# DavidXu-JJ/StreetUnveiler

Measured on AMD Instinct MI355X. Metric: Msplats/s fwd+bwd @1920x1080, 3M Gaussians, higher is better.
Workload: dtype f32; 1 GPU; C3: 3M Gaussians, 1920x1080, fwd+bwd with depth/normal aux outputs (all 7 aux-map gradients live); gaussians=3000000, width=1920, height=1080, sh_degree=3, frames_per_rank=1, parallelism=single GPU, camera_rig=benchmark

## Files before the change

streetunveiler_amd/csrc/api.hip:

```cpp
#include <cfloat>
#include <cstdarg>
#include <cstdio>
#include <cstring>
#include <cmath>
#include <atomic>
#include <mutex>

#include "launch.h"

using namespace sr;

namespace {

thread_local char g_err[512] = "";
std::atomic<int> g_timing{0};
std::mutex g_ring_mu;

int fail(int code, const char* fmt, ...) {
    va_list ap;
    va_start(ap, fmt);
    vsnprintf(g_err, sizeof(g_err), fmt, ap);
    va_end(ap);
    return code;
}

#define SR_HIP(expr)                                                                                         \
    do {                                                                                                     \
        hipError_t _e = (expr);                                                                              \
        if (_e != hipSuccess) return fail(SR_ERR_HIP, "%s failed: %s (%s:%d)", #expr, hipGetErrorString(_e), \
                                          __FILE__, __LINE__);                                               \
    } while (0)

constexpr int kEvRing = 512;
struct EvRing {
    hipEvent_t ev[kEvRing][2];
    bool closed[kEvRing];
    int created = 0, used = 0;
};
EvRing g_ring[SR_STAGE_COUNT];

struct StageTimer {
    int stage; hipStream_t s; int slot = -1;
    StageTimer(int st, hipStream_t stream) : stage(st), s(stream) {
        const int mode = g_timing.load();
        if (!mode || (mode != 1 && !((mode >> 1) & (1 << stage)))) return;
        std::lock_guard<std::mutex> lk(g_ring_mu);
        EvRing& r = g_ring[stage];
        if (r.used >= kEvRing) return;
        if (r.used >= r.created) {
            if (hipEventCreate(&r.ev[r.created][0]) != hipSuccess || hipEventCreate(&r.ev[r.created][1]) != hipSuccess) return;
            ++r.created;
        }
        slot = r.used++;
        r.closed[slot] = false;
        (void)hipEventRecord(r.ev[slot][0], s);
    }
    ~StageTimer() {
        if (slot < 0) return;
        std::lock_guard<std::mutex> lk(g_ring_mu);
        if (hipEventRecord(g_ring[stage].ev[slot][1], s) == hipSuccess) g_ring[stage].closed[slot] = true;
    }
};

int debug_sync(const SrFrame* frame, hipStream_t s, const char* what) {
    if (!frame->debug) return SR_OK;
    hipError_t e = hipStreamSynchronize(s);
    if (e == hipSuccess) e = hipGetLastError();
    if (e != hipSuccess) return fail(SR_ERR_HIP, "[debug] after %s: %s", what, hipGetErrorString(e));
    return SR_OK;
}

uint32_t* pinned_words() {
    static thread_local uint32_t* pinned = nullptr;
    if (!pinned && hipHostMalloc(reinterpret_cast<void**>(&pinned), 64, hipHostMallocPortable | hipHostMallocMapped) != hipSuccess) { pinned = nullptr; (void)hipGetLastError(); }
    return pinned;
}

int stream_device(hipStream_t s, int* dev) {
    hipDevice_t d = 0;
    if (s && hipStreamGetDevice(s, &d) == hipSuccess) { *dev = (int)d; return SR_OK; }
    (void)hipGetLastError();
    SR_HIP(hipGetDevice(dev));
    return SR_OK;
}

constexpr int kMaxDevices = 64;
std::atomic<int> g_rank_mode[kMaxDevices];
int rank_mode(hipStream_t s, bool force_ballot, RankMode* mode) {
    int dev = 0;
    { const int rc = stream_device(s, &dev); if (rc != SR_OK) return rc; }
    if (dev < 0 || dev >= kMaxDevices) return fail(SR_ERR_UNSUPPORTED, "device index %d beyond %d", dev, kMaxDevices);
    int m = g_rank_mode[dev].load(std::memory_order_acquire);
    if (m == kRankUnknown) {
        hipStreamCaptureStatus cap = hipStreamCaptureStatusNone;
        if (hipStreamIsCapturing(s, &cap) == hipSuccess && cap != hipStreamCaptureStatusNone)
            return fail(SR_ERR_UNSUPPORTED, "the stream is capturing and device %d has not run the rank self-check yet: call sr_rank_mode(stream) once before the capture", dev);
        (void)hipGetLastError();
        struct Scratch { uint32_t* p = nullptr; ~Scratch() { if (p) (void)hipFree(p); } } scratch;
        uint32_t* host = pinned_words();
        uint32_t* result = nullptr;
        const bool temp = !(host && hipHostGetDevicePointer(reinterpret_cast<void**>(&result), host + 8, 0) == hipSuccess && result);
        if (!temp) host[8] = 0;
        else { (void)hipGetLastError(); SR_HIP(hipMalloc(reinterpret_cast<void**>(&scratch.p), 4)); result = scratch.p; SR_HIP(hipMemsetAsync(result, 0, 4, s)); }
        SR_HIP(launch_rank_selfcheck(result, s));
        uint32_t r = 0;
        if (temp) { SR_HIP(hipMemcpyAsync(&r, result, 4, hipMemcpyDeviceToHost, s)); SR_HIP(hipStreamSynchronize(s)); }
        else { SR_HIP(hipStreamSynchronize(s)); r = *reinterpret_cast<volatile uint32_t*>(host + 8); }
        if (!(r & 0x100u)) return fail(SR_ERR_HIP, "the rank self-check kernel did not report back");
        m = (r & 1u) ? kRankAtomic : ((r & 2u) ? kRankBallot : kRankNone);
        g_rank_mode[dev].store(m, std::memory_order_release);
    }
    if (m == kRankNone) return fail(SR_ERR_UNSUPPORTED, "neither LDS-atomic nor ballot ranking passes the self-check on device %d", dev);
    *mode = force_ballot ? kRankBallot : static_cast<RankMode>(m);
    return SR_OK;
}

constexpr int kMaxTilesPerAxis = SR_MAX_TILES_PER_AXIS;
template <class T> T* at(void* base, size_t off) { return reinterpret_cast<T*>(static_cast<char*>(base) + off); }
struct Carver {
    size_t off = 0;
    size_t take(size_t bytes) { const size_t o = off; off = align_up(off + bytes, 256); return o; }
};

struct GeomLayout {
    size_t recs, depth_keys, tiles_touched, rect, clamped, sorted_keys, sorted_gid, rect_sorted, first, sh_jac, block_base, base_bytes,
        counts, temp, temp_bytes, total;
};
GeomLayout geom_layout(int P) {
    GeomLayout L{};
    const size_t n = (size_t)(P > 0 ? P : 1);
    Carver c;
    L.recs = c.take(n * kRecFloats * 4);
    L.depth_keys = c.take(n * 4);
    L.tiles_touched = c.take(n * 4);
    L.rect = c.take(n * 8);
    L.clamped = c.take(n);
    L.sorted_keys = c.take(n * 4);
    L.sorted_gid = c.take(n * 4);
    L.rect_sorted = c.take(n * 8);
    L.first = c.take(n * 4);
    L.sh_jac = c.take(n * 36);
    L.base_bytes = tile_scan_temp_bytes(P);
    L.block_base = c.take(L.base_bytes);
    const size_t n_scan_blocks = (n + 2047) / 2048;
    L.counts = L.block_base + n_scan_blocks * 4;
    static thread_local int memo_P = -1;
    static thread_local size_t memo_bytes = 0;
    if (memo_P != P) {
        memo_bytes = depth_sort_temp_bytes(P);
        const size_t hx = align_up(expand_x_hist_bytes(P, kMaxTilesPerAxis), 256);
        if (hx > memo_bytes) memo_bytes = hx;
        memo_P = P;
    }
    L.temp_bytes = memo_bytes;
    L.temp = c.take(L.temp_bytes);
    L.total = c.off;
    return L;
}
enum FrameCount { kCountDuplicates = 0, kCountVisible = 1, kCountOverflow = 2 };
struct GeomView {
    float4* recs; uint32_t* depth_keys; uint32_t* tiles_touched; uint2* rect; uint8_t* clamped;
    uint32_t* sorted_keys; uint32_t* sorted_gid; uint2* rect_sorted; uint32_t* first;
    float* sh_jac;
    uint32_t* block_base; void* temp;
    uint32_t* counts;
};
GeomView geom_view(void* geom, const GeomLayout& L) {
    return GeomView{at<float4>(geom, L.recs), at<uint32_t>(geom, L.depth_keys), at<uint32_t>(geom, L.tiles_touched), at<uint2>(geom, L.rect),
                    at<uint8_t>(geom, L.clamped), at<uint32_t>(geom, L.sorted_keys), at<uint32_t>(geom, L.sorted_gid), at<uint2>(geom, L.rect_sorted),
                    at<uint32_t>(geom, L.first), at<float>(geom, L.sh_jac), at<uint32_t>(geom, L.block_base), at<void>(geom, L.temp),
                    at<uint32_t>(geom, L.counts)};
}

struct BinLayout {
    size_t columns, point_list, hit_mask, ranges, order, tile_counts, row_total, n_columns, hist, hist_bytes, total;
};
BinLayout bin_layout(uint32_t D, int W, int H) {
    BinLayout L{};
    const size_t n = (size_t)(D > 0 ? D : 1);
    const int tiles = ((W + 7) / 8) * ((H + 7) / 8);
    Carver c;
    L.columns = c.take(n * 8);
    L.point_list = c.take(n * 4);
    L.hit_mask = c.take(n * 2);
    L.ranges = c.take((size_t)(tiles > 0 ? tiles : 1) * 8);
    L.order = c.take((size_t)(tiles > 0 ? tiles : 1) * 4);
    L.tile_counts = c.take((size_t)(tiles > 0 ? tiles : 1) * 4);
    L.row_total = c.take((size_t)kMaxTilesPerAxis * 4);
    L.n_columns = c.take(4);
    L.hist_bytes = expand_y_hist_bytes(D, (H + 7) / 8);
    L.hist = c.take(L.hist_bytes);
    L.total = c.off;
    return L;
}
struct BinView {
    uint2* columns;
    uint32_t* point_list; uint16_t* hit_mask; uint2* ranges; uint32_t* order; uint32_t* tile_counts; uint32_t* row_total; uint32_t* n_columns; uint32_t* hist;
    uint32_t* class_list() const { return reinterpret_cast<uint32_t*>(columns); }
};
BinView bin_view(void* binning, const BinLayout& L) {
    return BinView{at<uint2>(binning, L.columns), at<uint32_t>(binning, L.point_list), at<uint16_t>(binning, L.hit_mask), at<uint2>(binning, L.ranges),
                   at<uint32_t>(binning, L.order), at<uint32_t>(binning, L.tile_counts), at<uint32_t>(binning, L.row_total), at<uint32_t>(binning, L.n_columns),
                   at<uint32_t>(binning, L.hist)};
}

struct ImgLayout { size_t final_T, n_contrib, total; };
ImgLayout img_layout(int W, int H) {
    ImgLayout L{};
    const size_t hw = (size_t)(W > 0 ? W : 1) * (size_t)(H > 0 ? H : 1);
    L.final_T = 0;
    L.n_contrib = align_up(hw * 3 * 4, 256);
    L.total = align_up(L.n_contrib + hw * 2 * 4, 256);
    return L;
}
struct ImgView { float* final_T; uint32_t* n_contrib; };
ImgView img_view(void* image, const ImgLayout& L) { return ImgView{at<float>(image, L.final_T), at<uint32_t>(image, L.n_contrib)}; }

size_t record_bytes(int color_channels) { return (size_t)(color_channels == 9 ? kGradFloats + 4 : kGradFloats) * 4; }
struct WorkspaceLayout { size_t written, total; };
WorkspaceLayout workspace_layout(uint32_t D, int color_channels) {
    const size_t n = (size_t)(D > 0 ? D : 1);
    WorkspaceLayout L{};
    L.written = align_up(n * record_bytes(color_channels), 256);
    L.total = L.written + align_up(n, 256);
    return L;
}
struct WorkspaceView { float4* records; uint8_t* written; };
WorkspaceView workspace_view(void* workspace, uint32_t D, int color_channels) {
    return WorkspaceView{static_cast<float4*>(workspace), at<uint8_t>(workspace, workspace_layout(D, color_channels).written)};
}

struct TileShape { int w, h; };
TileShape tile_shape(const SrFrame* frame) {
    return TileShape{frame->tile_width > 0 ? frame->tile_width : kTile, frame->tile_height > 0 ? frame->tile_height : kTile};
}

int check_common(const SrFrame* frame, const SrGaussians* g) {
    if (!frame || !g) return fail(SR_ERR_INVALID_ARGUMENT, "frame / gaussians is NULL");
    if (frame->image_width <= 0 || frame->image_height <= 0) return fail(SR_ERR_INVALID_ARGUMENT, "bad image size %dx%d", frame->image_width, frame->image_height);
    if (g->P < 0) return fail(SR_ERR_INVALID_ARGUMENT, "P < 0");
    {
        const TileShape t = tile_shape(frame);
        const bool known = (t.w == 16 && t.h == 16) || (t.w == 8 && t.h == 8) || (t.w == 16 && t.h == 8) || (t.w == 32 && t.h == 8) || (t.w == 32 && t.h == 16);
        if (!known) return fail(SR_ERR_UNSUPPORTED, "tile shape %dx%d not in {8x8, 16x8, 16x16, 32x8, 32x16}", t.w, t.h);
    }
    if (!frame->bg || !frame->viewmatrix || !frame->projmatrix || !frame->campos) return fail(SR_ERR_INVALID_ARGUMENT, "bg / viewmatrix / projmatrix / campos must be non-NULL device pointers");
    if (g->P > 0) {
        if (!g->means3D || !g->opacities) return fail(SR_ERR_INVALID_ARGUMENT, "means3D / opacities is NULL");
        if (g->color_channels == 9) {
            if (!g->shs || !g->colors_precomp) return fail(SR_ERR_INVALID_ARGUMENT, "9 colour channels need SHs AND a [P,6] precomputed colour array");
        } else if ((g->shs != nullptr) == (g->colors_precomp != nullptr)) return fail(SR_ERR_INVALID_ARGUMENT, "Please provide exactly one of either SHs or precomputed colors!");
        if (g->color_channels != 0 && g->color_channels != 3 && g->color_channels != 6 && g->color_channels != 9) return fail(SR_ERR_UNSUPPORTED, "color_channels %d not in {3, 6, 9}", g->color_channels);
        if (g->activations & ~(SR_ACT_EXP_SCALES | SR_ACT_SIGMOID_OPACITY | SR_ACT_NORMALIZE_ROTATIONS)) return fail(SR_ERR_UNSUPPORTED, "unknown activation bits 0x%x", g->activations);
        if (g->color_channels == 6 && g->shs) return fail(SR_ERR_INVALID_ARGUMENT, "6 colour channels need precomputed colors, not SHs");
        const bool sr_pair = g->scales != nullptr && g->rotations != nullptr;
        if ((g->scales != nullptr) != (g->rotations != nullptr) || sr_pair == (g->transMat_precomp != nullptr))
            return fail(SR_ERR_INVALID_ARGUMENT, "Please provide exactly one of either scale/rotation pair or precomputed transMat!");
        if (g->shs) {
            if (frame->sh_degree < 0 || frame->sh_degree > 3) return fail(SR_ERR_UNSUPPORTED, "sh_degree %d not in 0..3", frame->sh_degree);
            if (g->sh_coeffs < (frame->sh_degree + 1) * (frame->sh_degree + 1)) return fail(SR_ERR_INVALID_ARGUMENT, "shs has %d coefficients, degree %d needs %d", g->sh_coeffs, frame->sh_degree, (frame->sh_degree + 1) * (frame->sh_degree + 1));
        }
    }
    return SR_OK;
}

int check_backward_frame(const SrFrame* frame) {
#if SR_BACKWARD_WH_FROM_FOCAL
    if (!(frame->tanfovx > 0.f) || !(frame->tanfovy > 0.f) || !std::isfinite(frame->tanfovx) || !std::isfinite(frame->tanfovy))
        return fail(SR_ERR_INVALID_ARGUMENT, "tanfovx / tanfovy must be finite and > 0 for a backward call (got %g, %g)", (double)frame->tanfovx, (double)frame->tanfovy);
#else
    (void)frame;
#endif
    return SR_OK;
}

FrameDev make_frame(const SrFrame* frame, const SrGaussians* g) {
    FrameDev f{};
    f.W = frame->image_width; f.H = frame->image_height;
    f.bw_W = f.W; f.bw_H = f.H;
#if SR_BACKWARD_WH_FROM_FOCAL
    if (frame->tanfovx > 0.f && frame->tanfovy > 0.f && std::isfinite(frame->tanfovx) && std::isfinite(frame->tanfovy)) {
        const float focal_x = (float)f.W / (2.0f * frame->tanfovx), focal_y = (float)f.H / (2.0f * frame->tanfovy);
        f.bw_W = (int)(focal_x * frame->tanfovx * 2); f.bw_H = (int)(focal_y * frame->tanfovy * 2);
    }
#endif
    const TileShape t = tile_shape(frame);
    f.tile_w = t.w; f.tile_h = t.h;
    f.inv_tile_w = 1.f / (float)f.tile_w; f.inv_tile_h = 1.f / (float)f.tile_h;
    f.tiles_x = (f.W + f.tile_w - 1) / f.tile_w; f.tiles_y = (f.H + f.tile_h - 1) / f.tile_h;
    f.sh_degree = frame->sh_degree; f.sh_coeffs = g->sh_coeffs;
    f.colors = g->color_channels == 6 ? 6 : (g->color_channels == 9 ? 9 : 3);
    f.activations = g->activations;
    f.scale_modifier = frame->scale_modifier;
    f.bg = frame->bg; f.view = frame->viewmatrix; f.proj = frame->projmatrix; f.campos = frame->campos;
    f.overflow = nullptr;
    return f;
}
void set_backward_state(FrameDev* f, const SrFrame* frame, const GeomView& G) {
    f->first = G.first; f->first_base = G.block_base; f->sh_jac = G.sh_jac;
    if (frame->flags & SR_FLAG_BINNING_CAPACITY) f->overflow = G.counts + kCountOverflow;
}

int choose_blend(const SrFrame* frame, const FrameDev& f, bool forward_call, BlendChoice* out) {
    const uint32_t flags = frame->flags;
    const uint32_t pair = flags & (SR_FLAG_ONE_WAVE_BACKWARD | SR_FLAG_COOP_BACKWARD | SR_FLAG_ROW_BACKWARD);
    if (pair & (pair - 1))
        return fail(SR_ERR_INVALID_ARGUMENT, "SR_FLAG_ONE_WAVE_BACKWARD, SR_FLAG_COOP_BACKWARD and SR_FLAG_ROW_BACKWARD exclude each other (flags 0x%x)", pair);
    const bool reference = f.tile_w == 16 && f.tile_h == 16 && f.colors == 3;
    const bool cull = !(flags & SR_FLAG_NO_QUADRANT_CULL), counters = forward_call && frame->blend_counters != nullptr;
    const bool rows = forward_call && (flags & SR_FLAG_ROW_MAPPED_FORWARD), quads = forward_call && (flags & SR_FLAG_QUADRANT_MAPPED_FORWARD);
    const bool fwd_only = forward_call && (flags & SR_FLAG_FORWARD_ONLY);
    if (fwd_only && counters) return fail(SR_ERR_UNSUPPORTED, "SR_FLAG_FORWARD_ONLY and blend_counters exclude each other");
    if (counters && !(f.tile_w == 16 && f.tile_h == 16 && (f.colors == 3 || f.colors == 6)))
        return fail(SR_ERR_UNSUPPORTED, "blend_counters: the counting variant of the forward blend exists for the 16x16 tile with 3 or 6 colour channels only");
    if (rows && quads) return fail(SR_ERR_INVALID_ARGUMENT, "SR_FLAG_ROW_MAPPED_FORWARD and SR_FLAG_QUADRANT_MAPPED_FORWARD exclude each other");
    if (rows && (!reference || counters || !cull))
        return fail(SR_ERR_UNSUPPORTED, "SR_FLAG_ROW_MAPPED_FORWARD: 16x16 tile, three colour channels, no counters, culling on");
    if ((pair & SR_FLAG_ROW_BACKWARD) && (!reference || counters || !cull || quads || fwd_only))
        return fail(SR_ERR_UNSUPPORTED, "SR_FLAG_ROW_BACKWARD: 16x16 tile, three colour channels, no counters, culling on, the row-mapped forward, a backward to follow");
    out->cull = cull;
    out->mask = HitMaskFormat::kQuadrant;
    out->backward = BackwardBlend::kOneWave;
    out->forward = counters ? ForwardBlend::kCounting : ForwardBlend::kQuadrantBands;
    if (!reference) return SR_OK;
    out->backward = (pair & SR_FLAG_ROW_BACKWARD) ? BackwardBlend::kRows
                    : (pair & SR_FLAG_ONE_WAVE_BACKWARD) ? BackwardBlend::kOneWave
                    : (pair & SR_FLAG_COOP_BACKWARD) ? BackwardBlend::kCoop : BackwardBlend::kByTileCount;
    if (counters) return SR_OK;
    if (cull && !rows && !quads && (pair & SR_FLAG_COOP_BACKWARD)) out->forward = ForwardBlend::kCoop;
    else if (pair & SR_FLAG_ROW_BACKWARD) { out->forward = ForwardBlend::kRowsCellMasks; out->mask = HitMaskFormat::kCell; }
    else if (rows) out->forward = ForwardBlend::kRows;
    else if (cull && !quads) out->forward = ForwardBlend::kDevicePicked;
    return SR_OK;
}

}

extern "C" {

int sr_abi_version(void) { return SR_ABI_VERSION; }
uint32_t sr_build_switches(void) { return SR_SWITCH_BITS; }
const char* sr_last_error(void) { return g_err; }

size_t sr_geom_bytes(int32_t P) { return geom_layout(P).total; }
size_t sr_binning_bytes(int32_t P, uint32_t num_rendered, int32_t W, int32_t H) { (void)P; return bin_layout(num_rendered, W, H).total; }
size_t sr_image_bytes(int32_t W, int32_t H) { return img_layout(W, H).total; }
size_t sr_backward_workspace_bytes(int32_t P, uint32_t num_rendered, int32_t color_channels) { (void)P; return workspace_layout(num_rendered, color_channels).total; }

int sr_geom_view(void* geom, size_t geom_bytes, int32_t P, SrGeomView* out) {
    if (!geom || !out) return fail(SR_ERR_INVALID_ARGUMENT, "NULL argument");
    const GeomLayout L = geom_layout(P);
    if (geom_bytes < L.total) return fail(SR_ERR_BUFFER_TOO_SMALL, "geom buffer %zu < %zu", geom_bytes, L.total);
    const GeomView G = geom_view(geom, L);
    out->splats = reinterpret_cast<float*>(G.recs); out->depth_keys = G.depth_keys;
    out->tiles_touched = G.tiles_touched; out->clamped = G.clamped;
    out->sorted_gid = G.sorted_gid;
    out->frame_counts = G.counts;
    return SR_OK;
}

int sr_binning_view(void* binning, size_t binning_bytes, int32_t P, uint32_t D, int32_t W, int32_t H, SrBinningView* out) {
    (void)P;
    if (!binning || !out) return fail(SR_ERR_INVALID_ARGUMENT, "NULL argument");
    const BinLayout L = bin_layout(D, W, H);
    if (binning_bytes < L.total) return fail(SR_ERR_BUFFER_TOO_SMALL, "binning buffer %zu < %zu", binning_bytes, L.total);
    const BinView B = bin_view(binning, L);
    out->point_list = B.point_list;
    out->ranges = reinterpret_cast<uint32_t*>(B.ranges); out->tile_order = B.order;
    return SR_OK;
}

int sr_image_view(void* image, size_t image_bytes, int32_t W, int32_t H, SrImageView* out) {
    if (!image || !out) return fail(SR_ERR_INVALID_ARGUMENT, "NULL argument");
    const ImgLayout L = img_layout(W, H);
    if (image_bytes < L.total) return fail(SR_ERR_BUFFER_TOO_SMALL, "image buffer %zu < %zu", image_bytes, L.total);
    const ImgView I = img_view(image, L);
    out->final_T = I.final_T; out->n_contrib = I.n_contrib;
    return SR_OK;
}

int sr_forward_plan(const SrFrame* frame, const SrGaussians* g, void* geom, size_t geom_bytes, int32_t* radii,
                    uint32_t* num_rendered_host, void* stream) {
    if (int rc = check_common(frame, g)) return rc;
    if (!num_rendered_host) return fail(SR_ERR_INVALID_ARGUMENT, "num_rendered_host is NULL");
    *num_rendered_host = 0;
    const int P = g->P;
    if (P == 0) return SR_OK;
    if (!geom || !radii) return fail(SR_ERR_INVALID_ARGUMENT, "geom / radii is NULL");
    const GeomLayout L = geom_layout(P);
    if (geom_bytes < L.total) return fail(SR_ERR_BUFFER_TOO_SMALL, "geom buffer %zu < %zu", geom_bytes, L.total);
    const GeomView G = geom_view(geom, L);
    hipStream_t s = static_cast<hipStream_t>(stream);
    FrameDev f = make_frame(frame, g);
    f.sh_jac = (frame->flags & SR_FLAG_FORWARD_ONLY) ? nullptr : G.sh_jac;
    {
        StageTimer t(SR_STAGE_PREPROCESS, s);
        SR_HIP(launch_preprocess_forward(P, f, *g, G.recs, G.depth_keys, G.tiles_touched, G.rect, G.clamped, radii, s));
    }
    if (int rc = debug_sync(frame, s, "preprocess_forward")) return rc;
    RankMode sort_mode = kRankUnknown;
    if (int rc = rank_mode(s, (frame->flags & SR_FLAG_BALLOT_RANKING) != 0, &sort_mode)) return rc;
    const bool read_back = !(frame->flags & SR_FLAG_BINNING_CAPACITY);
    uint32_t* pinned = read_back ? pinned_words() : nullptr;
    uint32_t* pinned_dev = nullptr;
    if (pinned && (hipHostGetDevicePointer(reinterpret_cast<void**>(&pinned_dev), pinned, 0) != hipSuccess)) pinned_dev = nullptr;
    {
        StageTimer t(SR_STAGE_SCAN, s);
        SR_HIP(run_tile_count_scan(P, G.tiles_touched, G.first, G.block_base, L.base_bytes, pinned_dev, s));
    }
    if (int rc = debug_sync(frame, s, "emission_scan")) return rc;
    hipEvent_t copied = nullptr;
    if (read_back) {
        static thread_local hipEvent_t copied_ev[kMaxDevices] = {};
        int dev = 0;
        SR_HIP(hipGetDevice(&dev));
        if (dev >= 0 && dev < kMaxDevices) {
            if (!copied_ev[dev] && hipEventCreateWithFlags(&copied_ev[dev], hipEventDisableTiming) != hipSuccess) copied_ev[dev] = nullptr;
            copied = copied_ev[dev];
        }
        if (!pinned_dev) SR_HIP(hipMemcpyAsync(pinned ? pinned : num_rendered_host, G.counts + kCountDuplicates, 4, hipMemcpyDeviceToHost, s));
        if (copied && pinned && hipEventRecord(copied, s) != hipSuccess) copied = nullptr;
    }
    {
        StageTimer t(SR_STAGE_DEPTH_SORT, s);
        SR_HIP(run_depth_sort(P, G.depth_keys, G.rect, G.sorted_keys, G.sorted_gid, G.rect_sorted, G.temp, L.temp_bytes, sort_mode,
                              (frame->flags & SR_FLAG_ONE_SWEEP_SORT) != 0, f.tiles_x, f.tiles_y, G.counts + kCountVisible, s));
    }
    if (!read_back) {
        *num_rendered_host = 0xFFFFFFFFu;
        return debug_sync(frame, s, "depth_sort");
    }
    if (int rc = debug_sync(frame, s, "depth_sort")) return rc;
    if (copied && pinned) SR_HIP(hipEventSynchronize(copied));
    else SR_HIP(hipStreamSynchronize(s));
    if (pinned) *num_rendered_host = *reinterpret_cast<volatile uint32_t*>(pinned);
    return SR_OK;
}

namespace {
int bin_duplicates(const SrFrame* frame, const SrGaussians* g, const FrameDev& f, void* geom, size_t geom_bytes, const BinView& B,
                   uint32_t D, hipStream_t s, float4** recs_out) {
    const int P = g->P;
    const int n_tiles = f.tiles_x * f.tiles_y;
    *recs_out = nullptr;
    if (P > 0 && D > 0) {
        if (!geom) return fail(SR_ERR_INVALID_ARGUMENT, "geom is NULL");
        const GeomLayout L = geom_layout(P);
        if (geom_bytes < L.total) return fail(SR_ERR_BUFFER_TOO_SMALL, "geom buffer %zu < %zu", geom_bytes, L.total);
        const GeomView G = geom_view(geom, L);
        *recs_out = G.recs;
        if (f.tiles_x > kMaxTilesPerAxis || f.tiles_y > kMaxTilesPerAxis)
            return fail(SR_ERR_INVALID_ARGUMENT, "%d x %d tiles: at most %d per axis (use a larger tile)", f.tiles_x, f.tiles_y, kMaxTilesPerAxis);
        if (L.temp_bytes < expand_x_hist_bytes(P, f.tiles_x)) return fail(SR_ERR_BUFFER_TOO_SMALL, "geom scratch too small for the column histogram");
        RankMode sort_mode = kRankUnknown;
        if (int rc = rank_mode(s, (frame->flags & SR_FLAG_BALLOT_RANKING) != 0, &sort_mode)) return rc;
        if (frame->flags & SR_FLAG_BINNING_CAPACITY)
            SR_HIP(run_capacity_guard(G.counts, D, s));
        {
            StageTimer t(SR_STAGE_EXPAND_X, s);
            SR_HIP(run_expand_columns(P, f.tiles_x, n_tiles, G.rect_sorted, G.sorted_gid, B.columns, B.n_columns, static_cast<uint32_t*>(G.temp), B.row_total,
                                      B.tile_counts, sort_mode, G.counts + kCountVisible, s));
        }
        if (int rc = debug_sync(frame, s, "expand_columns")) return rc;
        {
            StageTimer t(SR_STAGE_EXPAND_Y, s);
            SR_HIP(run_expand_rows(D, f.tiles_x, f.tiles_y, B.columns, B.n_columns, B.hist, B.row_total, B.point_list, B.tile_counts, sort_mode, s));
        }
        if (int rc = debug_sync(frame, s, "expand_rows")) return rc;
    } else {
        SR_HIP(launch_zero_bytes(B.tile_counts, sizeof(uint32_t) * (size_t)n_tiles, s));
    }
    {
        StageTimer t(SR_STAGE_RANGES, s);
        SR_HIP(run_tile_ranges_order(n_tiles, B.tile_counts, B.ranges, B.order, s));
    }
    return debug_sync(frame, s, "tile_ranges");
}

struct ClassLayout { size_t state, last, tile_total, ranges, total; };
ClassLayout class_layout(int W, int H, int n_classes) {
    ClassLayout L{};
    const size_t hw = (size_t)(W > 0 ? W : 1) * (size_t)(H > 0 ? H : 1), n = (size_t)(n_classes > 0 ? n_classes : 1);
    const size_t tiles = (size_t)((W + 7) / 8) * (size_t)((H + 7) / 8);
    L.state = 0;
    L.last = align_up(n * 3 * hw * 4, 256);
    L.tile_total = L.last + align_up(n * hw * 4, 256);
    L.ranges = L.tile_total + align_up((tiles > 0 ? tiles : 1) * n * 4, 256);
    L.total = L.ranges + align_up((tiles > 0 ? tiles : 1) * n * 8, 256);
    return L;
}
struct ClassView { float* state; uint32_t* last; uint32_t* tile_total; uint2* ranges; };
ClassView class_view(void* class_image, const ClassLayout& L) {
    return ClassView{at<float>(class_image, L.state), at<uint32_t>(class_image, L.last), at<uint32_t>(class_image, L.tile_total), at<uint2>(class_image, L.ranges)};
}

enum class ClassIds { kInColors, kOwnArray };
int check_class_pass(const SrFrame* frame, const SrGaussians* g, int n_classes, ClassIds ids, bool refuse_transmat) {
    if (int rc = check_common(frame, g)) return rc;
    if (frame->flags & SR_FLAG_BINNING_CAPACITY) return fail(SR_ERR_UNSUPPORTED, "SR_FLAG_BINNING_CAPACITY serves the operator (sr_forward_* / sr_backward*), not the per-class pass");
    if (n_classes < 1 || n_classes > 6) return fail(SR_ERR_UNSUPPORTED, "n_classes %d not in 1..6", n_classes);
    if (ids == ClassIds::kInColors && g->P > 0 && (g->shs || !g->colors_precomp || (g->color_channels != 0 && g->color_channels != 3)))
        return fail(SR_ERR_INVALID_ARGUMENT, "the per-class distortion pass takes the class ids in colors_precomp[P,3] (column 0), no SHs");
    if (refuse_transmat && g->transMat_precomp) return fail(SR_ERR_UNSUPPORTED, "the per-class pass takes scales and rotations, not a precomputed transMat");
    return SR_OK;
}
}

int sr_forward_render(const SrFrame* frame, const SrGaussians* g, void* geom, size_t geom_bytes, void* binning,
                      size_t binning_bytes, void* image, size_t image_bytes, uint32_t D, float* out_color,
                      float* out_allmap, void* stream) {
    if (int rc = check_common(frame, g)) return rc;
    const FrameDev f = make_frame(frame, g);
    BlendChoice blend;
    if (int rc = choose_blend(frame, f, true, &blend)) return rc;
    const bool fwd_only = (frame->flags & SR_FLAG_FORWARD_ONLY) != 0;
    if (!binning || (!image && !fwd_only) || !out_color || !out_allmap) return fail(SR_ERR_INVALID_ARGUMENT, "binning / image / out_color / out_allmap is NULL");
    const int W = frame->image_width, H = frame->image_height;
    const BinLayout BL = bin_layout(D, W, H);
    const ImgLayout IL = img_layout(W, H);
    if (binning_bytes < BL.total) return fail(SR_ERR_BUFFER_TOO_SMALL, "binning buffer %zu < %zu", binning_bytes, BL.total);
    if (!fwd_only && image_bytes < IL.total) return fail(SR_ERR_BUFFER_TOO_SMALL, "image buffer %zu < %zu", image_bytes, IL.total);
    const BinView B = bin_view(binning, BL);
    const ImgView I = fwd_only ? ImgView{nullptr, nullptr} : img_view(image, IL);
    hipStream_t s = static_cast<hipStream_t>(stream);
    float4* recs = nullptr;
    if (int rc = bin_duplicates(frame, g, f, geom, geom_bytes, B, D, s, &recs)) return rc;
    {
        StageTimer t(SR_STAGE_BLEND_FWD, s);
        const GeomView G = geom_view(geom, geom_layout(g->P));
        SR_HIP(launch_render_forward(f, B.ranges, B.order, B.point_list, recs, g->colors_precomp, out_color, out_allmap, I.final_T, I.n_contrib,
                                     fwd_only ? nullptr : B.hit_mask, blend, reinterpret_cast<unsigned long long*>(frame->blend_counters), G.counts, s));
    }
    return debug_sync(frame, s, "render_forward");
}

size_t sr_class_image_bytes(int32_t W, int32_t H, int32_t n_classes) { return class_layout(W, H, n_classes).total; }

int sr_class_forward_render(const SrFrame* frame, const SrGaussians* g, int32_t n_classes, void* geom, size_t geom_bytes, void* binning,
                            size_t binning_bytes, void* class_image, size_t class_image_bytes, uint32_t D, float* out_dist, void* stream) {
    if (int rc = check_class_pass(frame, g, n_classes, ClassIds::kInColors, false)) return rc;
    if (!binning || !class_image || !out_dist) return fail(SR_ERR_INVALID_ARGUMENT, "binning / class_image / out_dist is NULL");
    if (g->P > 0 && !geom) return fail(SR_ERR_INVALID_ARGUMENT, "geom is NULL (the class ids of the P Gaussians are staged in it, even when no duplicate was emitted)");
    const int W = frame->image_width, H = frame->image_height;
    const BinLayout BL = bin_layout(D, W, H);
    const ClassLayout CL = class_layout(W, H, n_classes);
    if (binning_bytes < BL.total) return fail(SR_ERR_BUFFER_TOO_SMALL, "binning buffer %zu < %zu", binning_bytes, BL.total);
    if (class_image_bytes < CL.total) return fail(SR_ERR_BUFFER_TOO_SMALL, "class image buffer %zu < %zu", class_image_bytes, CL.total);
    const BinView B = bin_view(binning, BL);
    const ClassView C = class_view(class_image, CL);
    hipStream_t s = static_cast<hipStream_t>(stream);
    const FrameDev f = make_frame(frame, g);
    float4* recs = nullptr;
    if (int rc = bin_duplicates(frame, g, f, geom, geom_bytes, B, D, s, &recs)) return rc;
    {
        StageTimer t(SR_STAGE_CLASS_PARTITION, s);
        uint8_t* ids = g->P > 0 && geom ? reinterpret_cast<uint8_t*>(geom_view(geom, geom_layout(g->P)).sh_jac) : nullptr;
        SR_HIP(launch_class_partition(g->P, f.tiles_x * f.tiles_y, n_classes, g->colors_precomp, nullptr, B.ranges, B.point_list, ids, B.class_list(), C.ranges, s));
    }
    if (int rc = debug_sync(frame, s, "class_partition")) return rc;
    {
        StageTimer t(SR_STAGE_CLASS_FWD, s);
        SR_HIP(launch_class_forward(f, n_classes, C.ranges, B.order, B.class_list(), recs, out_dist, C.state, C.last, C.tile_total, B.hit_mask,
                                    (frame->flags & SR_FLAG_NO_QUADRANT_CULL) ? 0 : 1, s));
    }
    return debug_sync(frame, s, "class_forward");
}

int sr_class_backward(const SrFrame* frame, const SrGaussians* g, int32_t n_classes, const int32_t* radii, void* geom, size_t geom_bytes,
                      void* binning, size_t binning_bytes, void* class_image, size_t class_image_bytes, uint32_t D, const float* dL_ddist,
                      void* workspace, size_t workspace_bytes, const SrGradients* grads, void* stream) {
    if (int rc = check_class_pass(frame, g, n_classes, ClassIds::kInColors, false)) return rc;
    if (int rc = check_backward_frame(frame)) return rc;
    if (!grads) return fail(SR_ERR_INVALID_ARGUMENT, "grads is NULL");
    const int P = g->P;
    if (P == 0) return SR_OK;
    if (!radii || !geom || !binning || !class_image || !dL_ddist || !workspace) return fail(SR_ERR_INVALID_ARGUMENT, "NULL buffer argument");
    const int W = frame->image_width, H = frame->image_height;
    const GeomLayout L = geom_layout(P);
    const BinLayout BL = bin_layout(D, W, H);
    const ClassLayout CL = class_layout(W, H, n_classes);
    if (geom_bytes < L.total || binning_bytes < BL.total || class_image_bytes < CL.total) return fail(SR_ERR_BUFFER_TOO_SMALL, "state buffer too small");
    if (workspace_bytes < workspace_layout(D, 3).total) return fail(SR_ERR_BUFFER_TOO_SMALL, "workspace %zu < %zu", workspace_bytes, workspace_layout(D, 3).total);
    const GeomView G = geom_view(geom, L);
    const BinView B = bin_view(binning, BL);
    const ClassView C = class_view(class_image, CL);
    const WorkspaceView ws = workspace_view(workspace, D, 3);
    hipStream_t s = static_cast<hipStream_t>(stream);
    FrameDev f = make_frame(frame, g);
    f.first = G.first; f.first_base = G.block_base; f.sh_jac = G.sh_jac;
    {
        StageTimer t(SR_STAGE_CLASS_BWD, s);
        if (D > 0) SR_HIP(launch_zero_bytes(ws.written, D, s));
        if (D > 0)
            SR_HIP(launch_class_backward(f, n_classes, C.ranges, B.order, B.class_list(), G.recs, C.state, C.last, C.tile_total, dL_ddist, B.hit_mask,
                                         ws.records, ws.written, 0, s));
    }
    if (int rc = debug_sync(frame, s, "class_backward")) return rc;
    {
        StageTimer t(SR_STAGE_PREPROCESS_BWD, s);
        SR_HIP(launch_preprocess_backward(P, f, *g, radii, G.clamped, G.recs, ws.records, ws.written, G.tiles_touched, *grads, s));
    }
    return debug_sync(frame, s, "preprocess_backward");
}

namespace {
struct ClassSharedLayout { ClassLayout C; size_t ids, hit, total; };
ClassSharedLayout class_shared_layout(int P, int W, int H, int n_classes, uint32_t D) {
    ClassSharedLayout L{};
    L.C = class_layout(W, H, n_classes);
    L.ids = L.C.total;
    L.hit = L.ids + align_up((size_t)(P > 0 ? P : 1), 256);
    L.total = L.hit + align_up((size_t)(D > 0 ? D : 1) * 2, 256);
    return L;
}
}

size_t sr_class_shared_bytes(int32_t P, int32_t W, int32_t H, int32_t n_classes, uint32_t D) { return class_shared_layout(P, W, H, n_classes, D).total; }

int sr_class_forward_shared(const SrFrame* frame, const SrGaussians* g, int32_t n_classes, const int32_t* classes, void* geom, size_t geom_bytes,
                            void* binning, size_t binning_bytes, void* class_state, size_t class_state_bytes, uint32_t D, float* out_dist, void* stream) {
    if (int rc = check_class_pass(frame, g, n_classes, ClassIds::kOwnArray, true)) return rc;
    if (!binning || !class_state || !out_dist || (g->P > 0 && !classes)) return fail(SR_ERR_INVALID_ARGUMENT, "binning / class_state / out_dist / classes is NULL");
    const int W = frame->image_width, H = frame->image_height, P = g->P;
    const BinLayout BL = bin_layout(D, W, H);
    const ClassSharedLayout SL = class_shared_layout(P, W, H, n_classes, D);
    if (binning_bytes < BL.total) return fail(SR_ERR_BUFFER_TOO_SMALL, "binning buffer %zu < %zu", binning_bytes, BL.total);
    if (class_state_bytes < SL.total) return fail(SR_ERR_BUFFER_TOO_SMALL, "class state buffer %zu < %zu", class_state_bytes, SL.total);
    float4* recs = nullptr;
    if (P > 0 && D > 0) {
        if (!geom) return fail(SR_ERR_INVALID_ARGUMENT, "geom is NULL");
        const GeomLayout L = geom_layout(P);
        if (geom_bytes < L.total) return fail(SR_ERR_BUFFER_TOO_SMALL, "geom buffer %zu < %zu", geom_bytes, L.total);
        recs = geom_view(geom, L).recs;
    }
    const BinView B = bin_view(binning, BL);
    const ClassView C = class_view(class_state, SL.C);
    hipStream_t s = static_cast<hipStream_t>(stream);
    const FrameDev f = make_frame(frame, g);
    {
        StageTimer t(SR_STAGE_CLASS_PARTITION, s);
        SR_HIP(launch_class_partition(P, f.tiles_x * f.tiles_y, n_classes, nullptr, classes, B.ranges, B.point_list, at<uint8_t>(class_state, SL.ids), B.class_list(),
                                      C.ranges, s));
    }
    if (int rc = debug_sync(frame, s, "class_partition")) return rc;
    {
        StageTimer t(SR_STAGE_CLASS_FWD, s);
        SR_HIP(launch_class_forward(f, n_classes, C.ranges, B.order, B.class_list(), recs, out_dist, C.state, C.last, C.tile_total, at<uint16_t>(class_state, SL.hit),
                                    (frame->flags & SR_FLAG_NO_QUADRANT_CULL) ? 0 : 1, s));
    }
    return debug_sync(frame, s, "class_forward");
}

int sr_class_backward_shared(const SrFrame* frame, const SrGaussians* g, int32_t n_classes, void* geom, size_t geom_bytes, void* binning,
                             size_t binning_bytes, void* class_state, size_t class_state_bytes, uint32_t D, const float* dL_ddist, void* workspace,
                             size_t workspace_bytes, void* stream) {
    if (int rc = check_class_pass(frame, g, n_classes, ClassIds::kOwnArray, false)) return rc;
    if (int rc = check_backward_frame(frame)) return rc;
    const int P = g->P;
    if (P == 0 || D == 0) return SR_OK;
    if (!geom || !binning || !class_state || !dL_ddist || !workspace) return fail(SR_ERR_INVALID_ARGUMENT, "NULL buffer argument");
    const int W = frame->image_width, H = frame->image_height;
    const GeomLayout L = geom_layout(P);
    const BinLayout BL = bin_layout(D, W, H);
    const ClassSharedLayout SL = class_shared_layout(P, W, H, n_classes, D);
    if (geom_bytes < L.total || binning_bytes < BL.total || class_state_bytes < SL.total) return fail(SR_ERR_BUFFER_TOO_SMALL, "state buffer too small");
    const size_t ws_bytes = workspace_layout(D, g->color_channels).total;
    if (workspace_bytes < ws_bytes) return fail(SR_ERR_BUFFER_TOO_SMALL, "workspace %zu < %zu", workspace_bytes, ws_bytes);
    const GeomView G = geom_view(geom, L);
    const BinView B = bin_view(binning, BL);
    const ClassView C = class_view(class_state, SL.C);
    const WorkspaceView ws = workspace_view(workspace, D, g->color_channels);
    hipStream_t s = static_cast<hipStream_t>(stream);
    FrameDev f = make_frame(frame, g);
    f.first = G.first; f.first_base = G.block_base;
    {
        StageTimer t(SR_STAGE_CLASS_BWD, s);
        SR_HIP(launch_class_backward(f, n_classes, C.ranges, B.order, B.class_list(), G.recs, C.state, C.last, C.tile_total, dL_ddist, at<uint16_t>(class_state, SL.hit),
                                     ws.records, ws.written, (int)(record_bytes(g->color_channels) / 16), s));
    }
    return debug_sync(frame, s, "class_backward_shared");
}

namespace {
struct BackwardCtx {
    int P; GeomView G; BinView B; ImgView I; WorkspaceView ws; FrameDev f; BlendChoice blend; hipStream_t s;
};
int backward_ctx(const SrFrame* frame, const SrGaussians* g, void* geom, size_t geom_bytes, void* binning, size_t binning_bytes,
                 void* image, size_t image_bytes, uint32_t D, void* workspace, size_t workspace_bytes, void* stream, BackwardCtx* c) {
    if (int rc = check_common(frame, g)) return rc;
    if (int rc = check_backward_frame(frame)) return rc;
    c->f = make_frame(frame, g);
    if (int rc = choose_blend(frame, c->f, false, &c->blend)) return rc;
    c->P = g->P;
    if (c->P == 0) return SR_OK;
    if (!geom || !binning || !image || !workspace) return fail(SR_ERR_INVALID_ARGUMENT, "NULL buffer argument");
    const int W = frame->image_width, H = frame->image_height;
    const GeomLayout L = geom_layout(c->P);
    const BinLayout BL = bin_layout(D, W, H);
    const ImgLayout IL = img_layout(W, H);
    if (geom_bytes < L.total) return fail(SR_ERR_BUFFER_TOO_SMALL, "geom buffer %zu < %zu", geom_bytes, L.total);
    if (binning_bytes < BL.total) return fail(SR_ERR_BUFFER_TOO_SMALL, "binning buffer %zu < %zu", binning_bytes, BL.total);
    if (image_bytes < IL.total) return fail(SR_ERR_BUFFER_TOO_SMALL, "image buffer %zu < %zu", image_bytes, IL.total);
    const size_t ws_bytes = workspace_layout(D, g->color_channels).total;
    if (workspace_bytes < ws_bytes) return fail(SR_ERR_BUFFER_TOO_SMALL, "workspace %zu < %zu", workspace_bytes, ws_bytes);
    c->G = geom_view(geom, L); c->B = bin_view(binning, BL); c->I = img_view(image, IL);
    c->ws = workspace_view(workspace, D, g->color_channels);
    c->s = static_cast<hipStream_t>(stream);
    set_backward_state(&c->f, frame, c->G);
    return SR_OK;
}
}

int sr_backward_blend(const SrFrame* frame, const SrGaussians* g, void* geom, size_t geom_bytes, void* binning, size_t binning_bytes,
                      void* image, size_t image_bytes, uint32_t D, const float* dL_dcolor, const float* dL_dallmap, void* workspace,
                      size_t workspace_bytes, void* stream) {
    BackwardCtx c;
    if (int rc = backward_ctx(frame, g, geom, geom_bytes, binning, binning_bytes, image, image_bytes, D, workspace, workspace_bytes, stream, &c)) return rc;
    if (c.P == 0) return SR_OK;
    if (!dL_dcolor || !dL_dallmap) return fail(SR_ERR_INVALID_ARGUMENT, "dL_dcolor / dL_dallmap is NULL");
    {
        StageTimer t(SR_STAGE_BLEND_BWD, c.s);
        if (D > 0) SR_HIP(launch_zero_bytes(c.ws.written, D, c.s));
        if (D > 0)
            SR_HIP(launch_render_backward(c.f, c.B.ranges, c.B.order, c.B.point_list, c.G.recs, g->colors_precomp, c.I.final_T, c.I.n_contrib, dL_dcolor, dL_dallmap,
                                          c.B.hit_mask, c.ws.records, c.ws.written, !(frame->flags & SR_FLAG_NO_PRECOMP_COLOR_GRAD), c.blend.backward, c.s));
    }
    return debug_sync(frame, c.s, "render_backward");
}

// ... 376 lines not shown
```

streetunveiler_amd/csrc/binning.hip:

```cpp
#include "launch.h"

namespace sr {

constexpr int kXpThreads = 256, kXpWaves = kXpThreads / 64;
constexpr int kXpInputsX = 1024, kXpInputsY = 2048;
template <int AXIS> constexpr int xp_inputs() { return AXIS == 0 ? kXpInputsX : kXpInputsY; }
constexpr int kXpBatch = 2048;
constexpr int kXpMaxBins = 1024;
__device__ inline uint32_t pack_column(int miny, int h, int tx) { return (uint32_t)miny | ((uint32_t)h << 10) | ((uint32_t)tx << 21); }

__device__ inline uint32_t block_exclusive_scan(uint32_t x, uint32_t* s_w, uint32_t& total) {
    const int lane = threadIdx.x & 63, w = threadIdx.x >> 6;
    uint32_t incl = wave_inclusive_scan(x);
    __syncthreads();
    if (lane == 63) s_w[w] = incl;
    __syncthreads();
    uint32_t off = 0, tot = 0;
#pragma unroll
    for (int k = 0; k < kXpWaves; ++k) { const uint32_t c = s_w[k]; if (k < w) off += c; tot += c; }
    total = tot;
    return off + incl - x;
}

template <int AXIS> __device__ inline void expansion_of(uint2 item, int& start, int& len) {
// ... 27 lines not shown
        const uint32_t idx = base + (uint32_t)(i * kXpThreads + tid);
        if (idx < n) {
            const uint2 it = in[idx];
            int start, len; expansion_of<AXIS>(it, start, len);
            if (len) {
                atomicAdd(&s_diff[start], 1u); atomicSub(&s_diff[start + len], 1u);
                if (AXIS == 1) {
                    const int tx = (int)(it.y >> 21);
                    const uint32_t rel = (uint32_t)(tx - tx0);
                    if (rel < 4u) { atomicAdd(&s_full[rel][start], 1u); atomicSub(&s_full[rel][start + len], 1u); }
                    else for (int k = 0; k < len; ++k) atomicAdd(&tile_counts[(start + k) * tiles_x + tx], 1u);
                }
            }
        }
    }
    __syncthreads();
    {
        uint32_t v[4], sum = 0;
#pragma unroll
        for (int j = 0; j < 4; ++j) { const int b = 4 * tid + j; sum += b < bins ? s_diff[b] : 0u; v[j] = sum; }
        uint32_t total;
        const uint32_t excl = block_exclusive_scan(sum, s_w, total);
#pragma unroll
        for (int j = 0; j < 4; ++j) { const int b = 4 * tid + j; if (b < bins) hist[(size_t)b * stride + blockIdx.x] = excl + v[j]; }
    }
    if (AXIS == 1 && tx0 + w < tiles_x) {
        uint32_t carry = 0;
        for (int c = 0; c < bins; c += 64) {
            const int row = c + lane;
            uint32_t incl = wave_inclusive_scan(row < bins ? s_full[w][row] : 0u);
            const uint32_t cnt = carry + incl;
            if (row < bins && cnt) atomicAdd(&tile_counts[row * tiles_x + tx0 + w], cnt);
            carry += (uint32_t)__shfl((int)incl, 63);
        }
    }
}

__global__ __launch_bounds__(kXpThreads) void expand_scan_rows_kernel(uint32_t* __restrict__ hist, int stride, uint32_t n_host,
                                                                      const uint32_t* __restrict__ n_dev, int inputs_per_block,
                                                                      uint32_t* __restrict__ row_total) {
    __shared__ uint32_t s_w[kXpWaves];
    const uint32_t n = n_dev ? *n_dev : n_host;
    const int nblocks = (int)((n + (uint32_t)inputs_per_block - 1) / (uint32_t)inputs_per_block);
    uint32_t* row = hist + (size_t)blockIdx.x * stride;
    uint32_t carry = 0;
    for (int c = 0; c < nblocks; c += kXpThreads) {
        const int i = c + (int)threadIdx.x;
        const uint32_t x = i < nblocks ? row[i] : 0u;
        uint32_t total;
        const uint32_t excl = block_exclusive_scan(x, s_w, total);
        if (i < nblocks) row[i] = carry + excl;
        carry += total;
    }
    if (threadIdx.x == 0) row_total[blockIdx.x] = carry;
}

template <int AXIS, int kBits, bool kAtomicRank>
__global__ __launch_bounds__(kXpThreads) void expand_scatter_kernel(
    const uint2* __restrict__ in, uint32_t n_host, const uint32_t* __restrict__ n_dev, int bins, const uint32_t* __restrict__ hist, int stride,
    const uint32_t* __restrict__ row_total,
    const uint32_t* __restrict__ sorted_gid, uint2* __restrict__ columns_out, uint32_t* __restrict__ n_columns_out,
    uint32_t* __restrict__ point_list) {
    constexpr int kBins = 1 << kBits;
    constexpr int kPer = kBins / kXpThreads > 0 ? kBins / kXpThreads : 1;
    constexpr int kInputs = xp_inputs<AXIS>(), kXpPerThread = kInputs / kXpThreads;
    __shared__ __attribute__((aligned(16))) uint8_t s_start[kXpBatch];
    __shared__ uint32_t s_prefix[kInputs + 1];
    __shared__ uint32_t s_count[kXpWaves][kBins];
    __shared__ uint32_t s_lstart[kBins];
    __shared__ uint32_t s_goff[kBins];
    __shared__ uint32_t s_w[kXpWaves];
    __shared__ uint32_t s_id[kXpBatch];
    __shared__ uint32_t s_rows[AXIS == 0 ? kXpBatch : 1];
    __shared__ uint16_t s_dig[kXpBatch];
    const int tid = threadIdx.x, lane = tid & 63, w = tid >> 6;
    const uint32_t n = n_dev ? *n_dev : n_host;
    const uint32_t base = blockIdx.x * (uint32_t)kInputs;
    if (base >= n) return;
    const int n_items = (int)min((uint32_t)kInputs, n - base);
    uint32_t E;
    uint32_t it_first[kXpPerThread];
    {
        uint32_t incl[kXpPerThread], sum = 0;
#pragma unroll
        for (int i = 0; i < kXpPerThread; ++i) {
            const int j = tid * kXpPerThread + i;
            int start = 0, len = 0;
            if (j < n_items) {
                const uint2 it = in[base + j];
                expansion_of<AXIS>(it, start, len);
            }
            it_first[i] = len ? sum : 0xFFFFFFFFu;
            sum += (uint32_t)len;
            incl[i] = sum;
        }
        for (int k = tid; k < kXpBatch / 4; k += kXpThreads) reinterpret_cast<uint32_t*>(s_start)[k] = 0;
        const uint32_t excl = block_exclusive_scan(sum, s_w, E);
#pragma unroll
        for (int i = 0; i < kXpPerThread; ++i) {
            s_prefix[tid * kXpPerThread + i + 1] = excl + incl[i];
            if (it_first[i] != 0xFFFFFFFFu) it_first[i] += excl;
        }
        if (tid == 0) s_prefix[0] = 0;
    }
    {
        uint32_t v[kPer], sum = 0;
#pragma unroll
        for (int j = 0; j < kPer; ++j) { const int d = tid * kPer + j; const uint32_t c = (d < bins) ? row_total[d] : 0u; v[j] = sum; sum += c; }
        uint32_t total;
        const uint32_t excl = block_exclusive_scan(sum, s_w, total);
#pragma unroll
        for (int j = 0; j < kPer; ++j) { const int d = tid * kPer + j; if (d < kBins) s_goff[d] = d < bins ? excl + v[j] + hist[(size_t)d * stride + blockIdx.x] : 0u; }
        if (AXIS == 0 && blockIdx.x == 0 && tid == 0) *n_columns_out = total;
    }
    for (uint32_t q0 = 0; q0 < E; q0 += kXpBatch) {
        for (int k = tid; k < kXpWaves * kBins; k += kXpThreads) (&s_count[0][0])[k] = 0;
#pragma unroll
        for (int i = 0; i < kXpPerThread; ++i)
            if (it_first[i] - q0 < (uint32_t)kXpBatch) s_start[it_first[i] - q0] = 1;
        __syncthreads();
        const uint32_t s0 = q0 + (uint32_t)(w * (kXpBatch / kXpWaves));
        uint32_t marks_before = 0;
        if (s0 < E) {
            int lo = 0;
#pragma unroll
            for (int step = kInputs / 2; step > 0; step >>= 1)
                if (lo + step < n_items && s_prefix[lo + step] <= s0) lo += step;
            marks_before = (uint32_t)lo + (s_prefix[lo] == s0 ? 0u : 1u);
        }
        uint32_t dig[kXpBatch / kXpThreads], id[kXpBatch / kXpThreads], rows[AXIS == 0 ? kXpBatch / kXpThreads : 1];
#pragma unroll
        for (int i = 0; i < kXpBatch / kXpThreads; ++i) {
            const uint32_t slot = s0 + (uint32_t)(i * 64 + lane);
            dig[i] = 0; id[i] = 0;
            if (AXIS == 0) rows[i] = 0;
            const bool mark = slot < E && s_start[slot - q0] != 0;
            const unsigned long long marks = ballot64(mark);
            const uint32_t lo = marks_before + __builtin_amdgcn_mbcnt_hi((uint32_t)(marks >> 32), __builtin_amdgcn_mbcnt_lo((uint32_t)marks, 0u)) +
                                (mark ? 1u : 0u) - 1u;
            marks_before += (uint32_t)__popcll(marks);
            if (slot < E) {
                const uint2 it = in[base + lo];
                int start, len; expansion_of<AXIS>(it, start, len);
                dig[i] = (uint32_t)start + (slot - s_prefix[lo]);
                if (AXIS == 0) { id[i] = sorted_gid[base + lo]; rows[i] = (it.x >> 16) | ((it.y >> 16) << 10); }
                else id[i] = it.x;
                atomicAdd(&s_count[w][dig[i]], 1u);
            }
        }
        __syncthreads();
        for (int k = tid; k < kXpBatch / 4; k += kXpThreads) reinterpret_cast<uint32_t*>(s_start)[k] = 0;
        uint32_t tot[kPer];
        {
            uint32_t sum = 0;
#pragma unroll
            for (int j = 0; j < kPer; ++j) {
                const int d = tid * kPer + j;
                tot[j] = 0;
                if (d < kBins) {
#pragma unroll
                    for (int k = 0; k < kXpWaves; ++k) tot[j] += s_count[k][d];
                }
                sum += tot[j];
            }
            uint32_t total;
            uint32_t run = block_exclusive_scan(sum, s_w, total);
#pragma unroll
            for (int j = 0; j < kPer; ++j) {
                const int d = tid * kPer + j;
                if (d < kBins) {
                    s_lstart[d] = run;
#pragma unroll
                    for (int k = 0; k < kXpWaves; ++k) { const uint32_t c = s_count[k][d]; s_count[k][d] = run; run += c; }
                }
            }
        }
        __syncthreads();
#pragma unroll
        for (int i = 0; i < kXpBatch / kXpThreads; ++i) {
            const uint32_t slot = q0 + (uint32_t)(w * (kXpBatch / kXpWaves) + i * 64 + lane);
            const bool live = slot < E;
            const uint32_t d = dig[i];
            const uint32_t pos = take_run_slot<kAtomicRank>(s_count[w], d, live, kBits);
            if (live) { s_id[pos] = id[i]; s_dig[pos] = (uint16_t)d; if (AXIS == 0) s_rows[pos] = rows[i]; }
        }
        __syncthreads();
        const uint32_t count = min((uint32_t)kXpBatch, E - q0);
#pragma unroll
        for (int i = 0; i < kXpBatch / kXpThreads; ++i) {
            const uint32_t li = (uint32_t)(i * kXpThreads + tid);
            if (li < count) {
                const uint32_t d = s_dig[li];
                const uint32_t g = s_goff[d] + (li - s_lstart[d]);
                if (AXIS == 0) columns_out[g] = make_uint2(s_id[li], s_rows[li] | (d << 21));
                else point_list[g] = s_id[li];
            }
        }
        __syncthreads();
#pragma unroll
        for (int j = 0; j < kPer; ++j) { const int d = tid * kPer + j; if (d < kBins) s_goff[d] += tot[j]; }
    }
}

constexpr int kOrderThreads = 1024, kOrderClasses = 16;
__device__ __forceinline__ uint32_t row_inclusive_scan16(uint32_t x) {
    int v = (int)x;
    v += __builtin_amdgcn_update_dpp(0, v, 0x111, 0xf, 0xf, true);
    v += __builtin_amdgcn_update_dpp(0, v, 0x112, 0xf, 0xf, true);
    v += __builtin_amdgcn_update_dpp(0, v, 0x114, 0xf, 0xf, true);
    v += __builtin_amdgcn_update_dpp(0, v, 0x118, 0xf, 0xf, true);
    return (uint32_t)v;
}
__global__ __launch_bounds__(kOrderThreads) void tile_ranges_order_kernel(int n_tiles, const uint32_t* __restrict__ counts, uint2* __restrict__ ranges,
                                                                          uint32_t* __restrict__ order) {
    constexpr int kPer = 8, kWaves = kOrderThreads / 64, kChunk = kOrderThreads * kPer;
    static_assert(kWaves == 16 && kOrderClasses == 16, "the cross-wave prefix below runs on 16 x 16 values, one 16-lane row per class");
    __shared__ uint32_t s_cls[kOrderClasses][kWaves];
    __shared__ uint32_t s_off[kOrderClasses][kWaves];
    __shared__ uint32_t s_tot[kOrderClasses];
    __shared__ uint32_t s_wsum[kWaves], s_woff[kWaves];
    __shared__ uint32_t s_carry, s_cls_base[kOrderClasses];
    const int tid = threadIdx.x, lane = tid & 63, w = tid >> 6;
    auto cls_of = [](uint32_t len) { return len ? min(kOrderClasses - 1, max(0, (int)__clz(len) - 11)) : kOrderClasses - 1; };
    const bool single_chunk = n_tiles <= kChunk;
    if (tid < kOrderClasses) s_cls_base[tid] = 0;
    if (tid == 0) s_carry = 0;
    if (!single_chunk) {
        uint32_t my_cls[kOrderClasses];
#pragma unroll
        for (int k = 0; k < kOrderClasses; ++k) my_cls[k] = 0;
        for (int t = tid; t < n_tiles; t += kOrderThreads) { const int c = cls_of(counts[t]);
#pragma unroll
            for (int k = 0; k < kOrderClasses; ++k) my_cls[k] += (c == k); }
        __syncthreads();
#pragma unroll
        for (int k = 0; k < kOrderClasses; ++k) {
            const uint32_t v = wave_inclusive_scan(my_cls[k]);
            if (lane == 63 && v) atomicAdd(&s_cls_base[k], v);
        }
        __syncthreads();
        if (tid == 0) { uint32_t run = 0; for (int k = 0; k < kOrderClasses; ++k) { const uint32_t c = s_cls_base[k]; s_cls_base[k] = run; run += c; } }
    }
    __syncthreads();
    for (int base = 0; base < n_tiles; base += kChunk) {
        const int t0 = base + tid * kPer;
        uint32_t c[kPer], sum = 0;
#pragma unroll
        for (int i = 0; i < kPer; ++i) { c[i] = t0 + i < n_tiles ? counts[t0 + i] : 0u; sum += c[i]; }
        const uint32_t incl = wave_inclusive_scan(sum);
        if (lane == 63) s_wsum[w] = incl;
        uint32_t mine[kOrderClasses];
#pragma unroll
        for (int k = 0; k < kOrderClasses; ++k) mine[k] = 0;
#pragma unroll
        for (int i = 0; i < kPer; ++i) { if (t0 + i < n_tiles) { const int cl = cls_of(c[i]);
#pragma unroll
            for (int k = 0; k < kOrderClasses; ++k) mine[k] += (cl == k); } }
        uint32_t before[kOrderClasses];
#pragma unroll
        for (int k = 0; k < kOrderClasses; ++k) {
            const uint32_t v = wave_inclusive_scan(mine[k]);
            before[k] = v - mine[k];
            if (lane == 63) s_cls[k][w] = v;
        }
        __syncthreads();
        if (tid < kOrderClasses * kWaves) {
            const uint32_t v = s_cls[tid >> 4][tid & 15], in = row_inclusive_scan16(v);
            s_off[tid >> 4][tid & 15] = in - v;
            if ((tid & 15) == 15) s_tot[tid >> 4] = in;
        } else if (tid < kOrderClasses * kWaves + 64) {
            const int j = tid - kOrderClasses * kWaves;
            const uint32_t v = j < kWaves ? s_wsum[j] : 0u, in = row_inclusive_scan16(v);
            if (j < kWaves) s_woff[j] = in - v;
        }
        __syncthreads();
        if (single_chunk) {
            if (tid == 0) { uint32_t run = 0; for (int k = 0; k < kOrderClasses; ++k) { s_cls_base[k] = run; run += s_tot[k]; } }
            __syncthreads();
        }
        uint32_t run = s_carry + s_woff[w] + incl - sum;
#pragma unroll
        for (int k = 0; k < kOrderClasses; ++k) before[k] += s_cls_base[k] + s_off[k][w];
#pragma unroll
        for (int i = 0; i < kPer; ++i) {
            if (t0 + i < n_tiles) {
                ranges[t0 + i] = c[i] ? make_uint2(run, run + c[i]) : make_uint2(0u, 0u);
                run += c[i];
                const int cl = cls_of(c[i]);
                uint32_t pos = 0;
#pragma unroll
                for (int k = 0; k < kOrderClasses; ++k) { if (cl == k) { pos = before[k]; before[k] += 1; } }
                order[pos] = (uint32_t)(t0 + i);
            }
        }
        __syncthreads();
        if (tid == kOrderThreads - 1) s_carry = run;
        if (tid < kOrderClasses) s_cls_base[tid] += s_tot[tid];
        __syncthreads();
    }
}

size_t depth_sort_temp_bytes(int P) {
    const uint32_t n = (uint32_t)(P > 0 ? P : 1);
    return align_up(radix_sort_temp_bytes(n), 256);
}
size_t tile_scan_temp_bytes(int P) { return tile_count_scan_temp_bytes((uint32_t)(P > 0 ? P : 1)); }

size_t expand_x_hist_bytes(int P, int tiles_x) { return (size_t)tiles_x * (((size_t)(P > 0 ? P : 1) + kXpInputsX - 1) / kXpInputsX) * 4; }
size_t expand_y_hist_bytes(uint32_t D, int tiles_y) { return (size_t)tiles_y * (((size_t)(D > 0 ? D : 1) + kXpInputsY - 1) / kXpInputsY) * 4; }

hipError_t run_depth_sort(int P, const uint32_t* depth_keys, const uint2* rect, uint32_t* sorted_keys,
                          uint32_t* sorted_gid, uint2* rect_sorted, void* temp, size_t temp_bytes, RankMode rank_mode, bool one_sweep, int tiles_x,
                          int tiles_y, const uint32_t* n_visible, hipStream_t s) {
    if (P == 0) return hipSuccess;
    const int bx = 32 - __builtin_clz((unsigned)(tiles_x > 0 ? tiles_x : 1)), by = 32 - __builtin_clz((unsigned)(tiles_y > 0 ? tiles_y : 1));
    return radix_sort_pairs(depth_keys, nullptr, sorted_keys, sorted_gid, (uint32_t)P, 32, temp, temp_bytes, s, rect, rect_sorted, rank_mode, one_sweep, bx, by, n_visible);
}

hipError_t run_tile_count_scan(int P, const uint32_t* tiles_touched, uint32_t* first, void* block_base, size_t base_bytes, uint32_t* total_host,
                               hipStream_t s) {
    if (P == 0) return hipSuccess;
    return tile_count_scan(tiles_touched, first, (uint32_t)P, block_base, base_bytes, total_host, s);
}

template <int AXIS, bool kAtomicRank, typename... Args>
static void launch_expand_scatter_r(int bins, int blocks, hipStream_t s, Args... a) {
    if (bins <= 128) hipLaunchKernelGGL((expand_scatter_kernel<AXIS, 7, kAtomicRank>), dim3(blocks), dim3(kXpThreads), 0, s, a...);
    else if (bins <= 256) hipLaunchKernelGGL((expand_scatter_kernel<AXIS, 8, kAtomicRank>), dim3(blocks), dim3(kXpThreads), 0, s, a...);
    else if (bins <= 512) hipLaunchKernelGGL((expand_scatter_kernel<AXIS, 9, kAtomicRank>), dim3(blocks), dim3(kXpThreads), 0, s, a...);
    else hipLaunchKernelGGL((expand_scatter_kernel<AXIS, 10, kAtomicRank>), dim3(blocks), dim3(kXpThreads), 0, s, a...);
}
template <int AXIS, typename... Args>
static void launch_expand_scatter(RankMode rank_mode, int bins, int blocks, hipStream_t s, Args... a) {
    if (rank_mode == kRankAtomic) launch_expand_scatter_r<AXIS, true>(bins, blocks, s, a...);
    else launch_expand_scatter_r<AXIS, false>(bins, blocks, s, a...);
}

hipError_t run_expand_columns(int P, int tiles_x, int n_tiles, const uint2* rect_sorted, const uint32_t* sorted_gid, uint2* columns,
                              uint32_t* n_columns, uint32_t* hist, uint32_t* row_total, uint32_t* tile_counts, RankMode rank_mode, const uint32_t* n_visible,
                              hipStream_t s) {
    if (P == 0) return hipSuccess;
    if (tiles_x > kXpMaxBins || (rank_mode != kRankAtomic && rank_mode != kRankBallot)) return hipErrorInvalidValue;
    const int nb = (P + kXpInputsX - 1) / kXpInputsX;
    hipLaunchKernelGGL(expand_hist_kernel<0>, dim3(nb), dim3(kXpThreads), 0, s, rect_sorted, (uint32_t)P, n_visible, tiles_x, hist, nb,
                       tiles_x, tile_counts, n_tiles);
    hipLaunchKernelGGL(expand_scan_rows_kernel, dim3(tiles_x), dim3(kXpThreads), 0, s, hist, nb, (uint32_t)P, n_visible, kXpInputsX, row_total);
    launch_expand_scatter<0>(rank_mode, tiles_x, nb, s, rect_sorted, (uint32_t)P, n_visible, tiles_x, (const uint32_t*)hist, nb,
                             (const uint32_t*)row_total, sorted_gid, columns, n_columns, (uint32_t*)nullptr);
    return hipGetLastError();
}

hipError_t run_expand_rows(uint32_t D, int tiles_x, int tiles_y, const uint2* columns, const uint32_t* n_columns, uint32_t* hist, uint32_t* row_total,
                           uint32_t* point_list, uint32_t* tile_counts, RankMode rank_mode, hipStream_t s) {
    if (D == 0) return hipSuccess;
    if (tiles_y > kXpMaxBins || (rank_mode != kRankAtomic && rank_mode != kRankBallot)) return hipErrorInvalidValue;
    const int nb = (int)((D + kXpInputsY - 1) / kXpInputsY);
    hipLaunchKernelGGL(expand_hist_kernel<1>, dim3(nb), dim3(kXpThreads), 0, s, columns, D, n_columns, tiles_y, hist, nb, tiles_x, tile_counts,
                       tiles_x * tiles_y);
    hipLaunchKernelGGL(expand_scan_rows_kernel, dim3(tiles_y), dim3(kXpThreads), 0, s, hist, nb, D, n_columns, kXpInputsY, row_total);
    launch_expand_scatter<1>(rank_mode, tiles_y, nb, s, columns, D, n_columns, tiles_y, (const uint32_t*)hist, nb, (const uint32_t*)row_total,
                             (const uint32_t*)nullptr, (uint2*)nullptr, (uint32_t*)nullptr, point_list);
    return hipGetLastError();
}

__global__ void capacity_guard_kernel(uint32_t* __restrict__ counts, uint32_t capacity) {
    const uint32_t over = counts[0] > capacity ? 1u : 0u;
    counts[2] = over;
    if (over) counts[1] = 0u;
}
__global__ __launch_bounds__(256) void zero_bytes_kernel(uint8_t* __restrict__ p, size_t n) {
    const size_t head = (size_t)((16 - (reinterpret_cast<uintptr_t>(p) & 15)) & 15);
    const size_t h = head < n ? head : n;
    const size_t body = (n - h) / 16;
    const size_t i = (size_t)blockIdx.x * 256 + threadIdx.x, stride = (size_t)gridDim.x * 256;
    uint4* q = reinterpret_cast<uint4*>(p + h);
    for (size_t k = i; k < body; k += stride) q[k] = make_uint4(0u, 0u, 0u, 0u);
    if (i < h) p[i] = 0;
    const size_t tail0 = h + body * 16;
    if (i < n - tail0) p[tail0 + i] = 0;
}
hipError_t launch_zero_bytes(void* p, size_t n, hipStream_t s) {
    if (n == 0) return hipSuccess;
    const size_t blocks = (n / 16 + 255) / 256;
    hipLaunchKernelGGL(zero_bytes_kernel, dim3((unsigned)(blocks < 1 ? 1 : (blocks > 4096 ? 4096 : blocks))), dim3(256), 0, s, static_cast<uint8_t*>(p), n);
    return hipGetLastError();
}

hipError_t run_capacity_guard(uint32_t* counts, uint32_t capacity, hipStream_t s) {
    hipLaunchKernelGGL(capacity_guard_kernel, dim3(1), dim3(1), 0, s, counts, capacity);
    return hipGetLastError();
}

hipError_t run_tile_ranges_order(int n_tiles, const uint32_t* tile_counts, uint2* ranges, uint32_t* order, hipStream_t s) {
    if (n_tiles == 0) return hipSuccess;
    hipLaunchKernelGGL(tile_ranges_order_kernel, dim3(1), dim3(kOrderThreads), 0, s, n_tiles, tile_counts, ranges, order);
    return hipGetLastError();
}

}
```

streetunveiler_amd/csrc/common.h:

```cpp
#pragma once
#include <hip/hip_runtime.h>
#include <stdint.h>

#include "../../include/surfel_raster.h"
#include "../../include/surfel_switches.h"

#if defined(__HIP_DEVICE_COMPILE__) && !defined(__gfx950__)
#error "these kernels are written for gfx950 (MI355X): wave64, v_permlane16/32_swap, DPP row controls, and the LDS-atomic lane order the sort kernels rank by (checked at run time, api.hip rank_mode)"
#endif

namespace sr {

constexpr int kTile = SR_TILE;
constexpr int kBlock = kTile * kTile;
constexpr float kNear = 0.2f;
constexpr float kFar = 100.0f;
constexpr float kFilterSize = 0.707106f;
constexpr float kFilterInvSquare = 2.0f;
constexpr float kCutoff = 3.0f;
constexpr float kAlphaCap = 0.99f;
constexpr float kAlphaFloor = 1.0f / 255.0f;
constexpr float kTStop = 0.0001f;
constexpr uint32_t kCulledKey = 0xFFFFFFFFu;

constexpr int kRecQuads = 5;
constexpr int kRecFloats = SR_SPLAT_FLOATS;

constexpr int kGradQuads = 6;
constexpr int kGradFloats = SR_GRAD_FLOATS;

struct FrameDev {
    int W, H, tiles_x, tiles_y;
    int bw_W, bw_H;
    int tile_w, tile_h;
    float inv_tile_w, inv_tile_h;
    int sh_degree, sh_coeffs;
    int colors;
    int activations;
    float scale_modifier;
    const float* bg;
    const float* view;
    const float* proj;
    const float* campos;
    const uint32_t* first;
    const uint32_t* first_base;
    float* sh_jac;
    const uint32_t* overflow;
};
constexpr int kScanTile = 2048;
__device__ __forceinline__ uint32_t first_index(const FrameDev& f, uint32_t gid) { return f.first[gid] + f.first_base[gid / kScanTile]; }

__host__ __device__ inline size_t align_up(size_t x, size_t a) { return (x + a - 1) / a * a; }

__device__ __forceinline__ unsigned long long ballot64(bool p) { return __builtin_amdgcn_ballot_w64(p); }

__device__ __forceinline__ uint32_t wave_inclusive_scan(uint32_t x) {
    int v = (int)x;
    v += __builtin_amdgcn_update_dpp(0, v, 0x111, 0xf, 0xf, true);
    v += __builtin_amdgcn_update_dpp(0, v, 0x112, 0xf, 0xf, true);
    v += __builtin_amdgcn_update_dpp(0, v, 0x114, 0xf, 0xf, true);
    v += __builtin_amdgcn_update_dpp(0, v, 0x118, 0xf, 0xf, true);
    v += __builtin_amdgcn_update_dpp(0, v, 0x142, 0xa, 0xf, true);
    v += __builtin_amdgcn_update_dpp(0, v, 0x143, 0xc, 0xf, true);
    return (uint32_t)v;
}

template <bool kAtomic>
__device__ __forceinline__ uint32_t take_run_slot(uint32_t* run, uint32_t d, bool live, int bits) {
    uint32_t pos = 0;
    if (kAtomic) {
        if (live) pos = atomicAdd(&run[d], 1u);
        return pos;
    }
    unsigned long long same = ballot64(live);
    for (int b = 0; b < bits; ++b) {
        const unsigned long long vote = ballot64(((d >> b) & 1u) != 0u);
        same &= ((d >> b) & 1u) ? vote : ~vote;
    }
    const uint32_t lane = threadIdx.x & 63u;
    const uint32_t rank = (uint32_t)__popcll(same & ((1ull << lane) - 1ull));
    if (live) pos = run[d] + rank;
    __builtin_amdgcn_wave_barrier();
    if (live && rank == 0) run[d] += (uint32_t)__popcll(same);
    __builtin_amdgcn_wave_barrier();
    return pos;
}
enum RankMode { kRankUnknown = 0, kRankAtomic = 1, kRankBallot = 2, kRankNone = 3 };

}
```

streetunveiler_amd/csrc/launch.h:

```cpp
#pragma once
#include "common.h"

namespace sr {

enum class ForwardBlend {
    kDevicePicked,
    kQuadrantBands,
    kRows,
    kRowsCellMasks,
    kCoop,
    kCounting,
};
enum class BackwardBlend {
    kByTileCount,
    kOneWave,
    kCoop,
    kRows,
};
enum class HitMaskFormat { kQuadrant, kCell };
struct BlendChoice {
    ForwardBlend forward;
    BackwardBlend backward;
    HitMaskFormat mask;
    bool cull;
};

hipError_t launch_preprocess_forward(int P, const FrameDev& f, const SrGaussians& g, float4* recs, uint32_t* depth_keys,
                                     uint32_t* tiles_touched, uint2* rect, uint8_t* clamped, int32_t* radii, hipStream_t s);
hipError_t launch_preprocess_backward(int P, const FrameDev& f, const SrGaussians& g, const int32_t* radii,
                                      const uint8_t* clamped, const float4* recs, const float4* inst_grads, const uint8_t* written,
                                      const uint32_t* tiles_touched, const SrGradients& out, hipStream_t s);
hipError_t launch_mark_visible(int P, const float* means3D, const float* view, uint8_t* present, hipStream_t s);
hipError_t launch_sh_gradient_expand(int P, int M, int deg, int V, const float* means3D, const float* campos, const float* gc,
                                     float* dL_dsh, hipStream_t s);
hipError_t launch_color_gradients(int P, const FrameDev& f, const int32_t* radii, const uint8_t* clamped, const float4* recs, const float4* inst_grads,
                                  const uint8_t* written, const uint32_t* tiles_touched, bool mask_clamped, float* dL_dcolors, hipStream_t s);

size_t radix_sort_temp_bytes(uint32_t n);
hipError_t radix_sort_pairs(const uint32_t* keys_in, const uint32_t* vals_in, uint32_t* keys_out, uint32_t* vals_out, uint32_t n,
                            int total_bits, void* temp, size_t temp_bytes, hipStream_t s, const uint2* aux_src, uint2* aux_out, RankMode rank_mode,
                            bool one_sweep, int rect_bx = 0, int rect_by = 0, const uint32_t* n_live = nullptr);
size_t tile_count_scan_temp_bytes(uint32_t n);
hipError_t tile_count_scan(const uint32_t* counts, uint32_t* out, uint32_t n, void* temp, size_t temp_bytes, uint32_t* total_host, hipStream_t s);
hipError_t launch_rank_selfcheck(uint32_t* result, hipStream_t s);
hipError_t lds_atomic_ranks(const uint32_t* digits, uint32_t* ranks, uint32_t n, int bins, hipStream_t s);

size_t depth_sort_temp_bytes(int P);
size_t tile_scan_temp_bytes(int P);
size_t expand_x_hist_bytes(int P, int tiles_x);
size_t expand_y_hist_bytes(uint32_t D, int tiles_y);
hipError_t run_depth_sort(int P, const uint32_t* depth_keys, const uint2* rect, uint32_t* sorted_keys,
                          uint32_t* sorted_gid, uint2* rect_sorted, void* temp, size_t temp_bytes, RankMode rank_mode, bool one_sweep, int tiles_x,
                          int tiles_y, const uint32_t* n_visible, hipStream_t s);
hipError_t run_tile_count_scan(int P, const uint32_t* tiles_touched, uint32_t* first, void* block_base, size_t base_bytes, uint32_t* total_host,
                               hipStream_t s);
hipError_t run_expand_columns(int P, int tiles_x, int n_tiles, const uint2* rect_sorted, const uint32_t* sorted_gid, uint2* columns,
                              uint32_t* n_columns, uint32_t* hist, uint32_t* row_total, uint32_t* tile_counts, RankMode rank_mode, const uint32_t* n_visible,
                              hipStream_t s);
hipError_t run_expand_rows(uint32_t D, int tiles_x, int tiles_y, const uint2* columns, const uint32_t* n_columns, uint32_t* hist, uint32_t* row_total,
                           uint32_t* point_list, uint32_t* tile_counts, RankMode rank_mode, hipStream_t s);
hipError_t run_tile_ranges_order(int n_tiles, const uint32_t* tile_counts, uint2* ranges, uint32_t* order, hipStream_t s);
hipError_t run_capacity_guard(uint32_t* counts, uint32_t capacity, hipStream_t s);
hipError_t launch_zero_bytes(void* p, size_t n, hipStream_t s);

hipError_t launch_render_forward(const FrameDev& f, const uint2* ranges, const uint32_t* tile_order, const uint32_t* point_list, const float4* recs,
                                 const float* extra, float* out_color, float* out_allmap, float* final_T, uint32_t* n_contrib, uint16_t* hit_mask,
                                 const BlendChoice& blend, unsigned long long* counters, const uint32_t* frame_counts, hipStream_t s);
hipError_t launch_render_backward(const FrameDev& f, const uint2* ranges, const uint32_t* tile_order, const uint32_t* point_list, const float4* recs,
                                  const float* extra, const float* final_T, const uint32_t* n_contrib, const float* dL_dcolor,
                                  const float* dL_dallmap, const uint16_t* hit_mask, float4* inst_grads, uint8_t* written, bool precomp_color_grads,
                                  BackwardBlend blend, hipStream_t s);
hipError_t launch_pair_decisions(const FrameDev& f, const uint2* ranges, const uint32_t* point_list, const float4* recs,
                                 unsigned long long* valid_bits, unsigned long long* use3d_bits, hipStream_t s);

hipError_t launch_class_partition(int P, int n_tiles, int n_classes, const float* class_cols, const int32_t* class_i32, const uint2* ranges,
                                  const uint32_t* point_list, uint8_t* ids, uint32_t* cls_list, uint2* cls_ranges, hipStream_t s);
hipError_t launch_class_forward(const FrameDev& f, int n_classes, const uint2* cls_ranges, const uint32_t* tile_order, const uint32_t* cls_list,
                                const float4* recs, float* out_dist, float* cls_state, uint32_t* cls_last, uint32_t* tile_total, uint16_t* hit_mask,
                                int cull, hipStream_t s);
hipError_t launch_class_backward(const FrameDev& f, int n_classes, const uint2* cls_ranges, const uint32_t* tile_order, const uint32_t* cls_list,
                                 const float4* recs, const float* cls_state, const uint32_t* cls_last, const uint32_t* tile_total,
                                 const float* dL_ddist, const uint16_t* hit_mask, float4* inst_grads, uint8_t* written, int shared_rec_quads, hipStream_t s);

size_t knn_workspace_bytes(int nq, int nr);
hipError_t knn_mean_dist2(int nq, const float* query, int nr, const float* reference, int K, int take_sqrt, float* out, void* ws,
                          size_t ws_bytes, RankMode rank_mode, hipStream_t s);
constexpr int kKnnBox = 512;
struct CloudOrder {
    uint32_t* codes;
    uint32_t* codes_sorted;
    uint32_t* order;
    float4* sorted;
};
size_t cloud_bounds_partial_bytes(int n);
hipError_t cloud_bounds_masked(const float* pts, const uint8_t* active, int n, float* partial, float* bounds, hipStream_t s);
hipError_t cloud_order(const float* pts, const uint8_t* active, bool masked, int n, const float* bounds, const CloudOrder& o, void* sort_temp,
                       size_t temp_bytes, RankMode rank_mode, hipStream_t s);
hipError_t cloud_boxes(const float4* sorted, int n, float4* boxes, hipStream_t s);

size_t cluster_workspace_bytes(int n);
hipError_t cluster_radius(int n, const float* xyz, const uint8_t* active, float radius, int64_t* labels, void* ws, size_t ws_bytes,
                          RankMode rank_mode, hipStream_t s);

struct PostCam {
    int W, H;
    float fx, fy, depth_ratio;
    const float* view;
};
hipError_t launch_postprocess_forward(const PostCam& cam, const float* allmap, float* rend_normal, float* surf_depth,
                                      float* surf_normal, float* surf_point, hipStream_t s);
hipError_t launch_postprocess_backward(const PostCam& cam, const float* allmap, const float* g_rend_normal, const float* g_surf_depth,
                                       const float* g_surf_normal, const float* g_surf_point, float* scratch6, float* g_allmap,
                                       hipStream_t s);

struct LossImages {
    int W, H, C;
    float lambda;
    const float* image;
    const float* gt;
    const float* sky;
    const float* alpha;
};
bool image_loss_supported(int W, int H, int C);
size_t image_loss_partial_bytes();
hipError_t launch_image_loss_forward(const LossImages& a, void* workspace, float* out3, hipStream_t s);
hipError_t launch_image_loss_backward(const LossImages& a, const void* workspace, const float* g_loss, float* g_image, float* g_sky,
                                      float* g_alpha, hipStream_t s);

bool adam_supported(const SrAdamSegment* segments, int n_segments);
hipError_t launch_adam_step(const SrAdamSegment* segments, int n_segments, double beta1, double beta2, double eps, hipStream_t s);
hipError_t launch_densification_stats(int P, const float* viewspace_grad, const int* radii, float* xyz_gradient_accum, float* denom,
                                      float* max_radii2D, hipStream_t s);

struct DensifyRule {
    float max_grad, min_opacity, percent_dense_extent, ws_limit;
    int select;
};
size_t densify_workspace_bytes(int P);
hipError_t densify_plan(int P, const float* accum, const float* denom, const float* opacity, const float* scaling, const DensifyRule& rule,
                        const uint8_t* prune_mask, void* workspace, uint32_t* counts_pinned_dev, hipStream_t s);
const uint32_t* densify_counts_device(int P, const void* workspace);
hipError_t densify_apply(int P, const uint32_t* counts, const float* noise, const float* rotation, const float* scaling,
                         const SrDensifySegment* segments, int n_segments, const void* workspace, hipStream_t s);

struct TsdfViewsDev {
    const float* maps;
    const float* full_proj;
    int V, H, W, channels;
};
struct TsdfSpace {
    float trunc;
    int contract;
    float center[3], radius;
};
struct TsdfGrid {
    float lo[3], step[3];
    int ny, nz, ix0;
};
hipError_t launch_tsdf_fuse(const TsdfViewsDev& views, const TsdfSpace& space, const TsdfGrid* grid, int n, const float* samples, float* tsdf,
                            float* rgb, float* weight, hipStream_t s);

}
```

streetunveiler_amd/csrc/preprocess.hip:

```cpp
#include "launch.h"

namespace sr {

__device__ __constant__ float kSH_C0 = 0.28209479177387814f;
__device__ __constant__ float kSH_C1 = 0.4886025119029199f;
__device__ __constant__ float kSH_C2[5] = {1.0925484305920792f, -1.0925484305920792f, 0.31539156525252005f,
                                            -1.0925484305920792f, 0.5462742152960396f};
__device__ __constant__ float kSH_C3[7] = {-0.5900435899266435f, 2.890611442640554f, -0.4570457994644658f,
                                            0.3731763325901154f, -0.4570457994644658f, 1.445305721320277f,
                                            -0.5900435899266435f};

__device__ __forceinline__ void quat_to_R(const float4 q, float R[9]) {
    const float r = q.x, x = q.y, y = q.z, z = q.w;
    R[0] = 1.f - 2.f * (y * y + z * z); R[1] = 2.f * (x * y - r * z);       R[2] = 2.f * (x * z + r * y);
    R[3] = 2.f * (x * y + r * z);       R[4] = 1.f - 2.f * (x * x + z * z); R[5] = 2.f * (y * z - r * x);
    R[6] = 2.f * (x * z - r * y);       R[7] = 2.f * (y * z + r * x);       R[8] = 1.f - 2.f * (x * x + y * y);
}

__device__ __forceinline__ float2 activate_scales(float2 s, int act) {
    if (act & SR_ACT_EXP_SCALES) { s.x = expf(s.x); s.y = expf(s.y); }
    return s;
}
__device__ __forceinline__ float2 load_scales(const float* __restrict__ scales, int i, int act) {
    return activate_scales(reinterpret_cast<const float2*>(scales)[i], act);
}
__device__ __forceinline__ float4 activate_rotation(float4 q, int act, float& norm) {
    norm = 1.f;
    if (act & SR_ACT_NORMALIZE_ROTATIONS) {
        norm = fmaxf(sqrtf(((q.x * q.x + q.y * q.y) + q.z * q.z) + q.w * q.w), 1e-12f);
        q.x /= norm; q.y /= norm; q.z /= norm; q.w /= norm;
    }
    return q;
}
__device__ __forceinline__ float4 load_rotation(const float* __restrict__ rotations, int i, int act, float& norm) {
    return activate_rotation(reinterpret_cast<const float4*>(rotations)[i], act, norm);
}
__device__ __forceinline__ float sigmoidf(float x) { return 1.f / (1.f + expf(-x)); }

__device__ __forceinline__ void build_B(const float* __restrict__ proj, int W, int H, float B[12]) {
    const float hw = 0.5f * (float)W, hh = 0.5f * (float)H;
    const float cw = 0.5f * (float)(W - 1), ch = 0.5f * (float)(H - 1);
#pragma unroll
    for (int k = 0; k < 4; ++k) {
        const float a0 = proj[4 * k + 0], a1 = proj[4 * k + 1], a3 = proj[4 * k + 3];
        B[0 + k] = hw * a0 + cw * a3;
        B[4 + k] = hh * a1 + ch * a3;
        B[8 + k] = a3;
    }
}

__device__ __forceinline__ float dot3(const float* a, float x, float y, float z) { return (a[0] * x + a[1] * y) + a[2] * z; }

constexpr int kShRowFloats = 48;
constexpr int kShLdsStride = 52;
#ifndef SR_PRE_BLOCK
#define SR_PRE_BLOCK 128
#endif
constexpr int kPreBlock = SR_PRE_BLOCK;

__device__ __forceinline__ void sh_rows_to_lds(const float* __restrict__ shs, int base, int P, float* s_sh, int tid) {
    const int nrows = min(kPreBlock, P - base);
    const int nvec = nrows * (kShRowFloats / 4);
    const float4* src = reinterpret_cast<const float4*>(shs + (size_t)base * kShRowFloats);
    float4* dst = reinterpret_cast<float4*>(s_sh);
    for (int f = tid; f < nvec; f += kPreBlock) {
        const int row = f / 12, c4 = f - row * 12;
        dst[row * (kShLdsStride / 4) + c4] = src[f];
    }
}

__device__ __forceinline__ void sh_rows_from_lds(float* __restrict__ out, int base, int P, const float* s_sh, int tid) {
    const int nrows = min(kPreBlock, P - base);
    const int nvec = nrows * (kShRowFloats / 4);
    float4* dst = reinterpret_cast<float4*>(out + (size_t)base * kShRowFloats);
    const float4* src = reinterpret_cast<const float4*>(s_sh);
    for (int f = tid; f < nvec; f += kPreBlock) {
        const int row = f / 12, c4 = f - row * 12;
        dst[f] = src[row * (kShLdsStride / 4) + c4];
    }
}

template <class Row>
__device__ __forceinline__ void sh_to_rgb(int deg, const Row sh, float dx, float dy, float dz, float rgb[3], uint8_t& clamped) {
#pragma unroll
    for (int c = 0; c < 3; ++c) {
        float res = kSH_C0 * sh[c];
        if (deg > 0) {
            const float x = dx, y = dy, z = dz;
            res = res - kSH_C1 * y * sh[3 + c] + kSH_C1 * z * sh[6 + c] - kSH_C1 * x * sh[9 + c];
            if (deg > 1) {
                const float xx = x * x, yy = y * y, zz = z * z, xy = x * y, yz = y * z, xz = x * z;
                res = res + kSH_C2[0] * xy * sh[12 + c] + kSH_C2[1] * yz * sh[15 + c] +
                      kSH_C2[2] * (2.f * zz - xx - yy) * sh[18 + c] + kSH_C2[3] * xz * sh[21 + c] +
                      kSH_C2[4] * (xx - yy) * sh[24 + c];
                if (deg > 2) {
                    res = res + kSH_C3[0] * y * (3.f * xx - yy) * sh[27 + c] + kSH_C3[1] * xy * z * sh[30 + c] +
                          kSH_C3[2] * y * (4.f * zz - xx - yy) * sh[33 + c] +
                          kSH_C3[3] * z * (2.f * zz - 3.f * xx - 3.f * yy) * sh[36 + c] +
                          kSH_C3[4] * x * (4.f * zz - xx - yy) * sh[39 + c] +
                          kSH_C3[5] * z * (xx - yy) * sh[42 + c] + kSH_C3[6] * x * (xx - 3.f * yy) * sh[45 + c];
                }
            }
        }
        res += 0.5f;
        if (res < 0.f) clamped |= (uint8_t)(1u << c);
        rgb[c] = fmaxf(res, 0.f);
    }
}

constexpr int kShHalfFloats = 24, kShHalfStride = 28;
__device__ __forceinline__ void sh_half_load(const float* __restrict__ shs, int base, int P, int half, int tid, const uint8_t* skip, float4 (&r)[6]) {
    const int nrows = min(kPreBlock, P - base);
    const float4* src = reinterpret_cast<const float4*>(shs + (size_t)base * kShRowFloats);
#pragma unroll
    for (int k = 0; k < 6; ++k) {
        const int f = tid + k * kPreBlock, row = f / 6, c4 = f - row * 6;
        r[k] = (row < nrows && !skip[row]) ? src[row * 12 + half * 6 + c4] : make_float4(0.f, 0.f, 0.f, 0.f);
    }
}
__device__ __forceinline__ void sh_half_store(float* s_sh, int tid, const float4 (&r)[6]) {
    float4* dst = reinterpret_cast<float4*>(s_sh);
#pragma unroll
    for (int k = 0; k < 6; ++k) {
        const int f = tid + k * kPreBlock, row = f / 6, c4 = f - row * 6;
        dst[row * (kShHalfStride / 4) + c4] = r[k];
    }
}
__device__ __forceinline__ void sh_to_rgb_lo(int deg, const float* lo, float x, float y, float z, float res[3]) {
#pragma unroll
    for (int c = 0; c < 3; ++c) {
        float r = kSH_C0 * lo[c];
        if (deg > 0) {
            r = r - kSH_C1 * y * lo[3 + c] + kSH_C1 * z * lo[6 + c] - kSH_C1 * x * lo[9 + c];
            if (deg > 1) {
                const float xx = x * x, yy = y * y, zz = z * z, xy = x * y, yz = y * z, xz = x * z;
                r = r + kSH_C2[0] * xy * lo[12 + c] + kSH_C2[1] * yz * lo[15 + c] + kSH_C2[2] * (2.f * zz - xx - yy) * lo[18 + c] +
                    kSH_C2[3] * xz * lo[21 + c];
            }
        }
        res[c] = r;
    }
}
__device__ __forceinline__ void sh_to_rgb_hi(int deg, const float* hi, float x, float y, float z, const float res[3], float rgb[3], uint8_t& clamped) {
#pragma unroll
    for (int c = 0; c < 3; ++c) {
        float r = res[c];
        if (deg > 1) {
            const float xx = x * x, yy = y * y, zz = z * z, xy = x * y;
            r = r + kSH_C2[4] * (xx - yy) * hi[c];
            if (deg > 2) {
                r = r + kSH_C3[0] * y * (3.f * xx - yy) * hi[3 + c] + kSH_C3[1] * xy * z * hi[6 + c] +
                    kSH_C3[2] * y * (4.f * zz - xx - yy) * hi[9 + c] +
                    kSH_C3[3] * z * (2.f * zz - 3.f * xx - 3.f * yy) * hi[12 + c] +
                    kSH_C3[4] * x * (4.f * zz - xx - yy) * hi[15 + c] +
                    kSH_C3[5] * z * (xx - yy) * hi[18 + c] + kSH_C3[6] * x * (xx - 3.f * yy) * hi[21 + c];
            }
        }
        r += 0.5f;
        if (r < 0.f) clamped |= (uint8_t)(1u << c);
        rgb[c] = fmaxf(r, 0.f);
    }
}
__device__ __forceinline__ void sh_dir_jacobian_lo(int deg, const float* lo, float x, float y, float z, float d[9]) {
#pragma clang fp contract(fast)
#pragma unroll
    for (int c = 0; c < 3; ++c) {
        float dx = 0.f, dy = 0.f, dz = 0.f;
        if (deg > 0) {
            dx = -kSH_C1 * lo[9 + c]; dy = -kSH_C1 * lo[3 + c]; dz = kSH_C1 * lo[6 + c];
            if (deg > 1) {
                dx += (kSH_C2[0] * y) * lo[12 + c] + (-2.f * kSH_C2[2] * x) * lo[18 + c] + (kSH_C2[3] * z) * lo[21 + c];
                dy += (kSH_C2[0] * x) * lo[12 + c] + (kSH_C2[1] * z) * lo[15 + c] + (-2.f * kSH_C2[2] * y) * lo[18 + c];
                dz += (kSH_C2[1] * y) * lo[15 + c] + (4.f * kSH_C2[2] * z) * lo[18 + c] + (kSH_C2[3] * x) * lo[21 + c];
            }
        }
        d[3 * c] = dx; d[3 * c + 1] = dy; d[3 * c + 2] = dz;
    }
}
__device__ __forceinline__ void sh_dir_jacobian_hi(int deg, const float* hi, float x, float y, float z, float len, const float d[9], float J[9]) {
#pragma clang fp contract(fast)
    const float inv_len = 1.f / len;
    const float xx = x * x, yy = y * y, zz = z * z, xy = x * y, yz = y * z, xz = x * z;
#pragma unroll
    for (int c = 0; c < 3; ++c) {
        float dx = d[3 * c], dy = d[3 * c + 1], dz = d[3 * c + 2];
        if (deg > 1) {
            dx += (2.f * kSH_C2[4] * x) * hi[c];
            dy += (-2.f * kSH_C2[4] * y) * hi[c];
            if (deg > 2) {
                dx += (6.f * kSH_C3[0] * xy) * hi[3 + c] + (kSH_C3[1] * yz) * hi[6 + c] + (-2.f * kSH_C3[2] * xy) * hi[9 + c] +
                      (-6.f * kSH_C3[3] * xz) * hi[12 + c] + (kSH_C3[4] * (-3.f * xx + 4.f * zz - yy)) * hi[15 + c] +
                      (2.f * kSH_C3[5] * xz) * hi[18 + c] + (3.f * kSH_C3[6] * (xx - yy)) * hi[21 + c];
                dy += (3.f * kSH_C3[0] * (xx - yy)) * hi[3 + c] + (kSH_C3[1] * xz) * hi[6 + c] + (kSH_C3[2] * (-3.f * yy + 4.f * zz - xx)) * hi[9 + c] +
                      (-6.f * kSH_C3[3] * yz) * hi[12 + c] + (-2.f * kSH_C3[4] * xy) * hi[15 + c] + (-2.f * kSH_C3[5] * yz) * hi[18 + c] +
                      (-6.f * kSH_C3[6] * xy) * hi[21 + c];
                dz += (kSH_C3[1] * xy) * hi[6 + c] + (8.f * kSH_C3[2] * yz) * hi[9 + c] + (3.f * kSH_C3[3] * (2.f * zz - xx - yy)) * hi[12 + c] +
                      (8.f * kSH_C3[4] * xz) * hi[15 + c] + (kSH_C3[5] * (xx - yy)) * hi[18 + c];
            }
        }
        const float nd = (x * dx + y * dy) + z * dz;
        J[3 * c + 0] = (dx - x * nd) * inv_len; J[3 * c + 1] = (dy - y * nd) * inv_len; J[3 * c + 2] = (dz - z * nd) * inv_len;
    }
}

template <class Row>
__device__ __forceinline__ void sh_dir_jacobian(int deg, const Row sh, float x, float y, float z, float len, float J[9]) {
#pragma clang fp contract(fast)
    const float inv_len = 1.f / len;
    const float xx = x * x, yy = y * y, zz = z * z, xy = x * y, yz = y * z, xz = x * z;
#pragma unroll
    for (int c = 0; c < 3; ++c) {
        float dx = 0.f, dy = 0.f, dz = 0.f;
        if (deg > 0) {
            dx = -kSH_C1 * sh[9 + c]; dy = -kSH_C1 * sh[3 + c]; dz = kSH_C1 * sh[6 + c];
            if (deg > 1) {
                dx += (kSH_C2[0] * y) * sh[12 + c] + (-2.f * kSH_C2[2] * x) * sh[18 + c] + (kSH_C2[3] * z) * sh[21 + c] + (2.f * kSH_C2[4] * x) * sh[24 + c];
                dy += (kSH_C2[0] * x) * sh[12 + c] + (kSH_C2[1] * z) * sh[15 + c] + (-2.f * kSH_C2[2] * y) * sh[18 + c] + (-2.f * kSH_C2[4] * y) * sh[24 + c];
                dz += (kSH_C2[1] * y) * sh[15 + c] + (4.f * kSH_C2[2] * z) * sh[18 + c] + (kSH_C2[3] * x) * sh[21 + c];
                if (deg > 2) {
                    dx += (6.f * kSH_C3[0] * xy) * sh[27 + c] + (kSH_C3[1] * yz) * sh[30 + c] + (-2.f * kSH_C3[2] * xy) * sh[33 + c] +
                          (-6.f * kSH_C3[3] * xz) * sh[36 + c] + (kSH_C3[4] * (-3.f * xx + 4.f * zz - yy)) * sh[39 + c] +
                          (2.f * kSH_C3[5] * xz) * sh[42 + c] + (3.f * kSH_C3[6] * (xx - yy)) * sh[45 + c];
                    dy += (3.f * kSH_C3[0] * (xx - yy)) * sh[27 + c] + (kSH_C3[1] * xz) * sh[30 + c] + (kSH_C3[2] * (-3.f * yy + 4.f * zz - xx)) * sh[33 + c] +
                          (-6.f * kSH_C3[3] * yz) * sh[36 + c] + (-2.f * kSH_C3[4] * xy) * sh[39 + c] + (-2.f * kSH_C3[5] * yz) * sh[42 + c] +
                          (-6.f * kSH_C3[6] * xy) * sh[45 + c];
                    dz += (kSH_C3[1] * xy) * sh[30 + c] + (8.f * kSH_C3[2] * yz) * sh[33 + c] + (3.f * kSH_C3[3] * (2.f * zz - xx - yy)) * sh[36 + c] +
                          (8.f * kSH_C3[4] * xz) * sh[39 + c] + (kSH_C3[5] * (xx - yy)) * sh[42 + c];
                }
            }
        }
        const float nd = (x * dx + y * dy) + z * dz;
        J[3 * c + 0] = (dx - x * nd) * inv_len; J[3 * c + 1] = (dy - y * nd) * inv_len; J[3 * c + 2] = (dz - z * nd) * inv_len;
    }
}

template <class RowOut>
__device__ __forceinline__ void sh_basis_adjoint(int deg, int M, RowOut dsh, float x, float y, float z, const float gcol[3]) {
#pragma unroll
    for (int c = 0; c < 3; ++c) {
        const float g = gcol[c];
        dsh[c] = kSH_C0 * g;
        if (deg > 0) {
            dsh[3 + c] = -kSH_C1 * y * g; dsh[6 + c] = kSH_C1 * z * g; dsh[9 + c] = -kSH_C1 * x * g;
            if (deg > 1) {
                const float xx = x * x, yy = y * y, zz = z * z, xy = x * y, yz = y * z, xz = x * z;
                dsh[12 + c] = kSH_C2[0] * xy * g; dsh[15 + c] = kSH_C2[1] * yz * g;
                dsh[18 + c] = kSH_C2[2] * (2.f * zz - xx - yy) * g;
                dsh[21 + c] = kSH_C2[3] * xz * g; dsh[24 + c] = kSH_C2[4] * (xx - yy) * g;
                if (deg > 2) {
                    dsh[27 + c] = kSH_C3[0] * y * (3.f * xx - yy) * g;
                    dsh[30 + c] = kSH_C3[1] * xy * z * g;
                    dsh[33 + c] = kSH_C3[2] * y * (4.f * zz - xx - yy) * g;
                    dsh[36 + c] = kSH_C3[3] * z * (2.f * zz - 3.f * xx - 3.f * yy) * g;
                    dsh[39 + c] = kSH_C3[4] * x * (4.f * zz - xx - yy) * g;
                    dsh[42 + c] = kSH_C3[5] * z * (xx - yy) * g;
                    dsh[45 + c] = kSH_C3[6] * x * (xx - 3.f * yy) * g;
                }
            }
        }
    }
    const int used = (deg + 1) * (deg + 1);
    for (int k = used * 3; k < M * 3; ++k) dsh[k] = 0.f;
}

__device__ __forceinline__ void splat_transform(const float B[12], float px, float py, float pz, const float R[9], float su, float sv, float Tm[9]) {
    const float L0[3] = {R[0] * su, R[3] * su, R[6] * su};
    const float L1[3] = {R[1] * sv, R[4] * sv, R[7] * sv};
#pragma unroll
    for (int r = 0; r < 3; ++r) {
        const float* b = B + 4 * r;
        Tm[3 * r + 0] = dot3(b, L0[0], L0[1], L0[2]);
        Tm[3 * r + 1] = dot3(b, L1[0], L1[1], L1[2]);
        Tm[3 * r + 2] = dot3(b, px, py, pz) + b[3];
    }
}
__device__ __forceinline__ float bbox_cutoff(float act_opacity) {
#if SR_TIGHTBBOX
    return sqrtf(fmaxf(9.f + 2.f * logf(act_opacity), 0.000001f));
#else
    (void)act_opacity;
    return kCutoff;
#endif
}
struct SplatBox { float dist, cx, cy, ex, ey; };
__device__ __forceinline__ SplatBox splat_box(const float Tm[9], float cutoff) {
    const float* Tu = Tm; const float* Tv = Tm + 3; const float* Tw = Tm + 6;
    const float c2 = cutoff * cutoff;
    const float t0 = c2, t1 = c2, t2 = -1.f;
    SplatBox b;
    b.dist = ((Tw[0] * Tw[0]) * t0 + (Tw[1] * Tw[1]) * t1) + (Tw[2] * Tw[2]) * t2;
    const float inv = 1.f / b.dist;
    const float f0 = inv * t0, f1 = inv * t1, f2 = inv * t2;
    b.cx = ((f0 * Tu[0]) * Tw[0] + (f1 * Tu[1]) * Tw[1]) + (f2 * Tu[2]) * Tw[2];
    b.cy = ((f0 * Tv[0]) * Tw[0] + (f1 * Tv[1]) * Tw[1]) + (f2 * Tv[2]) * Tw[2];
    const float tx = ((f0 * Tu[0]) * Tu[0] + (f1 * Tu[1]) * Tu[1]) + (f2 * Tu[2]) * Tu[2];
    const float ty = ((f0 * Tv[0]) * Tv[0] + (f1 * Tv[1]) * Tv[1]) + (f2 * Tv[2]) * Tv[2];
    const float hx = b.cx * b.cx - tx, hy = b.cy * b.cy - ty;
    b.ex = sqrtf(fmaxf(1e-4f, hx)); b.ey = sqrtf(fmaxf(1e-4f, hy));
    return b;
}

template <bool kLdsSH>
__global__ __launch_bounds__(kPreBlock) void preprocess_forward_kernel(
    int P, FrameDev f, const float* __restrict__ means3D, const float* __restrict__ opacities,
    const float* __restrict__ scales, const float* __restrict__ rotations, const float* __restrict__ shs,
    const float* __restrict__ colors_precomp, const float* __restrict__ transMat_precomp,
    const uint8_t* __restrict__ mask, float4* __restrict__ recs, uint32_t* __restrict__ depth_keys,
    uint32_t* __restrict__ tiles_touched, uint2* __restrict__ rect, uint8_t* __restrict__ clamped, int32_t* __restrict__ radii) {
    constexpr int kK1LdsFloats = kPreBlock * (kShHalfStride > kRecFloats + 9 ? kShHalfStride : kRecFloats + 9);
    __shared__ __attribute__((aligned(16))) float s_sh[kLdsSH ? kK1LdsFloats : 4];
    __shared__ uint8_t s_skip[kLdsSH ? kPreBlock : 4];
    const int tid = threadIdx.x, base = blockIdx.x * kPreBlock;
    const int i = base + tid;
    float px = 0.f, py = 0.f, pz = 0.f, raw_opacity = 0.f;
    float4 raw_rot = make_float4(0.f, 0.f, 0.f, 0.f);
    float2 raw_scales = make_float2(0.f, 0.f);
    bool kept = true;
    if (i < P) {
        px = means3D[3 * i]; py = means3D[3 * i + 1]; pz = means3D[3 * i + 2];
        raw_opacity = opacities[i];
        if (!transMat_precomp) { raw_rot = reinterpret_cast<const float4*>(rotations)[i]; raw_scales = reinterpret_cast<const float2*>(scales)[i]; }
        if (mask) kept = mask[i] != 0;
    }
    float4 half_b[6];
    if (kLdsSH) {
        const float* vw = f.view;
        s_skip[tid] = !(i < P && kept && ((vw[2] * px + vw[6] * py) + vw[10] * pz) + vw[14] > kNear);
        __syncthreads();
        float4 half_a[6];
        sh_half_load(shs, base, P, 0, tid, s_skip, half_a);
        sh_half_load(shs, base, P, 1, tid, s_skip, half_b);
        sh_half_store(s_sh, tid, half_a);
        __syncthreads();
    }
    const bool in_range = i < P;
    if (!kLdsSH && !in_range) return;
    int32_t out_radius = 0;
    uint32_t out_tiles = 0, out_key = kCulledKey;
    uint2 out_rect = make_uint2(0u, 0u);
    uint8_t out_clamped = 0;
    float4 q0 = make_float4(0, 0, 0, 0), q1 = q0, q2 = q0, q3 = q0, q4 = q0;

    const float* v = f.view;
    const float vx = ((v[0] * px + v[4] * py) + v[8] * pz) + v[12];
    const float vy = ((v[1] * px + v[5] * py) + v[9] * pz) + v[13];
    const float vz = ((v[2] * px + v[6] * py) + v[10] * pz) + v[14];
    bool alive = in_range && vz > kNear && kept;
    bool need_sh = false;
    float sdx = 0.f, sdy = 0.f, sdz = 0.f, slen = 1.f, sradius = 0.f;
    if (alive) {
        float Tm[9], nrm[3];
        if (transMat_precomp) {
#pragma unroll
            for (int k = 0; k < 9; ++k) Tm[k] = transMat_precomp[9 * (size_t)i + k];
            nrm[0] = 0.f; nrm[1] = 0.f; nrm[2] = 1.f;
        } else {
            float B[12], R[9];
            build_B(f.proj, f.W, f.H, B);
            float qn;
            quat_to_R(activate_rotation(raw_rot, f.activations, qn), R);
            const float2 s = activate_scales(raw_scales, f.activations);
            splat_transform(B, px, py, pz, R, f.scale_modifier * s.x, f.scale_modifier * s.y, Tm);
            const float nx = R[2], ny = R[5], nz = R[8];
            nrm[0] = (v[0] * nx + v[4] * ny) + v[8] * nz;
            nrm[1] = (v[1] * nx + v[5] * ny) + v[9] * nz;
            nrm[2] = (v[2] * nx + v[6] * ny) + v[10] * nz;
        }
        const float cosv = -((vx * nrm[0] + vy * nrm[1]) + vz * nrm[2]);
        alive = cosv != 0.f;
        const float mult = cosv > 0.f ? 1.f : -1.f;
        nrm[0] *= mult; nrm[1] *= mult; nrm[2] *= mult;

        const float* Tu = Tm; const float* Tv = Tm + 3; const float* Tw = Tm + 6;
        const float cutoff = bbox_cutoff((f.activations & SR_ACT_SIGMOID_OPACITY) ? sigmoidf(raw_opacity) : raw_opacity);
        const SplatBox box = splat_box(Tm, cutoff);
        alive = alive && (box.dist != 0.f);
        if (alive) {
            const float cx = box.cx, cy = box.cy, ex = box.ex, ey = box.ey;
#if SR_RADIUS_FILTER_FLOOR
            const float radius = ceilf(fmaxf(fmaxf(ex, ey), cutoff * kFilterSize));
#else
            const float radius = ceilf(fmaxf(ex, ey));
#endif
            int minx = (int)((cx - radius) * f.inv_tile_w), miny = (int)((cy - radius) * f.inv_tile_h);
            int maxx = (int)((cx + radius + (float)(f.tile_w - 1)) * f.inv_tile_w);
            int maxy = (int)((cy + radius + (float)(f.tile_h - 1)) * f.inv_tile_h);
            minx = min(f.tiles_x, max(0, minx)); maxx = min(f.tiles_x, max(0, maxx));
            miny = min(f.tiles_y, max(0, miny)); maxy = min(f.tiles_y, max(0, maxy));
            const int area = (maxx - minx) * (maxy - miny);
            if (area > 0) {
                float rgb[3] = {0.f, 0.f, 0.f};
                if (colors_precomp && f.colors != 9) {
                    const float* c = colors_precomp + (size_t)f.colors * i;
                    rgb[0] = c[0]; rgb[1] = c[1]; rgb[2] = c[2];
                } else {
                    float dx = px - f.campos[0], dy = py - f.campos[1], dz = pz - f.campos[2];
                    const float len = sqrtf((dx * dx + dy * dy) + dz * dz);
                    dx /= len; dy /= len; dz /= len;
                    if (kLdsSH) {
                        need_sh = true; sdx = dx; sdy = dy; sdz = dz; slen = len; sradius = radius;
                    } else {
                        float J[9];
                        sh_to_rgb(f.sh_degree, shs + (size_t)i * f.sh_coeffs * 3, dx, dy, dz, rgb, out_clamped);
                        if (f.sh_jac) {
                            sh_dir_jacobian(f.sh_degree, shs + (size_t)i * f.sh_coeffs * 3, dx, dy, dz, len, J);
#pragma unroll
                            for (int k = 0; k < 9; ++k) f.sh_jac[9 * (size_t)i + k] = J[k];
                        }
                    }
                }
                out_radius = (int32_t)radius;
                out_tiles = (uint32_t)area;
                out_rect = make_uint2((uint32_t)minx | ((uint32_t)miny << 16), (uint32_t)(maxx - minx) | ((uint32_t)(maxy - miny) << 16));
                out_key = __float_as_uint(vz);
                q0 = make_float4(Tu[0], Tu[1], Tu[2], Tv[0]);
                q1 = make_float4(Tv[1], Tv[2], Tw[0], Tw[1]);
                q2 = make_float4(Tw[2], cx, cy, (f.activations & SR_ACT_SIGMOID_OPACITY) ? sigmoidf(raw_opacity) : raw_opacity);
                q3 = make_float4(nrm[0], nrm[1], nrm[2], rgb[0]);
                q4 = make_float4(rgb[1], rgb[2], vz, radius);
            }
        }
    }
    if (kLdsSH) {
        const float* row = s_sh + tid * kShHalfStride;
        float res[3] = {0.f, 0.f, 0.f}, dd[9];
        const bool want_jac = f.sh_jac != nullptr;
        if (need_sh) {
            sh_to_rgb_lo(f.sh_degree, row, sdx, sdy, sdz, res);
            if (want_jac) sh_dir_jacobian_lo(f.sh_degree, row, sdx, sdy, sdz, dd);
        }
        __syncthreads();
        sh_half_store(s_sh, tid, half_b);
        __syncthreads();
        float J[9] = {0.f, 0.f, 0.f, 0.f, 0.f, 0.f, 0.f, 0.f, 0.f};
        if (need_sh) {
            float rgb[3];
            sh_to_rgb_hi(f.sh_degree, row, sdx, sdy, sdz, res, rgb, out_clamped);
            if (want_jac) sh_dir_jacobian_hi(f.sh_degree, row, sdx, sdy, sdz, slen, dd, J);
            q3.w = rgb[0];
            q4 = make_float4(rgb[1], rgb[2], q4.z, sradius);
        }
        __syncthreads();
        float4* s_rec = reinterpret_cast<float4*>(s_sh);
        float* s_jac = s_sh + kPreBlock * kRecFloats;
        s_skip[tid] = out_tiles == 0u;
        s_rec[tid * kRecQuads + 0] = q0; s_rec[tid * kRecQuads + 1] = q1; s_rec[tid * kRecQuads + 2] = q2; s_rec[tid * kRecQuads + 3] = q3;
        s_rec[tid * kRecQuads + 4] = q4;
        if (want_jac) {
#pragma unroll
            for (int k = 0; k < 9; ++k) s_jac[tid * 9 + k] = J[k];
        }
        __syncthreads();
        {
            const int nrows = min(kPreBlock, P - base);
            float4* dst = recs + (size_t)base * kRecQuads;
            for (int fq = tid; fq < nrows * kRecQuads; fq += kPreBlock) {
                const int c0 = fq & ~7, r0 = c0 / kRecQuads, r1 = min((c0 + 7) / kRecQuads, nrows - 1);
                if (!(s_skip[r0] & s_skip[min(r0 + 1, r1)] & s_skip[r1])) dst[fq] = s_rec[fq];
            }
            if (want_jac) {
                float* jd = f.sh_jac + (size_t)base * 9;
                const int nf = nrows * 9, nq = nf / 4;
                for (int fq = tid; fq < nq; fq += kPreBlock) {
                    const int f0 = (fq & ~7) * 4, r0 = f0 / 9, r1 = min((f0 + 31) / 9, nrows - 1);
                    bool dead = true;
                    for (int r = r0; r <= r1; ++r) dead = dead && s_skip[r];
                    if (!dead) reinterpret_cast<float4*>(jd)[fq] = reinterpret_cast<const float4*>(s_jac)[fq];
                }
                for (int fk = nq * 4 + tid; fk < nf; fk += kPreBlock) jd[fk] = s_jac[fk];
            }
        }
        if (!in_range) return;
        radii[i] = out_radius; tiles_touched[i] = out_tiles; rect[i] = out_rect; depth_keys[i] = out_key; clamped[i] = out_clamped;
        return;
    }
    radii[i] = out_radius;
    tiles_touched[i] = out_tiles;
    rect[i] = out_rect;
    depth_keys[i] = out_key;
    clamped[i] = out_clamped;
    float4* rec = recs + (size_t)i * kRecQuads;
    rec[0] = q0; rec[1] = q1; rec[2] = q2; rec[3] = q3; rec[4] = q4;
}

template <bool kLdsSH, int NC>
__global__ __launch_bounds__(kPreBlock) void preprocess_backward_kernel(
    int P, FrameDev f, const float* __restrict__ means3D, const float* __restrict__ scales,
    const float* __restrict__ rotations, const float* __restrict__ shs, const float* __restrict__ transMat_precomp,
    const int32_t* __restrict__ radii, const uint8_t* __restrict__ clamped, const float4* __restrict__ recs,
    const float4* __restrict__ inst_grads, const uint8_t* __restrict__ written, const uint32_t* __restrict__ tiles_touched,
    SrGradients out) {
    __shared__ __attribute__((aligned(16))) float s_sh[kLdsSH ? kPreBlock * kShLdsStride : 4];
    const int tid = threadIdx.x, base = blockIdx.x * kPreBlock;
    const int i = base + tid;
    const int M = f.sh_coeffs;
    if (i < P) {
        float g_means3D[3] = {0, 0, 0}, g_scales[2] = {0, 0}, g_rot[4] = {0, 0, 0, 0}, g_m2d[2] = {0, 0};
        float dT[9] = {0, 0, 0, 0, 0, 0, 0, 0, 0}, dTr[9] = {0, 0, 0, 0, 0, 0, 0, 0, 0}, g_col[9] = {0, 0, 0, 0, 0, 0, 0, 0, 0}, g_opa = 0.f;
        const bool vis = radii[i] > 0 && !(f.overflow && *f.overflow);
        float* dsh_g = (!kLdsSH && out.dL_dsh) ? out.dL_dsh + (size_t)i * M * 3 : nullptr;
        float* row = s_sh + tid * kShLdsStride;
        if (vis) {
            const float px = means3D[3 * i], py = means3D[3 * i + 1], pz = means3D[3 * i + 2];
            float act_opacity = 1.f;
            if (SR_TIGHTBBOX || (f.activations & SR_ACT_SIGMOID_OPACITY)) act_opacity = reinterpret_cast<const float*>(recs)[(size_t)i * kRecFloats + 11];
            float Tm[9];
            float qn = 1.f;
            float4 q = make_float4(1.f, 0.f, 0.f, 0.f);
            float R[9] = {1.f, 0.f, 0.f, 0.f, 1.f, 0.f, 0.f, 0.f, 1.f};
            float2 sc = make_float2(1.f, 1.f);
            if (transMat_precomp) {
#pragma unroll
                for (int k = 0; k < 9; ++k) Tm[k] = transMat_precomp[9 * (size_t)i + k];
            } else {
                float Bf[12];
                build_B(f.proj, f.W, f.H, Bf);
                q = load_rotation(rotations, i, f.activations, qn);
                quat_to_R(q, R);
                sc = load_scales(scales, i, f.activations);
                splat_transform(Bf, px, py, pz, R, f.scale_modifier * sc.x, f.scale_modifier * sc.y, Tm);
            }
            const SplatBox box = splat_box(Tm, bbox_cutoff(act_opacity));
            float4 g0, g1, g2, g3, g4, g5;
            {
                constexpr int kGQ = NC == 9 ? kGradQuads + 1 : kGradQuads;
                float4 g[kGQ];
#pragma unroll
                for (int k = 0; k < kGQ; ++k) g[k] = make_float4(0.f, 0.f, 0.f, 0.f);
                const uint32_t first = first_index(f, (uint32_t)i), cnt = tiles_touched[i];
                constexpr int kTrip = 4;
                const uint32_t end = first + cnt;
                auto load_flags = [&](uint32_t e, uint8_t (&fl)[kTrip]) {
#pragma unroll
                    for (int t = 0; t < kTrip; ++t) fl[t] = e + t < end ? written[e + t] : (uint8_t)0;
                };
                uint8_t fl[kTrip], fn[kTrip] = {0, 0, 0, 0};
                load_flags(first, fl);
                for (uint32_t e = first; e < end; e += kTrip) {
                    if (e + kTrip < end) load_flags(e + kTrip, fn);
                    float4 a[kTrip][kGQ];
#pragma unroll
                    for (int t = 0; t < kTrip; ++t) {
                        const float4* gr = inst_grads + (size_t)(e + t) * kGQ;
#pragma unroll
                        for (int k = 0; k < kGQ; ++k) a[t][k] = fl[t] ? gr[k] : make_float4(0.f, 0.f, 0.f, 0.f);
                    }
#pragma unroll
                    for (int t = 0; t < kTrip; ++t) {
                        if (fl[t]) {
#pragma unroll
                            for (int k = 0; k < kGQ; ++k) { g[k].x += a[t][k].x; g[k].y += a[t][k].y; g[k].z += a[t][k].z; g[k].w += a[t][k].w; }
                        }
                        fl[t] = fn[t];
                    }
                }
                g0 = g[0]; g1 = g[1]; g2 = g[2]; g3 = g[3]; g4 = g[4]; g5 = g[5];
                if (NC == 9) { g_col[6] = g[kGQ - 1].x; g_col[7] = g[kGQ - 1].y; g_col[8] = g[kGQ - 1].z; }
            }
            const float Tu[3] = {Tm[0], Tm[1], Tm[2]}, Tv[3] = {Tm[3], Tm[4], Tm[5]}, Tw[3] = {Tm[6], Tm[7], Tm[8]};
            {
                const float cx = fminf(fmaxf(box.cx, 0.f), (float)(f.W - 1)), cy = fminf(fmaxf(box.cy, 0.f), (float)(f.H - 1));
                const float Tuc[3] = {Tu[0] - cx * Tw[0], Tu[1] - cx * Tw[1], Tu[2] - cx * Tw[2]};
                const float Tvc[3] = {Tv[0] - cy * Tw[0], Tv[1] - cy * Tw[1], Tv[2] - cy * Tw[2]};
                const float S0[3] = {g0.x, g0.y, g0.z}, Sx[3] = {g0.w, g1.x, g1.y}, Sy[3] = {g1.z, g1.w, g2.x}, Z[3] = {g2.y, g2.z, g2.w};
#pragma unroll
                for (int c = 0; c < 3; ++c) {
                    const int c1 = (c + 1) % 3, c2 = (c + 2) % 3;
                    dT[0 + c] = (Tvc[c1] * S0[c2] - Tvc[c2] * S0[c1]) - (Tw[c1] * Sy[c2] - Tw[c2] * Sy[c1]);
                    dT[3 + c] = (S0[c1] * Tuc[c2] - S0[c2] * Tuc[c1]) - (Sx[c1] * Tw[c2] - Sx[c2] * Tw[c1]);
                    dT[6 + c] = (Tuc[c1] * Sy[c2] - Tuc[c2] * Sy[c1]) - (Tvc[c1] * Sx[c2] - Tvc[c2] * Sx[c1]) + Z[c];
                }
#pragma unroll
                for (int c = 0; c < 3; ++c) dT[6 + c] = (dT[6 + c] - cx * dT[0 + c]) - cy * dT[3 + c];
            }
            const float gx2 = g3.x, gy2 = g3.y;
            g_opa = g3.z;
            if (f.activations & SR_ACT_SIGMOID_OPACITY) { const float o = act_opacity; g_opa *= o * (1.f - o); }
            const float gn[3] = {g3.w, g4.x, g4.y};
            g_col[0] = g4.z; g_col[1] = g4.w; g_col[2] = g5.x;
            if (NC >= 6) { g_col[3] = g5.y; g_col[4] = g5.z; g_col[5] = g5.w; }
#if SR_PROXY_DEPTH_VIEW_Z
            const float depth_c = ((f.view[2] * px + f.view[6] * py) + f.view[10] * pz) + f.view[14];
#else
            const float depth_c = Tw[2];
#endif
            g_m2d[0] = dT[2] * depth_c * 0.5f * (float)f.bw_W;
            g_m2d[1] = dT[5] * depth_c * 0.5f * (float)f.bw_H;
#pragma unroll
            for (int k = 0; k < 9; ++k) dTr[k] = dT[k];
            if (gx2 != 0.f || gy2 != 0.f) {
                const float t[3] = {9.f, 9.f, -1.f};
                const float d = (t[0] * Tw[0] * Tw[0] + t[1] * Tw[1] * Tw[1]) + t[2] * Tw[2] * Tw[2];
                float fv[3], dLdd = 0.f;
#pragma unroll
                for (int c = 0; c < 3; ++c) { fv[c] = t[c] / d; dLdd += (gx2 * Tu[c] * Tw[c] + gy2 * Tv[c] * Tw[c]) * fv[c]; }
                dLdd *= (-1.f / d);
#pragma unroll
                for (int c = 0; c < 3; ++c) {
                    dT[0 + c] += gx2 * fv[c] * Tw[c];
                    dT[3 + c] += gy2 * fv[c] * Tw[c];
                    dT[6 + c] += gx2 * fv[c] * Tu[c] + gy2 * fv[c] * Tv[c] + dLdd * (t[c] * Tw[c] * 2.f);
                }
            }
            if (!transMat_precomp) {
                float B[12];
                build_B(f.proj, f.bw_W, f.bw_H, B);
                float dL0[3], dL1[3];
#pragma unroll
                for (int k = 0; k < 3; ++k) {
                    dL0[k] = B[0 + k] * dT[0] + B[4 + k] * dT[3] + B[8 + k] * dT[6];
                    dL1[k] = B[0 + k] * dT[1] + B[4 + k] * dT[4] + B[8 + k] * dT[7];
                    g_means3D[k] = B[0 + k] * dT[2] + B[4 + k] * dT[5] + B[8 + k] * dT[8];
                }
                const float* v = f.view;
                float dtn[3] = {v[0] * gn[0] + v[1] * gn[1] + v[2] * gn[2], v[4] * gn[0] + v[5] * gn[1] + v[6] * gn[2],
                                v[8] * gn[0] + v[9] * gn[1] + v[10] * gn[2]};
                const float vx = ((v[0] * px + v[4] * py) + v[8] * pz) + v[12];
                const float vy = ((v[1] * px + v[5] * py) + v[9] * pz) + v[13];
                const float vz = ((v[2] * px + v[6] * py) + v[10] * pz) + v[14];
                const float nx = R[2], ny = R[5], nz = R[8];
                const float n0 = (v[0] * nx + v[4] * ny) + v[8] * nz;
                const float n1 = (v[1] * nx + v[5] * ny) + v[9] * nz;
                const float n2 = (v[2] * nx + v[6] * ny) + v[10] * nz;
                const float cosv = -((vx * n0 + vy * n1) + vz * n2);
                const float mult = cosv > 0.f ? 1.f : -1.f;
                dtn[0] *= mult; dtn[1] *= mult; dtn[2] *= mult;
                float G[9];
#pragma unroll
                for (int k = 0; k < 3; ++k) { G[3 * k + 0] = dL0[k] * sc.x; G[3 * k + 1] = dL1[k] * sc.y; G[3 * k + 2] = dtn[k]; }
                g_scales[0] = dL0[0] * R[0] + dL0[1] * R[3] + dL0[2] * R[6];
                g_scales[1] = dL1[0] * R[1] + dL1[1] * R[4] + dL1[2] * R[7];
                const float r = q.x, x = q.y, y = q.z, z = q.w;
                g_rot[0] = 2.f * (-z * G[1] + y * G[2] + z * G[3] - x * G[5] - y * G[6] + x * G[7]);
                g_rot[1] = 2.f * (y * G[1] + z * G[2] + y * G[3] - 2.f * x * G[4] - r * G[5] + z * G[6] + r * G[7] - 2.f * x * G[8]);
                g_rot[2] = 2.f * (-2.f * y * G[0] + x * G[1] + r * G[2] + x * G[3] + z * G[5] - r * G[6] + z * G[7] - 2.f * y * G[8]);
                g_rot[3] = 2.f * (-2.f * z * G[0] - r * G[1] + x * G[2] + r * G[3] - 2.f * z * G[4] + y * G[5] + x * G[6] + y * G[7]);
                if (f.activations & SR_ACT_EXP_SCALES) { g_scales[0] *= sc.x; g_scales[1] *= sc.y; }
                if (f.activations & SR_ACT_NORMALIZE_ROTATIONS) {
                    const float qg = ((q.x * g_rot[0] + q.y * g_rot[1]) + q.z * g_rot[2]) + q.w * g_rot[3];
                    g_rot[0] = (g_rot[0] - q.x * qg) / qn; g_rot[1] = (g_rot[1] - q.y * qg) / qn;
                    g_rot[2] = (g_rot[2] - q.z * qg) / qn; g_rot[3] = (g_rot[3] - q.w * qg) / qn;
                }
            }
            if (shs) {
                const float ox = px - f.campos[0], oy = py - f.campos[1], oz = pz - f.campos[2];
                const float len = sqrtf((ox * ox + oy * oy) + oz * oz);
                const float x = ox / len, y = oy / len, z = oz / len;
                const uint8_t cl = clamped[i];
                const float gc[3] = {(cl & 1) ? 0.f : g_col[0], (cl & 2) ? 0.f : g_col[1], (cl & 4) ? 0.f : g_col[2]};
                g_col[0] = gc[0]; g_col[1] = gc[1]; g_col[2] = gc[2];
                if (kLdsSH) { if (out.dL_dsh) sh_basis_adjoint(f.sh_degree, M, row, x, y, z, gc); }
                else if (dsh_g) sh_basis_adjoint(f.sh_degree, M, dsh_g, x, y, z, gc);
                const float* J = f.sh_jac + 9 * (size_t)i;
#pragma unroll
                for (int k = 0; k < 3; ++k) g_means3D[k] += (gc[0] * J[k] + gc[1] * J[3 + k]) + gc[2] * J[6 + k];
            }
        } else if (shs) {
            if (kLdsSH) {
#pragma unroll
                for (int k = 0; k < kShRowFloats / 4; ++k) reinterpret_cast<float4*>(row)[k] = make_float4(0.f, 0.f, 0.f, 0.f);
            } else if (dsh_g) {
                for (int k = 0; k < M * 3; ++k) dsh_g[k] = 0.f;
            }
        }
        if (out.dL_dmeans3D) { out.dL_dmeans3D[3 * (size_t)i] = g_means3D[0]; out.dL_dmeans3D[3 * (size_t)i + 1] = g_means3D[1]; out.dL_dmeans3D[3 * (size_t)i + 2] = g_means3D[2]; }
        if (out.dL_dmeans2D) { out.dL_dmeans2D[3 * (size_t)i] = g_m2d[0]; out.dL_dmeans2D[3 * (size_t)i + 1] = g_m2d[1]; out.dL_dmeans2D[3 * (size_t)i + 2] = 0.f; }
        if (out.dL_dscales) {
            if ((reinterpret_cast<uintptr_t>(out.dL_dscales) & 7u) == 0) reinterpret_cast<float2*>(out.dL_dscales)[i] = make_float2(g_scales[0], g_scales[1]);
            else { out.dL_dscales[2 * (size_t)i] = g_scales[0]; out.dL_dscales[2 * (size_t)i + 1] = g_scales[1]; }
        }
        if (out.dL_drotations) { reinterpret_cast<float4*>(out.dL_drotations)[i] = make_float4(g_rot[0], g_rot[1], g_rot[2], g_rot[3]); }
        if (out.dL_dopacity) out.dL_dopacity[i] = g_opa;
        if (out.dL_dcolors) {
            if (NC == 9) {
#pragma unroll
                for (int c = 0; c < 6; ++c) out.dL_dcolors[6 * (size_t)i + c] = g_col[3 + c];
            } else {
#pragma unroll
                for (int c = 0; c < NC; ++c) out.dL_dcolors[NC * (size_t)i + c] = g_col[c];
            }
        }
        if (out.dL_dtransMat) {
#pragma unroll
            for (int k = 0; k < 9; ++k) out.dL_dtransMat[9 * (size_t)i + k] = transMat_precomp ? dT[k] : dTr[k];
        }
    }
    if (kLdsSH && out.dL_dsh) {
        __syncthreads();
        sh_rows_from_lds(out.dL_dsh, base, P, s_sh, tid);
    }
}

__global__ __launch_bounds__(256) void color_gradient_kernel(int P, const int32_t* __restrict__ radii, const uint8_t* __restrict__ clamped,
                                                             const float4* __restrict__ recs, const float4* __restrict__ inst_grads,
                                                             const uint8_t* __restrict__ written, const uint32_t* __restrict__ tiles_touched,
                                                             FrameDev f, int mask_clamped, float* __restrict__ dL_dcolors) {
    const int i = blockIdx.x * 256 + threadIdx.x;
    if (i >= P) return;
    float c0 = 0.f, c1 = 0.f, c2 = 0.f;
    if (radii[i] > 0 && !(f.overflow && *f.overflow)) {
        const uint32_t first = first_index(f, (uint32_t)i), end = first + tiles_touched[i];
        constexpr int kTrip = 4;
        auto load_flags = [&](uint32_t e, uint8_t (&fl)[kTrip]) {
#pragma unroll
            for (int t = 0; t < kTrip; ++t) fl[t] = e + t < end ? written[e + t] : (uint8_t)0;
        };
        uint8_t fl[kTrip], fn[kTrip] = {0, 0, 0, 0};
        load_flags(first, fl);
        for (uint32_t e = first; e < end; e += kTrip) {
            if (e + kTrip < end) load_flags(e + kTrip, fn);
            float4 a4[kTrip]; float a5[kTrip];
#pragma unroll
            for (int t = 0; t < kTrip; ++t) {
                const float4* gr = inst_grads + (size_t)(e + t) * kGradQuads;
                a4[t] = fl[t] ? gr[4] : make_float4(0.f, 0.f, 0.f, 0.f);
                a5[t] = fl[t] ? gr[5].x : 0.f;
            }
#pragma unroll
            for (int t = 0; t < kTrip; ++t) {
                if (fl[t]) { c0 += a4[t].z; c1 += a4[t].w; c2 += a5[t]; }
                fl[t] = fn[t];
            }
        }
        if (mask_clamped) { const uint8_t cl = clamped[i]; if (cl & 1) c0 = 0.f; if (cl & 2) c1 = 0.f; if (cl & 4) c2 = 0.f; }
    }
    dL_dcolors[3 * (size_t)i] = c0; dL_dcolors[3 * (size_t)i + 1] = c1; dL_dcolors[3 * (size_t)i + 2] = c2;
}

__device__ __forceinline__ void sh_basis(int deg, float x, float y, float z, float b[16]) {
#pragma unroll
    for (int k = 0; k < 16; ++k) b[k] = 0.f;
    b[0] = kSH_C0;
    if (deg > 0) {
        b[1] = -kSH_C1 * y; b[2] = kSH_C1 * z; b[3] = -kSH_C1 * x;
        if (deg > 1) {
            const float xx = x * x, yy = y * y, zz = z * z, xy = x * y, yz = y * z, xz = x * z;
            b[4] = kSH_C2[0] * xy; b[5] = kSH_C2[1] * yz; b[6] = kSH_C2[2] * (2.f * zz - xx - yy);
            b[7] = kSH_C2[3] * xz; b[8] = kSH_C2[4] * (xx - yy);
            if (deg > 2) {
                b[9] = kSH_C3[0] * y * (3.f * xx - yy);
                b[10] = kSH_C3[1] * xy * z;
                b[11] = kSH_C3[2] * y * (4.f * zz - xx - yy);
                b[12] = kSH_C3[3] * z * (2.f * zz - 3.f * xx - 3.f * yy);
                b[13] = kSH_C3[4] * x * (4.f * zz - xx - yy);
                b[14] = kSH_C3[5] * z * (xx - yy);
                b[15] = kSH_C3[6] * x * (xx - 3.f * yy);
            }
        }
    }
}

template <bool kLdsSH>
__global__ __launch_bounds__(kPreBlock) void sh_gradient_expand_kernel(int P, int M, int deg, int V, const float* __restrict__ means3D,
                                                                  const float* __restrict__ campos, const float* __restrict__ gc,
                                                                  float* __restrict__ dL_dsh) {
    __shared__ __attribute__((aligned(16))) float s_sh[kLdsSH ? kPreBlock * kShLdsStride : 4];
    const int tid = threadIdx.x, base = blockIdx.x * kPreBlock;
    const int i = base + tid;
    if (i < P) {
        float acc[48];
#pragma unroll
        for (int k = 0; k < 48; ++k) acc[k] = 0.f;
        const float px = means3D[3 * (size_t)i], py = means3D[3 * (size_t)i + 1], pz = means3D[3 * (size_t)i + 2];
        for (int v = 0; v < V; ++v) {
            const float* g = gc + ((size_t)v * P + i) * 3;
            const float g0 = g[0], g1 = g[1], g2 = g[2];
            if (g0 == 0.f && g1 == 0.f && g2 == 0.f) continue;
            const float ox = px - campos[3 * v], oy = py - campos[3 * v + 1], oz = pz - campos[3 * v + 2];
            const float len = sqrtf((ox * ox + oy * oy) + oz * oz);
            float b[16];
            sh_basis(deg, ox / len, oy / len, oz / len, b);
#pragma unroll
            for (int k = 0; k < 16; ++k) { acc[3 * k] += b[k] * g0; acc[3 * k + 1] += b[k] * g1; acc[3 * k + 2] += b[k] * g2; }
        }
        if (kLdsSH) {
            float4* row = reinterpret_cast<float4*>(s_sh + tid * kShLdsStride);
#pragma unroll
            for (int k = 0; k < kShRowFloats / 4; ++k) row[k] = make_float4(acc[4 * k], acc[4 * k + 1], acc[4 * k + 2], acc[4 * k + 3]);
        } else {
            float* row = dL_dsh + (size_t)i * M * 3;
#pragma unroll
            for (int k = 0; k < 48; ++k) { if (k < M * 3) row[k] = acc[k]; }
            for (int k = 48; k < M * 3; ++k) row[k] = 0.f;
        }
    }
    if (kLdsSH) {
        __syncthreads();
        sh_rows_from_lds(dL_dsh, base, P, s_sh, tid);
    }
}

__global__ void mark_visible_kernel(int P, const float* __restrict__ means3D, const float* __restrict__ view,
                                    uint8_t* __restrict__ present) {
    const int i = blockIdx.x * blockDim.x + threadIdx.x;
    if (i >= P) return;
    const float vz = ((view[2] * means3D[3 * i] + view[6] * means3D[3 * i + 1]) + view[10] * means3D[3 * i + 2]) + view[14];
    present[i] = vz > kNear ? 1 : 0;
}

static bool aligned16(const void* p) { return (reinterpret_cast<uintptr_t>(p) & 15u) == 0; }

hipError_t launch_preprocess_forward(int P, const FrameDev& f, const SrGaussians& g, float4* recs, uint32_t* depth_keys,
                                     uint32_t* tiles_touched, uint2* rect, uint8_t* clamped, int32_t* radii, hipStream_t s) {
    if (P == 0) return hipSuccess;
    const dim3 grid((P + kPreBlock - 1) / kPreBlock), block(kPreBlock);
    if (g.shs && g.sh_coeffs == 16 && aligned16(g.shs))
        hipLaunchKernelGGL(preprocess_forward_kernel<true>, grid, block, 0, s, P, f, g.means3D, g.opacities, g.scales,
                           g.rotations, g.shs, g.colors_precomp, g.transMat_precomp, g.mask, recs, depth_keys, tiles_touched, rect, clamped, radii);
    else
        hipLaunchKernelGGL(preprocess_forward_kernel<false>, grid, block, 0, s, P, f, g.means3D, g.opacities, g.scales,
                           g.rotations, g.shs, g.colors_precomp, g.transMat_precomp, g.mask, recs, depth_keys, tiles_touched, rect, clamped, radii);
    return hipGetLastError();
}

hipError_t launch_preprocess_backward(int P, const FrameDev& f, const SrGaussians& g, const int32_t* radii,
                                      const uint8_t* clamped, const float4* recs, const float4* inst_grads, const uint8_t* written,
                                      const uint32_t* tiles_touched, const SrGradients& out, hipStream_t s) {
    if (P == 0) return hipSuccess;
    const dim3 grid((P + kPreBlock - 1) / kPreBlock), block(kPreBlock);
    if (f.colors == 9 && g.sh_coeffs == 16 && aligned16(g.shs) && (!out.dL_dsh || aligned16(out.dL_dsh)))
        hipLaunchKernelGGL((preprocess_backward_kernel<true, 9>), grid, block, 0, s, P, f, g.means3D, g.scales, g.rotations, g.shs,
                           g.transMat_precomp, radii, clamped, recs, inst_grads, written, tiles_touched, out);
    else if (f.colors == 9)
        hipLaunchKernelGGL((preprocess_backward_kernel<false, 9>), grid, block, 0, s, P, f, g.means3D, g.scales, g.rotations, g.shs,
                           g.transMat_precomp, radii, clamped, recs, inst_grads, written, tiles_touched, out);
    else if (f.colors == 6)
        hipLaunchKernelGGL((preprocess_backward_kernel<false, 6>), grid, block, 0, s, P, f, g.means3D, g.scales, g.rotations, g.shs,
                           g.transMat_precomp, radii, clamped, recs, inst_grads, written, tiles_touched, out);
    else if (g.shs && g.sh_coeffs == 16 && aligned16(g.shs) && (!out.dL_dsh || aligned16(out.dL_dsh)))
        hipLaunchKernelGGL((preprocess_backward_kernel<true, 3>), grid, block, 0, s, P, f, g.means3D, g.scales, g.rotations, g.shs,
                           g.transMat_precomp, radii, clamped, recs, inst_grads, written, tiles_touched, out);
    else
        hipLaunchKernelGGL((preprocess_backward_kernel<false, 3>), grid, block, 0, s, P, f, g.means3D, g.scales, g.rotations, g.shs,
                           g.transMat_precomp, radii, clamped, recs, inst_grads, written, tiles_touched, out);
    return hipGetLastError();
}

hipError_t launch_sh_gradient_expand(int P, int M, int deg, int V, const float* means3D, const float* campos, const float* gc,
                                     float* dL_dsh, hipStream_t s) {
    if (P == 0) return hipSuccess;
    const dim3 grid((P + kPreBlock - 1) / kPreBlock), block(kPreBlock);
    if (M == 16 && aligned16(dL_dsh))
        hipLaunchKernelGGL(sh_gradient_expand_kernel<true>, grid, block, 0, s, P, M, deg, V, means3D, campos, gc, dL_dsh);
    else
        hipLaunchKernelGGL(sh_gradient_expand_kernel<false>, grid, block, 0, s, P, M, deg, V, means3D, campos, gc, dL_dsh);
    return hipGetLastError();
}

hipError_t launch_color_gradients(int P, const FrameDev& f, const int32_t* radii, const uint8_t* clamped, const float4* recs, const float4* inst_grads,
                                  const uint8_t* written, const uint32_t* tiles_touched, bool mask_clamped, float* dL_dcolors, hipStream_t s) {
    if (P == 0) return hipSuccess;
    hipLaunchKernelGGL(color_gradient_kernel, dim3((P + 255) / 256), dim3(256), 0, s, P, radii, clamped, recs, inst_grads, written, tiles_touched,
                       f, mask_clamped ? 1 : 0, dL_dcolors);
    return hipGetLastError();
}

hipError_t launch_mark_visible(int P, const float* means3D, const float* view, uint8_t* present, hipStream_t s) {
    if (P == 0) return hipSuccess;
    hipLaunchKernelGGL(mark_visible_kernel, dim3((P + 255) / 256), dim3(256), 0, s, P, means3D, view, present);
    return hipGetLastError();
}

}
```

streetunveiler_amd/csrc/radix_sort.hip:

```cpp
#include <cstdlib>
#include "launch.h"

namespace sr {

constexpr int kRsThreads = 256;
constexpr int kRsItems = 8;
constexpr int kRsTile = kRsThreads * kRsItems;
static_assert(kRsTile == kScanTile, "first_index() divides by the scan's block size");
constexpr int kSortItemsBig = 16;
constexpr uint32_t kSortBigFrom = 2u << 20;
constexpr int kRsMaxBins = 256;
constexpr uint32_t kSortRideFrom = 1u << 20;

constexpr uint32_t kDropKey = kCulledKey;
template <int kSortItems>
__global__ __launch_bounds__(kRsThreads) void rs_hist_kernel(const uint32_t* __restrict__ keys, uint32_t n_host, const uint32_t* __restrict__ n_dev, int drop,
                                                             int shift, int bits, uint32_t* __restrict__ hist, int nblocks) {
    constexpr int kSortTile = kRsThreads * kSortItems;
    __shared__ uint32_t s_h[kRsThreads / 64][kRsMaxBins];
    const int tid = threadIdx.x, bins = 1 << bits, w = tid >> 6;
    const uint32_t mask = (uint32_t)bins - 1u;
    const uint32_t n = n_dev ? min(*n_dev, n_host) : n_host;
    const uint32_t base = blockIdx.x * (uint32_t)kSortTile;
    if (base >= n) return;
    for (int k = tid; k < (kRsThreads / 64) * kRsMaxBins; k += kRsThreads) (&s_h[0][0])[k] = 0;
    uint32_t key[kSortItems];
#pragma unroll
    for (int i = 0; i < kSortItems; ++i) { const uint32_t idx = base + (uint32_t)(i * kRsThreads + tid); key[i] = idx < n ? keys[idx] : kDropKey; }
    __syncthreads();
#pragma unroll
    for (int i = 0; i < kSortItems; ++i) {
        const uint32_t idx = base + (uint32_t)(i * kRsThreads + tid);
        if (idx < n && !(drop && key[i] == kDropKey)) atomicAdd(&s_h[w][(key[i] >> shift) & mask], 1u);
    }
    __syncthreads();
    if (tid < bins) hist[(size_t)tid * nblocks + blockIdx.x] = (s_h[0][tid] + s_h[1][tid]) + (s_h[2][tid] + s_h[3][tid]);
}

constexpr uint32_t kOneSweepFrom = 1u << 18;
constexpr uint32_t kSwInclusive = 1u << 28, kSwValue = (1u << 28) - 1u;
template <int kSortItems>
__global__ __launch_bounds__(kRsThreads) void rs_hist_all_kernel(const uint32_t* __restrict__ keys, uint32_t n, int drop, uint32_t* __restrict__ ghist) {
    constexpr int kSortTile = kRsThreads * kSortItems;
    __shared__ uint32_t s_h[kRsThreads / 64][4][kRsMaxBins];
    const int tid = threadIdx.x, w = tid >> 6;
    const uint32_t base = blockIdx.x * (uint32_t)kSortTile;
    for (int k = tid; k < (kRsThreads / 64) * 4 * kRsMaxBins; k += kRsThreads) (&s_h[0][0][0])[k] = 0;
    __syncthreads();
#pragma unroll
    for (int i = 0; i < kSortItems; ++i) {
        const uint32_t idx = base + (uint32_t)(i * kRsThreads + tid);
        if (idx < n) {
            const uint32_t key = keys[idx];
            if (!(drop && key == kDropKey)) {
                atomicAdd(&s_h[w][0][key & 255u], 1u); atomicAdd(&s_h[w][1][(key >> 8) & 255u], 1u);
                atomicAdd(&s_h[w][2][(key >> 16) & 255u], 1u); atomicAdd(&s_h[w][3][key >> 24], 1u);
            }
        }
    }
    __syncthreads();
#pragma unroll
    for (int p = 0; p < 4; ++p) {
        const uint32_t c = (s_h[0][p][tid] + s_h[1][p][tid]) + (s_h[2][p][tid] + s_h[3][p][tid]);
        if (c) atomicAdd(&ghist[p * kRsMaxBins + tid], c);
    }
}

__global__ __launch_bounds__(kRsThreads) void rs_scan_rows_kernel(uint32_t* __restrict__ hist, int stride, const uint32_t* __restrict__ n_dev, uint32_t n_host,
                                                                  int items_per_block, uint32_t* __restrict__ row_total) {
    __shared__ uint32_t s_w[kRsThreads / 64];
    __shared__ uint32_t s_carry;
    const uint32_t n = n_dev ? min(*n_dev, n_host) : n_host;
    const int nblocks = (int)((n + (uint32_t)items_per_block - 1) / (uint32_t)items_per_block);
    uint32_t* row = hist + (size_t)blockIdx.x * stride;
    const int tid = threadIdx.x, lane = tid & 63, w = tid >> 6;
    if (tid == 0) s_carry = 0;
    __syncthreads();
    for (int c = 0; c < nblocks; c += kRsThreads) {
        const int i = c + tid;
        const uint32_t x = i < nblocks ? row[i] : 0u;
        uint32_t incl = wave_inclusive_scan(x);
        if (lane == 63) s_w[w] = incl;
        __syncthreads();
        uint32_t wbase = 0;
        for (int k = 0; k < w; ++k) wbase += s_w[k];
        const uint32_t carry = s_carry;
        if (i < nblocks) row[i] = carry + wbase + incl - x;
        __syncthreads();
        if (tid == kRsThreads - 1) s_carry = carry + wbase + incl;
        __syncthreads();
    }
    if (tid == 0) row_total[blockIdx.x] = s_carry;
}

__device__ __forceinline__ uint32_t pack_rect(uint2 r, int bx, int by) {
    return (r.x & 0xFFFFu) | ((r.y & 0xFFFFu) << bx) | ((r.x >> 16) << (2 * bx)) | ((r.y >> 16) << (2 * bx + by));
}
__device__ __forceinline__ uint2 unpack_rect(uint32_t w, int bx, int by) {
    const uint32_t mx = (1u << bx) - 1u, my = (1u << by) - 1u;
    return make_uint2((w & mx) | (((w >> (2 * bx)) & my) << 16), ((w >> bx) & mx) | ((w >> (2 * bx + by)) << 16));
}

template <int kBits, bool kAtomicRank, int kSortItems, bool kWide, bool kOneSweep = false>
__global__ __launch_bounds__(kRsThreads) void rs_scatter_kernel(const uint32_t* __restrict__ keys_in, const uint32_t* __restrict__ vals_in,
                                                                uint32_t* __restrict__ keys_out, uint32_t* __restrict__ vals_out,
                                                                uint32_t n_host, const uint32_t* __restrict__ n_dev, int drop, int shift, int bits_rt,
                                                                const uint32_t* __restrict__ hist,
                                                                const uint32_t* __restrict__ row_total, int nblocks,
                                                                const uint2* __restrict__ aux_src, uint2* __restrict__ aux_out,
                                                                const uint32_t* __restrict__ ride_in, uint32_t* __restrict__ ride_out, int bx, int by,
                                                                uint32_t* __restrict__ sw_status = nullptr, uint32_t* __restrict__ sw_ticket = nullptr, uint32_t sw_tag = 0) {
    constexpr int kSortTile = kRsThreads * kSortItems;
    __shared__ uint32_t s_bid;
    __shared__ uint32_t s_run[kRsThreads / 64][kRsMaxBins];
    __shared__ uint32_t s_lstart[kRsMaxBins];
    __shared__ uint32_t s_gbase[kRsMaxBins];
    __shared__ uint32_t s_wsum[kRsThreads / 64];
    __shared__ uint32_t s_live;
    static_assert(kRsThreads / 64 == 4, "s_live sums four wave totals");
    __shared__ uint32_t s_key[kSortTile], s_val[kSortTile];
    const int bits = kBits ? kBits : bits_rt;
    const int tid = threadIdx.x, lane = tid & 63, w = tid >> 6, bins = 1 << bits;
    const uint32_t mask = (uint32_t)bins - 1u;
    const uint32_t n = n_dev ? min(*n_dev, n_host) : n_host;
    if (kOneSweep) {
        if (tid == 0) s_bid = atomicAdd(sw_ticket, 1u);
        __syncthreads();
    }
    const uint32_t bid = kOneSweep ? s_bid : blockIdx.x;
    const uint32_t tile_base = bid * (uint32_t)kSortTile;
    if (tile_base >= n) return;
    for (int b = tid; b < (kRsThreads / 64) * kRsMaxBins; b += kRsThreads) (&s_run[0][0])[b] = 0;
    __syncthreads();
    const uint32_t wbase = tile_base + (uint32_t)w * (64 * kSortItems);
    uint32_t key[kSortItems], val[kSortItems], ride[kWide ? kSortItems : 1], slot[kWide ? kSortItems : 1];
#pragma unroll
    for (int i = 0; i < kSortItems; ++i) {
        const uint32_t idx = wbase + (uint32_t)(i * 64 + lane);
        key[i] = kDropKey; val[i] = 0;
        if constexpr (kWide) ride[i] = 0;
        if (idx < n) {
            key[i] = keys_in[idx];
            val[i] = vals_in ? vals_in[idx] : idx;
            if constexpr (kWide) ride[i] = ride_in ? ride_in[idx] : pack_rect(aux_src[idx], bx, by);
            if (!(drop && key[i] == kDropKey)) atomicAdd(&s_run[w][(key[i] >> shift) & mask], 1u);
        }
    }
    __syncthreads();
    {
        uint32_t tot = 0;
        if (tid < bins) {
#pragma unroll
            for (int k = 0; k < kRsThreads / 64; ++k) tot += s_run[k][tid];
        }
        uint32_t incl = wave_inclusive_scan(tot);
        if (lane == 63) s_wsum[w] = incl;
        __syncthreads();
        uint32_t off = incl - tot;
        for (int k = 0; k < w; ++k) off += s_wsum[k];
        if (tid == 0) s_live = (s_wsum[0] + s_wsum[1]) + (s_wsum[2] + s_wsum[3]);
        const uint32_t rt = tid < bins ? row_total[tid] : 0u;
        uint32_t rincl = wave_inclusive_scan(rt);
        __syncthreads();
        if (lane == 63) s_wsum[w] = rincl;
        __syncthreads();
        uint32_t bin_base = rincl - rt;
        for (int k = 0; k < w; ++k) bin_base += s_wsum[k];
        uint32_t before = 0;
        if (kOneSweep) {
            if (tid < bins) {
                uint32_t* mine = sw_status + (size_t)bid * kRsMaxBins + tid;
                __hip_atomic_store(mine, sw_tag | (bid == 0 ? kSwInclusive : 0u) | tot, __ATOMIC_RELAXED, __HIP_MEMORY_SCOPE_AGENT);
                if (bid > 0) {
                    for (int p = (int)bid - 1; p >= 0; --p) {
                        uint32_t v;
                        while ((((v = __hip_atomic_load(sw_status + (size_t)p * kRsMaxBins + tid, __ATOMIC_RELAXED, __HIP_MEMORY_SCOPE_AGENT)) >> 29) << 29) != sw_tag)
                            __builtin_amdgcn_s_sleep(1);
                        before += v & kSwValue;
                        if (v & kSwInclusive) break;
                    }
                    __hip_atomic_store(mine, sw_tag | kSwInclusive | (before + tot), __ATOMIC_RELAXED, __HIP_MEMORY_SCOPE_AGENT);
                }
            }
        } else if (tid < bins) {
            before = hist[(size_t)tid * nblocks + blockIdx.x];
        }
        if (tid < bins) {
            s_lstart[tid] = off;
            s_gbase[tid] = bin_base + before;
            uint32_t run = off;
#pragma unroll
            for (int k = 0; k < kRsThreads / 64; ++k) { const uint32_t c = s_run[k][tid]; s_run[k][tid] = run; run += c; }
        }
    }
    __syncthreads();
#pragma unroll
    for (int i = 0; i < kSortItems; ++i) {
        const uint32_t idx = wbase + (uint32_t)(i * 64 + lane);
        const bool live = idx < n && !(drop && key[i] == kDropKey);
        const uint32_t d = (key[i] >> shift) & mask;
        const uint32_t pos = take_run_slot<kAtomicRank>(s_run[w], d, live, bits);
        if (live) { s_key[pos] = key[i]; s_val[pos] = val[i]; }
        if constexpr (kWide) slot[i] = pos;
    }
    __syncthreads();
    const uint32_t count = s_live;
    uint32_t dest[kWide ? kSortItems : 1];
#pragma unroll
    for (int i = 0; i < kSortItems; ++i) {
        const uint32_t li = (uint32_t)(i * kRsThreads + tid);
        if (li < count) {
            const uint32_t k = s_key[li];
            const uint32_t d = (k >> shift) & mask;
            const uint32_t g = s_gbase[d] + (li - s_lstart[d]);
            const uint32_t v = s_val[li];
            if constexpr (kWide) dest[i] = g;
            keys_out[g] = k;
            vals_out[g] = v;
            if (!kWide && aux_out) aux_out[g] = aux_src[v];
        }
    }
    if constexpr (kWide) {
        __syncthreads();
#pragma unroll
        for (int i = 0; i < kSortItems; ++i)
            if (wbase + (uint32_t)(i * 64 + lane) < n && !(drop && key[i] == kDropKey)) s_val[slot[i]] = ride[i];
        __syncthreads();
#pragma unroll
        for (int i = 0; i < kSortItems; ++i) {
            const uint32_t li = (uint32_t)(i * kRsThreads + tid);
            if (li < count) {
                if (ride_out) ride_out[dest[i]] = s_val[li];
                else aux_out[dest[i]] = unpack_rect(s_val[li], bx, by);
            }
        }
    }
}

__global__ __launch_bounds__(kRsThreads) void scan_blocks_kernel(const uint32_t* __restrict__ counts, uint32_t n, uint32_t* __restrict__ out,
                                                                 uint32_t* __restrict__ block_total) {
    __shared__ uint32_t s_w[kRsThreads / 64], s_nz[kRsThreads / 64];
    const int tid = threadIdx.x, lane = tid & 63, w = tid >> 6;
    const uint32_t base = blockIdx.x * (uint32_t)kRsTile + (uint32_t)tid * kRsItems;
    uint32_t c[kRsItems];
    if (base + kRsItems <= n) {
        const uint4 c0 = reinterpret_cast<const uint4*>(counts + base)[0], c1 = reinterpret_cast<const uint4*>(counts + base)[1];
        c[0] = c0.x; c[1] = c0.y; c[2] = c0.z; c[3] = c0.w; c[4] = c1.x; c[5] = c1.y; c[6] = c1.z; c[7] = c1.w;
    } else {
#pragma unroll
        for (int i = 0; i < kRsItems; ++i) c[i] = base + i < n ? counts[base + i] : 0u;
    }
    uint32_t v[kRsItems], sum = 0, nz = 0;
#pragma unroll
    for (int i = 0; i < kRsItems; ++i) {
        v[i] = sum;
        sum += c[i];
        nz += c[i] != 0u;
    }
    uint32_t incl = wave_inclusive_scan(sum);
    const uint32_t nz_incl = wave_inclusive_scan(nz);
    if (lane == 63) { s_w[w] = incl; s_nz[w] = nz_incl; }
    __syncthreads();
    uint32_t off = incl - sum;
    for (int k = 0; k < w; ++k) off += s_w[k];
    if (base + kRsItems <= n) {
        reinterpret_cast<uint4*>(out + base)[0] = make_uint4(off + v[0], off + v[1], off + v[2], off + v[3]);
        reinterpret_cast<uint4*>(out + base)[1] = make_uint4(off + v[4], off + v[5], off + v[6], off + v[7]);
    } else {
#pragma unroll
        for (int i = 0; i < kRsItems; ++i) if (base + i < n) out[base + i] = off + v[i];
    }
    if (tid == kRsThreads - 1) {
        block_total[blockIdx.x] = off + sum;
        uint32_t n_vis = 0;
        for (int k = 0; k < kRsThreads / 64; ++k) n_vis += s_nz[k];
        block_total[gridDim.x + 2 + blockIdx.x] = n_vis;
    }
}

__global__ __launch_bounds__(kRsThreads) void scan_totals_kernel(uint32_t* __restrict__ block_total, int nblocks, uint32_t* __restrict__ total_host) {
    __shared__ uint32_t s_w[kRsThreads / 64];
    __shared__ uint32_t s_carry, s_vis;
    const int tid = threadIdx.x, lane = tid & 63, w = tid >> 6;
    if (tid == 0) { s_carry = 0; s_vis = 0; }
    __syncthreads();
    uint32_t vis_mine = 0;
    for (int c = 0; c < nblocks; c += kRsThreads) {
        const int i = c + tid;
        const uint32_t x = i < nblocks ? block_total[i] : 0u;
        vis_mine += i < nblocks ? block_total[nblocks + 2 + i] : 0u;
        uint32_t incl = wave_inclusive_scan(x);
        if (lane == 63) s_w[w] = incl;
        __syncthreads();
        uint32_t wb = 0;
        for (int k = 0; k < w; ++k) wb += s_w[k];
        const uint32_t carry = s_carry;
        if (i < nblocks) block_total[i] = carry + wb + incl - x;
        __syncthreads();
        if (tid == kRsThreads - 1) s_carry = carry + wb + incl;
        __syncthreads();
    }
    {
        const uint32_t tot = wave_inclusive_scan(vis_mine);
        if (lane == 63 && tot) atomicAdd(&s_vis, tot);
        __syncthreads();
    }
    if (tid == 0) { block_total[nblocks] = s_carry; block_total[nblocks + 1] = s_vis; if (total_host) { total_host[0] = s_carry; total_host[1] = s_vis; } }
}

__global__ __launch_bounds__(kRsThreads) void rank_selfcheck_kernel(uint32_t* __restrict__ result) {
    __shared__ uint32_t s_a[kRsThreads / 64][1024], s_b[kRsThreads / 64][1024], s_c[kRsThreads / 64][1024];
    __shared__ uint32_t s_dig[kRsThreads / 64][64];
    __shared__ uint32_t s_ok;
    const int tid = threadIdx.x, lane = tid & 63, w = tid >> 6;
    for (int i = tid; i < (kRsThreads / 64) * 1024; i += kRsThreads) { (&s_a[0][0])[i] = 0; (&s_b[0][0])[i] = 0; (&s_c[0][0])[i] = 0; }
    if (tid == 0) s_ok = 3u;
    __syncthreads();
    uint32_t ok = 3u;
    for (int round = 0; round < 64; ++round) {
        const uint32_t alphabets[8] = {1u, 2u, 3u, 16u, 64u, 256u, 700u, 1000u};
        const uint32_t bins = alphabets[round & 7];
        uint32_t h = (uint32_t)(round * 64 + lane) * 2654435761u + (uint32_t)w * 40503u;
        h ^= h >> 15; h *= 2246822519u; h ^= h >> 13;
        const uint32_t d = (round & 8) ? (h % bins) : ((h >> 3) % ((bins + 3u) / 4u));
        const bool live = (round & 16) ? lane < 37 : true;
        const uint32_t pa = take_run_slot<true>(s_a[w], d, live, 10);
        const uint32_t pb = take_run_slot<false>(s_b[w], d, live, 10);
        s_dig[w][lane] = live ? d : 0xFFFFFFFFu;
        __builtin_amdgcn_wave_barrier();
        uint32_t lower = 0, higher = 0;
        for (int k = 0; k < 64; ++k) { const uint32_t dk = s_dig[w][k]; lower += (k < lane && dk == d); higher += (k > lane && dk == d); }
        const uint32_t pc = s_c[w][d] + lower;
        __builtin_amdgcn_wave_barrier();
        if (live && higher == 0) s_c[w][d] = pc + 1u;
        __builtin_amdgcn_wave_barrier();
        if (live && pa != pc) ok &= ~1u;
        if (live && pb != pc) ok &= ~2u;
    }
    atomicAnd(&s_ok, ok);
    __syncthreads();
    if (tid == 0) *result = s_ok | 0x100u;
}
hipError_t launch_rank_selfcheck(uint32_t* result, hipStream_t s) {
    hipLaunchKernelGGL(rank_selfcheck_kernel, dim3(1), dim3(kRsThreads), 0, s, result);
    return hipGetLastError();
}

__global__ __launch_bounds__(kRsThreads) void lds_atomic_ranks_kernel(const uint32_t* __restrict__ digits, uint32_t* __restrict__ ranks, uint32_t n, int bins) {
    __shared__ uint32_t s_cnt[kRsThreads / 64][1024];
    const int tid = threadIdx.x, w = tid >> 6;
    for (int i = tid; i < (kRsThreads / 64) * 1024; i += kRsThreads) (&s_cnt[0][0])[i] = 0;
    __syncthreads();
    for (int it = 0; it < kRsItems; ++it) {
        const uint32_t idx = (blockIdx.x * (uint32_t)kRsItems + it) * kRsThreads + tid;
        if (idx < n) ranks[idx] = atomicAdd(&s_cnt[w][digits[idx] % (uint32_t)bins], 1u);
    }
}
hipError_t lds_atomic_ranks(const uint32_t* digits, uint32_t* ranks, uint32_t n, int bins, hipStream_t s) {
    if (n == 0) return hipSuccess;
    hipLaunchKernelGGL(lds_atomic_ranks_kernel, dim3((n + kRsTile - 1) / kRsTile), dim3(kRsThreads), 0, s, digits, ranks, n, bins);
    return hipGetLastError();
}

__global__ __launch_bounds__(kRsThreads) void rs_zero_words_kernel(uint32_t* __restrict__ p, uint32_t n) {
    for (uint32_t i = blockIdx.x * kRsThreads + threadIdx.x; i < n; i += gridDim.x * kRsThreads) p[i] = 0u;
}
static inline int rs_blocks(uint32_t n, int items = kRsItems) { return (int)((n + (uint32_t)(kRsThreads * items) - 1) / (uint32_t)(kRsThreads * items)); }
static inline int scan_blocks(uint32_t n) { return (int)((n + kRsTile - 1) / kRsTile); }

size_t radix_sort_temp_bytes(uint32_t n) {
    const size_t nb = (size_t)rs_blocks(n > 0 ? n : 1);
    return align_up((size_t)(n > 0 ? n : 1) * 4, 256) * 3 + align_up(nb * kRsMaxBins * 4, 256) + align_up(kRsMaxBins * 4 * 5 + 64, 256);
}

hipError_t radix_sort_pairs(const uint32_t* keys_in, const uint32_t* vals_in, uint32_t* keys_out, uint32_t* vals_out, uint32_t n,
                            int total_bits, void* temp, size_t temp_bytes, hipStream_t s, const uint2* aux_src, uint2* aux_out, RankMode rank_mode,
                            bool one_sweep, int rect_bx, int rect_by, const uint32_t* n_live) {
    if (n == 0) return hipSuccess;
    if (temp_bytes < radix_sort_temp_bytes(n) || (rank_mode != kRankAtomic && rank_mode != kRankBallot)) return hipErrorInvalidValue;
    int passes = (total_bits + 7) / 8;
    if (passes < 1) passes = 1;
    if (passes & 1) ++passes;
    const int nb8 = rs_blocks(n);
    char* t = static_cast<char*>(temp);
    uint32_t* tk = reinterpret_cast<uint32_t*>(t); t += align_up((size_t)n * 4, 256);
    uint32_t* tv = reinterpret_cast<uint32_t*>(t); t += align_up((size_t)n * 4, 256);
    uint32_t* tr = reinterpret_cast<uint32_t*>(t); t += align_up((size_t)n * 4, 256);
    const bool wide = aux_out && !vals_in && rect_bx > 0 && rect_by > 0 && 2 * (rect_bx + rect_by) <= 32 && passes >= 2 && n >= kSortRideFrom;
    uint32_t* hist = reinterpret_cast<uint32_t*>(t); t += align_up((size_t)nb8 * kRsMaxBins * 4, 256);
    uint32_t* row_total = reinterpret_cast<uint32_t*>(t);
    uint32_t* ghist = row_total + kRsMaxBins;
    uint32_t* tickets = ghist + 4 * kRsMaxBins;
    const uint32_t* ki = keys_in; const uint32_t* vi = vals_in;
    int shift = 0, left = total_bits;
    const bool sweep = one_sweep && total_bits == 32 && passes == 4 && n >= kOneSweepFrom && n <= kSwValue;
    if (sweep) {
        const size_t zero_bytes = (size_t)(reinterpret_cast<char*>(tickets + 16) - reinterpret_cast<char*>(hist));
        hipLaunchKernelGGL(rs_zero_words_kernel, dim3(256), dim3(kRsThreads), 0, s, hist, (uint32_t)(zero_bytes / 4));
        const bool bigh = n >= kSortBigFrom;
        if (bigh) hipLaunchKernelGGL(rs_hist_all_kernel<kSortItemsBig>, dim3(rs_blocks(n, kSortItemsBig)), dim3(kRsThreads), 0, s, keys_in, n, n_live ? 1 : 0, ghist);
        else hipLaunchKernelGGL(rs_hist_all_kernel<kRsItems>, dim3(nb8), dim3(kRsThreads), 0, s, keys_in, n, n_live ? 1 : 0, ghist);
    }
    for (int p = 0; p < passes; ++p) {
        const int remaining_passes = passes - p;
        int bits = left > 0 ? (left + remaining_passes - 1) / remaining_passes : 1;
        if (bits > 8) bits = 8;
        if (bits < 1) bits = 1;
        const bool last = p == passes - 1;
        uint32_t* ko = (p & 1) ? keys_out : tk;
        uint32_t* vo = (p & 1) ? vals_out : tv;
        const uint32_t* ri = p == 0 ? nullptr : ((p & 1) ? tr : reinterpret_cast<const uint32_t*>(aux_out));
        uint32_t* ro = last ? nullptr : ((p & 1) ? reinterpret_cast<uint32_t*>(aux_out) : tr);
        const bool big = bits == 8 && n >= kSortBigFrom;
        const int nb = big ? rs_blocks(n, kSortItemsBig) : nb8;
        const uint32_t* nd = (n_live && p > 0) ? n_live : nullptr;
        const int drop = (n_live && p == 0) ? 1 : 0;
        if (!sweep) {
            if (big) hipLaunchKernelGGL(rs_hist_kernel<kSortItemsBig>, dim3(nb), dim3(kRsThreads), 0, s, ki, n, nd, drop, shift, bits, hist, nb);
            else hipLaunchKernelGGL(rs_hist_kernel<kRsItems>, dim3(nb), dim3(kRsThreads), 0, s, ki, n, nd, drop, shift, bits, hist, nb);
            hipLaunchKernelGGL(rs_scan_rows_kernel, dim3(1 << bits), dim3(kRsThreads), 0, s, hist, nb, nd, n, kRsThreads * (big ? kSortItemsBig : kRsItems), row_total);
        }
#define SR_SCATTER_W(B, A, I, Wd) do { if (sweep && B == 8) hipLaunchKernelGGL((rs_scatter_kernel<B == 8 ? 8 : 0, A, I, Wd, B == 8>), dim3(nb), dim3(kRsThreads), 0, s, ki, vi, ko, vo, n, nd, drop, shift, bits, \
                                                 (const uint32_t*)nullptr, (const uint32_t*)(ghist + p * kRsMaxBins), nb, (Wd ? p == 0 : last) ? aux_src : nullptr, last ? aux_out : nullptr, ri, ro, rect_bx, rect_by, \
                                                 hist, tickets + p, (uint32_t)(p + 1) << 29);                                                                    \
                                   else hipLaunchKernelGGL((rs_scatter_kernel<B, A, I, Wd>), dim3(nb), dim3(kRsThreads), 0, s, ki, vi, ko, vo, n, nd, drop, shift, bits, (const uint32_t*)hist, \
                                                 (const uint32_t*)row_total, nb, (Wd ? p == 0 : last) ? aux_src : nullptr, last ? aux_out : nullptr, ri, ro, rect_bx, rect_by, (uint32_t*)nullptr, (uint32_t*)nullptr, 0u); } while (0)
#define SR_SCATTER_R(B, A, I) do { if (wide) SR_SCATTER_W(B, A, I, true); else SR_SCATTER_W(B, A, I, false); } while (0)
#define SR_SCATTER(B, I) do { if (rank_mode == kRankAtomic) SR_SCATTER_R(B, true, I); else SR_SCATTER_R(B, false, I); } while (0)
        switch (bits) {
            case 8: if (big) SR_SCATTER(8, kSortItemsBig); else SR_SCATTER(8, kRsItems); break;
            case 7: SR_SCATTER(7, kRsItems); break;
            case 6: SR_SCATTER(6, kRsItems); break;
            default: SR_SCATTER(0, kRsItems); break;
        }
#undef SR_SCATTER
#undef SR_SCATTER_R
#undef SR_SCATTER_W
        ki = ko; vi = vo;
        shift += bits; left -= bits;
    }
    return hipGetLastError();
}

size_t tile_count_scan_temp_bytes(uint32_t n) { return align_up((2 * (size_t)scan_blocks(n > 0 ? n : 1) + 2) * 4, 256); }

hipError_t tile_count_scan(const uint32_t* counts, uint32_t* out, uint32_t n, void* temp, size_t temp_bytes, uint32_t* total_host, hipStream_t s) {
    if (n == 0) return hipSuccess;
    if (temp_bytes < tile_count_scan_temp_bytes(n)) return hipErrorInvalidValue;
    const int nb = scan_blocks(n);
    uint32_t* totals = static_cast<uint32_t*>(temp);
    hipLaunchKernelGGL(scan_blocks_kernel, dim3(nb), dim3(kRsThreads), 0, s, counts, n, out, totals);
    hipLaunchKernelGGL(scan_totals_kernel, dim3(1), dim3(kRsThreads), 0, s, totals, nb, total_host);
    return hipGetLastError();
}

}
```

Measured before the change: 923.2 Msplats/s.

## Shrink depth-sort passes using visible key span bounds from preprocess

Preprocess now writes each wave's min and max depth key for visible Gaussians. The tile-count scan reduces these per-wave values into global key bounds. A new depth sort subtracts the minimum key and, when the span fits in 27 bits, sorts in three 9-bit passes instead of four 8-bit passes; otherwise it falls back to four 8-bit passes. The aim is to cut one full radix scatter and histogram pass over 3M keys. The cost is larger 512-bin histograms and scans, plus device-side branching on the bounds, while the kernel launch count stays the same.

```diff
diff --git a/streetunveiler_amd/csrc/api.hip b/streetunveiler_amd/csrc/api.hip
--- a/streetunveiler_amd/csrc/api.hip
+++ b/streetunveiler_amd/csrc/api.hip
@@ -124,11 +124,12 @@
 
 struct GeomLayout {
     size_t recs, depth_keys, tiles_touched, rect, clamped, sorted_keys, sorted_gid, rect_sorted, first, sh_jac, block_base, base_bytes,
-        counts, temp, temp_bytes, total;
+        counts, temp, temp_bytes, total, n;
 };
 GeomLayout geom_layout(int P) {
     GeomLayout L{};
     const size_t n = (size_t)(P > 0 ? P : 1);
+    L.n = n;
     Carver c;
     L.recs = c.take(n * kRecFloats * 4);
     L.depth_keys = c.take(n * 4);
@@ -164,12 +165,14 @@
     float* sh_jac;
     uint32_t* block_base; void* temp;
     uint32_t* counts;
+    uint2* wave_keys; uint2* block_keys; uint32_t* key_bounds;
 };
 GeomView geom_view(void* geom, const GeomLayout& L) {
     return GeomView{at<float4>(geom, L.recs), at<uint32_t>(geom, L.depth_keys), at<uint32_t>(geom, L.tiles_touched), at<uint2>(geom, L.rect),
                     at<uint8_t>(geom, L.clamped), at<uint32_t>(geom, L.sorted_keys), at<uint32_t>(geom, L.sorted_gid), at<uint2>(geom, L.rect_sorted),
                     at<uint32_t>(geom, L.first), at<float>(geom, L.sh_jac), at<uint32_t>(geom, L.block_base), at<void>(geom, L.temp),
-                    at<uint32_t>(geom, L.counts)};
+                    at<uint32_t>(geom, L.counts), at<uint2>(geom, L.temp), at<uint2>(geom, L.temp + depth_sort_block_keys_offset((uint32_t)L.n)),
+                    at<uint32_t>(geom, L.temp + depth_sort_key_bounds_offset((uint32_t)L.n))};
 }
 
 struct BinLayout {
@@ -395,7 +398,7 @@
     f.sh_jac = (frame->flags & SR_FLAG_FORWARD_ONLY) ? nullptr : G.sh_jac;
     {
         StageTimer t(SR_STAGE_PREPROCESS, s);
-        SR_HIP(launch_preprocess_forward(P, f, *g, G.recs, G.depth_keys, G.tiles_touched, G.rect, G.clamped, radii, s));
+        SR_HIP(launch_preprocess_forward(P, f, *g, G.recs, G.depth_keys, G.tiles_touched, G.rect, G.clamped, radii, G.wave_keys, s));
     }
     if (int rc = debug_sync(frame, s, "preprocess_forward")) return rc;
     RankMode sort_mode = kRankUnknown;
@@ -406,7 +409,7 @@
     if (pinned && (hipHostGetDevicePointer(reinterpret_cast<void**>(&pinned_dev), pinned, 0) != hipSuccess)) pinned_dev = nullptr;
     {
         StageTimer t(SR_STAGE_SCAN, s);
-        SR_HIP(run_tile_count_scan(P, G.tiles_touched, G.first, G.block_base, L.base_bytes, pinned_dev, s));
+        SR_HIP(run_tile_count_scan(P, G.tiles_touched, G.first, G.block_base, L.base_bytes, pinned_dev, G.wave_keys, G.block_keys, G.key_bounds, s));
     }
     if (int rc = debug_sync(frame, s, "emission_scan")) return rc;
     hipEvent_t copied = nullptr;
@@ -424,7 +427,7 @@
     {
         StageTimer t(SR_STAGE_DEPTH_SORT, s);
         SR_HIP(run_depth_sort(P, G.depth_keys, G.rect, G.sorted_keys, G.sorted_gid, G.rect_sorted, G.temp, L.temp_bytes, sort_mode,
-                              (frame->flags & SR_FLAG_ONE_SWEEP_SORT) != 0, f.tiles_x, f.tiles_y, G.counts + kCountVisible, s));
+                              (frame->flags & SR_FLAG_ONE_SWEEP_SORT) != 0, f.tiles_x, f.tiles_y, G.counts + kCountVisible, G.key_bounds, s));
     }
     if (!read_back) {
         *num_rendered_host = 0xFFFFFFFFu;
diff --git a/streetunveiler_amd/csrc/binning.hip b/streetunveiler_amd/csrc/binning.hip
--- a/streetunveiler_amd/csrc/binning.hip
+++ b/streetunveiler_amd/csrc/binning.hip
@@ -353,7 +353,7 @@
 
 size_t depth_sort_temp_bytes(int P) {
     const uint32_t n = (uint32_t)(P > 0 ? P : 1);
-    return align_up(radix_sort_temp_bytes(n), 256);
+    return align_up(depth_sort_pairs_temp_bytes(n), 256);
 }
 size_t tile_scan_temp_bytes(int P) { return tile_count_scan_temp_bytes((uint32_t)(P > 0 ? P : 1)); }
 
@@ -362,16 +362,17 @@
 
 hipError_t run_depth_sort(int P, const uint32_t* depth_keys, const uint2* rect, uint32_t* sorted_keys,
                           uint32_t* sorted_gid, uint2* rect_sorted, void* temp, size_t temp_bytes, RankMode rank_mode, bool one_sweep, int tiles_x,
-                          int tiles_y, const uint32_t* n_visible, hipStream_t s) {
+                          int tiles_y, const uint32_t* n_visible, const uint32_t* key_bounds, hipStream_t s) {
     if (P == 0) return hipSuccess;
     const int bx = 32 - __builtin_clz((unsigned)(tiles_x > 0 ? tiles_x : 1)), by = 32 - __builtin_clz((unsigned)(tiles_y > 0 ? tiles_y : 1));
-    return radix_sort_pairs(depth_keys, nullptr, sorted_keys, sorted_gid, (uint32_t)P, 32, temp, temp_bytes, s, rect, rect_sorted, rank_mode, one_sweep, bx, by, n_visible);
+    if (one_sweep) return radix_sort_pairs(depth_keys, nullptr, sorted_keys, sorted_gid, (uint32_t)P, 32, temp, temp_bytes, s, rect, rect_sorted, rank_mode, true, bx, by, n_visible);
+    return depth_sort_pairs(depth_keys, sorted_keys, sorted_gid, (uint32_t)P, temp, temp_bytes, s, rect, rect_sorted, rank_mode, bx, by, n_visible, key_bounds);
 }
 
 hipError_t run_tile_count_scan(int P, const uint32_t* tiles_touched, uint32_t* first, void* block_base, size_t base_bytes, uint32_t* total_host,
-                               hipStream_t s) {
+                               const uint2* wave_keys, uint2* block_keys, uint32_t* key_bounds, hipStream_t s) {
     if (P == 0) return hipSuccess;
-    return tile_count_scan(tiles_touched, first, (uint32_t)P, block_base, base_bytes, total_host, s);
+    return tile_count_scan(tiles_touched, first, (uint32_t)P, block_base, base_bytes, total_host, wave_keys, block_keys, key_bounds, s);
 }
 
 template <int AXIS, bool kAtomicRank, typename... Args>
diff --git a/streetunveiler_amd/csrc/common.h b/streetunveiler_amd/csrc/common.h
--- a/streetunveiler_amd/csrc/common.h
+++ b/streetunveiler_amd/csrc/common.h
@@ -65,6 +65,20 @@
     return (uint32_t)v;
 }
 
+__device__ __forceinline__ uint32_t wave_inclusive_max(uint32_t x) {
+    int v = (int)x;
+#define SR_DPP_MAX(ctrl, rows) v = (int)max((uint32_t)v, (uint32_t)__builtin_amdgcn_update_dpp(0, v, ctrl, rows, 0xf, true))
+    SR_DPP_MAX(0x111, 0xf); SR_DPP_MAX(0x112, 0xf); SR_DPP_MAX(0x114, 0xf); SR_DPP_MAX(0x118, 0xf); SR_DPP_MAX(0x142, 0xa); SR_DPP_MAX(0x143, 0xc);
+#undef SR_DPP_MAX
+    return (uint32_t)v;
+}
+
+constexpr int kSpanDigitBits = 9, kSpanBits = 3 * kSpanDigitBits;
+__device__ __forceinline__ bool span_fits(const uint32_t* __restrict__ bounds) {
+    const uint32_t kmin = bounds[0], kmax = bounds[1];
+    return kmax >= kmin && kmax - kmin < (1u << kSpanBits);
+}
+
 template <bool kAtomic>
 __device__ __forceinline__ uint32_t take_run_slot(uint32_t* run, uint32_t d, bool live, int bits) {
     uint32_t pos = 0;
diff --git a/streetunveiler_amd/csrc/launch.h b/streetunveiler_amd/csrc/launch.h
--- a/streetunveiler_amd/csrc/launch.h
+++ b/streetunveiler_amd/csrc/launch.h
@@ -26,7 +26,7 @@
 };
 
 hipError_t launch_preprocess_forward(int P, const FrameDev& f, const SrGaussians& g, float4* recs, uint32_t* depth_keys,
-                                     uint32_t* tiles_touched, uint2* rect, uint8_t* clamped, int32_t* radii, hipStream_t s);
+                                     uint32_t* tiles_touched, uint2* rect, uint8_t* clamped, int32_t* radii, uint2* wave_keys, hipStream_t s);
 hipError_t launch_preprocess_backward(int P, const FrameDev& f, const SrGaussians& g, const int32_t* radii,
                                       const uint8_t* clamped, const float4* recs, const float4* inst_grads, const uint8_t* written,
                                       const uint32_t* tiles_touched, const SrGradients& out, hipStream_t s);
@@ -40,8 +40,15 @@
 hipError_t radix_sort_pairs(const uint32_t* keys_in, const uint32_t* vals_in, uint32_t* keys_out, uint32_t* vals_out, uint32_t n,
                             int total_bits, void* temp, size_t temp_bytes, hipStream_t s, const uint2* aux_src, uint2* aux_out, RankMode rank_mode,
                             bool one_sweep, int rect_bx = 0, int rect_by = 0, const uint32_t* n_live = nullptr);
+size_t depth_sort_pairs_temp_bytes(uint32_t n);
+size_t depth_sort_key_bounds_offset(uint32_t n);
+size_t depth_sort_block_keys_offset(uint32_t n);
+hipError_t depth_sort_pairs(const uint32_t* keys_in, uint32_t* keys_out, uint32_t* vals_out, uint32_t n, void* temp, size_t temp_bytes, hipStream_t s,
+                            const uint2* aux_src, uint2* aux_out, RankMode rank_mode, int rect_bx, int rect_by, const uint32_t* n_live,
+                            const uint32_t* key_bounds);
 size_t tile_count_scan_temp_bytes(uint32_t n);
-hipError_t tile_count_scan(const uint32_t* counts, uint32_t* out, uint32_t n, void* temp, size_t temp_bytes, uint32_t* total_host, hipStream_t s);
+hipError_t tile_count_scan(const uint32_t* counts, uint32_t* out, uint32_t n, void* temp, size_t temp_bytes, uint32_t* total_host, const uint2* wave_keys,
+                           uint2* block_keys, uint32_t* key_bounds, hipStream_t s);
 hipError_t launch_rank_selfcheck(uint32_t* result, hipStream_t s);
 hipError_t lds_atomic_ranks(const uint32_t* digits, uint32_t* ranks, uint32_t n, int bins, hipStream_t s);
 
@@ -51,9 +58,9 @@
 size_t expand_y_hist_bytes(uint32_t D, int tiles_y);
 hipError_t run_depth_sort(int P, const uint32_t* depth_keys, const uint2* rect, uint32_t* sorted_keys,
                           uint32_t* sorted_gid, uint2* rect_sorted, void* temp, size_t temp_bytes, RankMode rank_mode, bool one_sweep, int tiles_x,
-                          int tiles_y, const uint32_t* n_visible, hipStream_t s);
+                          int tiles_y, const uint32_t* n_visible, const uint32_t* key_bounds, hipStream_t s);
 hipError_t run_tile_count_scan(int P, const uint32_t* tiles_touched, uint32_t* first, void* block_base, size_t base_bytes, uint32_t* total_host,
-                               hipStream_t s);
+                               const uint2* wave_keys, uint2* block_keys, uint32_t* key_bounds, hipStream_t s);
 hipError_t run_expand_columns(int P, int tiles_x, int n_tiles, const uint2* rect_sorted, const uint32_t* sorted_gid, uint2* columns,
                               uint32_t* n_columns, uint32_t* hist, uint32_t* row_total, uint32_t* tile_counts, RankMode rank_mode, const uint32_t* n_visible,
                               hipStream_t s);
diff --git a/streetunveiler_amd/csrc/preprocess.hip b/streetunveiler_amd/csrc/preprocess.hip
--- a/streetunveiler_amd/csrc/preprocess.hip
+++ b/streetunveiler_amd/csrc/preprocess.hip
@@ -306,7 +306,8 @@
     const float* __restrict__ scales, const float* __restrict__ rotations, const float* __restrict__ shs,
     const float* __restrict__ colors_precomp, const float* __restrict__ transMat_precomp,
     const uint8_t* __restrict__ mask, float4* __restrict__ recs, uint32_t* __restrict__ depth_keys,
-    uint32_t* __restrict__ tiles_touched, uint2* __restrict__ rect, uint8_t* __restrict__ clamped, int32_t* __restrict__ radii) {
+    uint32_t* __restrict__ tiles_touched, uint2* __restrict__ rect, uint8_t* __restrict__ clamped, int32_t* __restrict__ radii,
+    uint2* __restrict__ wave_keys) {
     constexpr int kK1LdsFloats = kPreBlock * (kShHalfStride > kRecFloats + 9 ? kShHalfStride : kRecFloats + 9);
     __shared__ __attribute__((aligned(16))) float s_sh[kLdsSH ? kK1LdsFloats : 4];
     __shared__ uint8_t s_skip[kLdsSH ? kPreBlock : 4];
@@ -334,7 +335,6 @@
         __syncthreads();
     }
     const bool in_range = i < P;
-    if (!kLdsSH && !in_range) return;
     int32_t out_radius = 0;
     uint32_t out_tiles = 0, out_key = kCulledKey;
     uint2 out_rect = make_uint2(0u, 0u);
@@ -421,6 +421,11 @@
             }
         }
     }
+    {
+        const uint32_t kmin = ~wave_inclusive_max(~out_key), kmax = wave_inclusive_max(out_tiles ? out_key : 0u);
+        static_assert(kPreBlock % 64 == 0, "wave w of the grid holds Gaussians 64 w .. 64 w + 63");
+        if ((tid & 63) == 63 && i - 63 < P) wave_keys[(uint32_t)i >> 6] = make_uint2(kmin, kmax);
+    }
     if (kLdsSH) {
         const float* row = s_sh + tid * kShHalfStride;
         float res[3] = {0.f, 0.f, 0.f}, dd[9];
@@ -474,6 +479,7 @@
         radii[i] = out_radius; tiles_touched[i] = out_tiles; rect[i] = out_rect; depth_keys[i] = out_key; clamped[i] = out_clamped;
         return;
     }
+    if (!in_range) return;
     radii[i] = out_radius;
     tiles_touched[i] = out_tiles;
     rect[i] = out_rect;
@@ -801,15 +807,15 @@
 static bool aligned16(const void* p) { return (reinterpret_cast<uintptr_t>(p) & 15u) == 0; }
 
 hipError_t launch_preprocess_forward(int P, const FrameDev& f, const SrGaussians& g, float4* recs, uint32_t* depth_keys,
-                                     uint32_t* tiles_touched, uint2* rect, uint8_t* clamped, int32_t* radii, hipStream_t s) {
+                                     uint32_t* tiles_touched, uint2* rect, uint8_t* clamped, int32_t* radii, uint2* wave_keys, hipStream_t s) {
     if (P == 0) return hipSuccess;
     const dim3 grid((P + kPreBlock - 1) / kPreBlock), block(kPreBlock);
     if (g.shs && g.sh_coeffs == 16 && aligned16(g.shs))
         hipLaunchKernelGGL(preprocess_forward_kernel<true>, grid, block, 0, s, P, f, g.means3D, g.opacities, g.scales,
-                           g.rotations, g.shs, g.colors_precomp, g.transMat_precomp, g.mask, recs, depth_keys, tiles_touched, rect, clamped, radii);
+                           g.rotations, g.shs, g.colors_precomp, g.transMat_precomp, g.mask, recs, depth_keys, tiles_touched, rect, clamped, radii, wave_keys);
     else
         hipLaunchKernelGGL(preprocess_forward_kernel<false>, grid, block, 0, s, P, f, g.means3D, g.opacities, g.scales,
-                           g.rotations, g.shs, g.colors_precomp, g.transMat_precomp, g.mask, recs, depth_keys, tiles_touched, rect, clamped, radii);
+                           g.rotations, g.shs, g.colors_precomp, g.transMat_precomp, g.mask, recs, depth_keys, tiles_touched, rect, clamped, radii, wave_keys);
     return hipGetLastError();
 }
 
diff --git a/streetunveiler_amd/csrc/radix_sort.hip b/streetunveiler_amd/csrc/radix_sort.hip
--- a/streetunveiler_amd/csrc/radix_sort.hip
+++ b/streetunveiler_amd/csrc/radix_sort.hip
@@ -10,20 +10,39 @@
 constexpr int kSortItemsBig = 16;
 constexpr uint32_t kSortBigFrom = 2u << 20;
 constexpr int kRsMaxBins = 256;
+constexpr int kSpanMaxBins = 1 << kSpanDigitBits;
+
+struct SpanArgs {
+    const uint32_t* bounds;
+    int pass;
+    uint32_t* tk; uint32_t* tv; uint32_t* tr;
+    uint32_t* ok; uint32_t* ov; uint2* oaux;
+};
+__device__ __forceinline__ bool span_out_is_temp(bool fits, int pass) { return fits ? pass == 1 : !(pass & 1); }
 constexpr uint32_t kSortRideFrom = 1u << 20;
 
 constexpr uint32_t kDropKey = kCulledKey;
-template <int kSortItems>
+template <int kSortItems, bool kSpan = false>
 __global__ __launch_bounds__(kRsThreads) void rs_hist_kernel(const uint32_t* __restrict__ keys, uint32_t n_host, const uint32_t* __restrict__ n_dev, int drop,
-                                                             int shift, int bits, uint32_t* __restrict__ hist, int nblocks) {
+                                                             int shift, int bits, uint32_t* __restrict__ hist, int nblocks, SpanArgs sp) {
     constexpr int kSortTile = kRsThreads * kSortItems;
-    __shared__ uint32_t s_h[kRsThreads / 64][kRsMaxBins];
+    constexpr int kBins = kSpan ? kSpanMaxBins : kRsMaxBins;
+    __shared__ uint32_t s_h[kRsThreads / 64][kBins];
+    uint32_t sub = 0;
+    if constexpr (kSpan) {
+        const bool fits = span_fits(sp.bounds);
+        if (fits && sp.pass == 3) return;
+        bits = fits ? kSpanDigitBits : 8;
+        shift = sp.pass * bits;
+        if (sp.pass > 0) keys = span_out_is_temp(fits, sp.pass - 1) ? sp.tk : sp.ok;
+        else if (fits) sub = sp.bounds[0];
+    }
     const int tid = threadIdx.x, bins = 1 << bits, w = tid >> 6;
     const uint32_t mask = (uint32_t)bins - 1u;
     const uint32_t n = n_dev ? min(*n_dev, n_host) : n_host;
     const uint32_t base = blockIdx.x * (uint32_t)kSortTile;
     if (base >= n) return;
-    for (int k = tid; k < (kRsThreads / 64) * kRsMaxBins; k += kRsThreads) (&s_h[0][0])[k] = 0;
+    for (int k = tid; k < (kRsThreads / 64) * kBins; k += kRsThreads) (&s_h[0][0])[k] = 0;
     uint32_t key[kSortItems];
 #pragma unroll
     for (int i = 0; i < kSortItems; ++i) { const uint32_t idx = base + (uint32_t)(i * kRsThreads + tid); key[i] = idx < n ? keys[idx] : kDropKey; }
@@ -31,10 +50,10 @@
 #pragma unroll
     for (int i = 0; i < kSortItems; ++i) {
         const uint32_t idx = base + (uint32_t)(i * kRsThreads + tid);
-        if (idx < n && !(drop && key[i] == kDropKey)) atomicAdd(&s_h[w][(key[i] >> shift) & mask], 1u);
-    }
-    __syncthreads();
-    if (tid < bins) hist[(size_t)tid * nblocks + blockIdx.x] = (s_h[0][tid] + s_h[1][tid]) + (s_h[2][tid] + s_h[3][tid]);
+        if (idx < n && !(drop && key[i] == kDropKey)) atomicAdd(&s_h[w][((key[i] - sub) >> shift) & mask], 1u);
+    }
+    __syncthreads();
+    for (int b = tid; b < bins; b += kRsThreads) hist[(size_t)b * nblocks + blockIdx.x] = (s_h[0][b] + s_h[1][b]) + (s_h[2][b] + s_h[3][b]);
 }
 
 constexpr uint32_t kOneSweepFrom = 1u << 18;
@@ -67,9 +86,14 @@
 }
 
 __global__ __launch_bounds__(kRsThreads) void rs_scan_rows_kernel(uint32_t* __restrict__ hist, int stride, const uint32_t* __restrict__ n_dev, uint32_t n_host,
-                                                                  int items_per_block, uint32_t* __restrict__ row_total) {
+                                                                  int items_per_block, uint32_t* __restrict__ row_total,
+                                                                  const uint32_t* __restrict__ span_bounds, int span_pass) {
     __shared__ uint32_t s_w[kRsThreads / 64];
     __shared__ uint32_t s_carry;
+    if (span_bounds) {
+        const bool fits = span_fits(span_bounds);
+        if (fits ? span_pass == 3 : (int)blockIdx.x >= kRsMaxBins) return;
+    }
     const uint32_t n = n_dev ? min(*n_dev, n_host) : n_host;
     const int nblocks = (int)((n + (uint32_t)items_per_block - 1) / (uint32_t)items_per_block);
     uint32_t* row = hist + (size_t)blockIdx.x * stride;
@@ -101,7 +125,7 @@
     return make_uint2((w & mx) | (((w >> (2 * bx)) & my) << 16), ((w >> bx) & mx) | ((w >> (2 * bx + by)) << 16));
 }
 
-template <int kBits, bool kAtomicRank, int kSortItems, bool kWide, bool kOneSweep = false>
+template <int kBits, bool kAtomicRank, int kSortItems, bool kWide, bool kOneSweep = false, bool kSpan = false>
 __global__ __launch_bounds__(kRsThreads) void rs_scatter_kernel(const uint32_t* __restrict__ keys_in, const uint32_t* __restrict__ vals_in,
                                                                 uint32_t* __restrict__ keys_out, uint32_t* __restrict__ vals_out,
                                                                 uint32_t n_host, const uint32_t* __restrict__ n_dev, int drop, int shift, int bits_rt,
@@ -109,17 +133,39 @@
                                                                 const uint32_t* __restrict__ row_total, int nblocks,
                                                                 const uint2* __restrict__ aux_src, uint2* __restrict__ aux_out,
                                                                 const uint32_t* __restrict__ ride_in, uint32_t* __restrict__ ride_out, int bx, int by,
-                                                                uint32_t* __restrict__ sw_status = nullptr, uint32_t* __restrict__ sw_ticket = nullptr, uint32_t sw_tag = 0) {
+                                                                uint32_t* __restrict__ sw_status, uint32_t* __restrict__ sw_ticket, uint32_t sw_tag, SpanArgs sp) {
     constexpr int kSortTile = kRsThreads * kSortItems;
+    constexpr int kBins = kSpan ? kSpanMaxBins : kRsMaxBins, kDig = kBins / kRsThreads;
+    static_assert(!(kSpan && kOneSweep), "the one-sweep passes stay on four 8-bit digits");
     __shared__ uint32_t s_bid;
-    __shared__ uint32_t s_run[kRsThreads / 64][kRsMaxBins];
-    __shared__ uint32_t s_lstart[kRsMaxBins];
-    __shared__ uint32_t s_gbase[kRsMaxBins];
+    __shared__ uint32_t s_run[kRsThreads / 64][kBins];
+    __shared__ uint32_t s_lstart[kBins];
+    __shared__ uint32_t s_gbase[kBins];
     __shared__ uint32_t s_wsum[kRsThreads / 64];
     __shared__ uint32_t s_live;
     static_assert(kRsThreads / 64 == 4, "s_live sums four wave totals");
     __shared__ uint32_t s_key[kSortTile], s_val[kSortTile];
-    const int bits = kBits ? kBits : bits_rt;
+    uint32_t sub = 0;
+    if constexpr (kSpan) {
+        const bool fits = span_fits(sp.bounds);
+        if (fits && sp.pass == 3) return;
+        bits_rt = fits ? kSpanDigitBits : 8;
+        shift = sp.pass * bits_rt;
+        const bool last = sp.pass == (fits ? 2 : 3);
+        if (sp.pass == 0) {
+            if (fits) sub = sp.bounds[0];
+        } else {
+            const bool in_temp = span_out_is_temp(fits, sp.pass - 1);
+            keys_in = in_temp ? sp.tk : sp.ok; vals_in = in_temp ? sp.tv : sp.ov;
+            ride_in = in_temp ? sp.tr : reinterpret_cast<const uint32_t*>(sp.oaux);
+        }
+        const bool out_temp = span_out_is_temp(fits, sp.pass);
+        keys_out = out_temp ? sp.tk : ((last && fits) ? nullptr : sp.ok); vals_out = out_temp ? sp.tv : sp.ov;
+        ride_out = last ? nullptr : (out_temp ? sp.tr : reinterpret_cast<uint32_t*>(sp.oaux));
+        aux_out = last ? sp.oaux : nullptr;
+        if (!kWide) ride_in = ride_out = nullptr;
+    }
+    const int bits = (kBits && !kSpan) ? kBits : bits_rt;
     const int tid = threadIdx.x, lane = tid & 63, w = tid >> 6, bins = 1 << bits;
     const uint32_t mask = (uint32_t)bins - 1u;
     const uint32_t n = n_dev ? min(*n_dev, n_host) : n_host;
@@ -130,7 +176,7 @@
     const uint32_t bid = kOneSweep ? s_bid : blockIdx.x;
     const uint32_t tile_base = bid * (uint32_t)kSortTile;
     if (tile_base >= n) return;
-    for (int b = tid; b < (kRsThreads / 64) * kRsMaxBins; b += kRsThreads) (&s_run[0][0])[b] = 0;
+    for (int b = tid; b < (kRsThreads / 64) * kBins; b += kRsThreads) (&s_run[0][0])[b] = 0;
     __syncthreads();
     const uint32_t wbase = tile_base + (uint32_t)w * (64 * kSortItems);
     uint32_t key[kSortItems], val[kSortItems], ride[kWide ? kSortItems : 1], slot[kWide ? kSortItems : 1];
@@ -141,6 +187,7 @@
         if constexpr (kWide) ride[i] = 0;
         if (idx < n) {
             key[i] = keys_in[idx];
+            if constexpr (kSpan) { if (key[i] != kDropKey) key[i] -= sub; }
             val[i] = vals_in ? vals_in[idx] : idx;
             if constexpr (kWide) ride[i] = ride_in ? ride_in[idx] : pack_rect(aux_src[idx], bx, by);
             if (!(drop && key[i] == kDropKey)) atomicAdd(&s_run[w][(key[i] >> shift) & mask], 1u);
@@ -148,49 +195,66 @@
     }
     __syncthreads();
     {
-        uint32_t tot = 0;
-        if (tid < bins) {
-#pragma unroll
-            for (int k = 0; k < kRsThreads / 64; ++k) tot += s_run[k][tid];
-        }
-        uint32_t incl = wave_inclusive_scan(tot);
+        uint32_t tot[kDig], sum = 0;
+#pragma unroll
+        for (int j = 0; j < kDig; ++j) {
+            const int d = tid * kDig + j;
+            tot[j] = 0;
+            if (d < bins) {
+#pragma unroll
+                for (int k = 0; k < kRsThreads / 64; ++k) tot[j] += s_run[k][d];
+            }
+            sum += tot[j];
+        }
+        uint32_t incl = wave_inclusive_scan(sum);
         if (lane == 63) s_wsum[w] = incl;
         __syncthreads();
-        uint32_t off = incl - tot;
+        uint32_t off = incl - sum;
         for (int k = 0; k < w; ++k) off += s_wsum[k];
         if (tid == 0) s_live = (s_wsum[0] + s_wsum[1]) + (s_wsum[2] + s_wsum[3]);
-        const uint32_t rt = tid < bins ? row_total[tid] : 0u;
-        uint32_t rincl = wave_inclusive_scan(rt);
+        uint32_t rt[kDig], rsum = 0;
+#pragma unroll
+        for (int j = 0; j < kDig; ++j) { const int d = tid * kDig + j; rt[j] = d < bins ? row_total[d] : 0u; rsum += rt[j]; }
+        uint32_t rincl = wave_inclusive_scan(rsum);
         __syncthreads();
         if (lane == 63) s_wsum[w] = rincl;
         __syncthreads();
-        uint32_t bin_base = rincl - rt;
+        uint32_t bin_base = rincl - rsum;
         for (int k = 0; k < w; ++k) bin_base += s_wsum[k];
-        uint32_t before = 0;
-        if (kOneSweep) {
+        uint32_t before[kDig];
+#pragma unroll
+        for (int j = 0; j < kDig; ++j) before[j] = 0;
+        if constexpr (kOneSweep) {
+            const uint32_t tot0 = tot[0];
             if (tid < bins) {
                 uint32_t* mine = sw_status + (size_t)bid * kRsMaxBins + tid;
-                __hip_atomic_store(mine, sw_tag | (bid == 0 ? kSwInclusive : 0u) | tot, __ATOMIC_RELAXED, __HIP_MEMORY_SCOPE_AGENT);
+                __hip_atomic_store(mine, sw_tag | (bid == 0 ? kSwInclusive : 0u) | tot0, __ATOMIC_RELAXED, __HIP_MEMORY_SCOPE_AGENT);
                 if (bid > 0) {
                     for (int p = (int)bid - 1; p >= 0; --p) {
                         uint32_t v;
                         while ((((v = __hip_atomic_load(sw_status + (size_t)p * kRsMaxBins + tid, __ATOMIC_RELAXED, __HIP_MEMORY_SCOPE_AGENT)) >> 29) << 29) != sw_tag)
                             __builtin_amdgcn_s_sleep(1);
-                        before += v & kSwValue;
+                        before[0] += v & kSwValue;
                         if (v & kSwInclusive) break;
                     }
-                    __hip_atomic_store(mine, sw_tag | kSwInclusive | (before + tot), __ATOMIC_RELAXED, __HIP_MEMORY_SCOPE_AGENT);
+                    __hip_atomic_store(mine, sw_tag | kSwInclusive | (before[0] + tot0), __ATOMIC_RELAXED, __HIP_MEMORY_SCOPE_AGENT);
                 }
             }
-        } else if (tid < bins) {
-            before = hist[(size_t)tid * nblocks + blockIdx.x];
-        }
-        if (tid < bins) {
-            s_lstart[tid] = off;
-            s_gbase[tid] = bin_base + before;
-            uint32_t run = off;
-#pragma unroll
-            for (int k = 0; k < kRsThreads / 64; ++k) { const uint32_t c = s_run[k][tid]; s_run[k][tid] = run; run += c; }
+        } else {
+#pragma unroll
+            for (int j = 0; j < kDig; ++j) { const int d = tid * kDig + j; if (d < bins) before[j] = hist[(size_t)d * nblocks + blockIdx.x]; }
+        }
+#pragma unroll
+        for (int j = 0; j < kDig; ++j) {
+            const int d = tid * kDig + j;
+            if (d < bins) {
+                s_lstart[d] = off;
+                s_gbase[d] = bin_base + before[j];
+                uint32_t run = off;
+#pragma unroll
+                for (int k = 0; k < kRsThreads / 64; ++k) { const uint32_t c = s_run[k][d]; s_run[k][d] = run; run += c; }
+            }
+            off += tot[j]; bin_base += rt[j];
         }
     }
     __syncthreads();
@@ -215,7 +279,7 @@
             const uint32_t g = s_gbase[d] + (li - s_lstart[d]);
             const uint32_t v = s_val[li];
             if constexpr (kWide) dest[i] = g;
-            keys_out[g] = k;
+            if (!kSpan || keys_out) keys_out[g] = k;
             vals_out[g] = v;
             if (!kWide && aux_out) aux_out[g] = aux_src[v];
         }
@@ -238,7 +302,8 @@
 }
 
 __global__ __launch_bounds__(kRsThreads) void scan_blocks_kernel(const uint32_t* __restrict__ counts, uint32_t n, uint32_t* __restrict__ out,
-                                                                 uint32_t* __restrict__ block_total) {
+                                                                 uint32_t* __restrict__ block_total, const uint2* __restrict__ wave_keys,
+                                                                 uint2* __restrict__ block_keys) {
     __shared__ uint32_t s_w[kRsThreads / 64], s_nz[kRsThreads / 64];
     const int tid = threadIdx.x, lane = tid & 63, w = tid >> 6;
     const uint32_t base = blockIdx.x * (uint32_t)kRsTile + (uint32_t)tid * kRsItems;
@@ -276,19 +341,29 @@
         for (int k = 0; k < kRsThreads / 64; ++k) n_vis += s_nz[k];
         block_total[gridDim.x + 2 + blockIdx.x] = n_vis;
     }
-}
-
-__global__ __launch_bounds__(kRsThreads) void scan_totals_kernel(uint32_t* __restrict__ block_total, int nblocks, uint32_t* __restrict__ total_host) {
+    if (wave_keys && w == 0) {
+        static_assert(kRsTile / 64 <= 64, "one wave folds the block's pairs");
+        const uint32_t wi = blockIdx.x * (uint32_t)(kRsTile / 64) + (uint32_t)lane, n_waves = (n + 63u) / 64u;
+        const uint2 k = (lane < kRsTile / 64 && wi < n_waves) ? wave_keys[wi] : make_uint2(0xFFFFFFFFu, 0u);
+        const uint32_t kmin = ~wave_inclusive_max(~k.x), kmax = wave_inclusive_max(k.y);
+        if (lane == 63) block_keys[blockIdx.x] = make_uint2(kmin, kmax);
+    }
+}
+
+__global__ __launch_bounds__(kRsThreads) void scan_totals_kernel(uint32_t* __restrict__ block_total, int nblocks, uint32_t* __restrict__ total_host,
+                                                                 const uint2* __restrict__ block_keys, uint32_t* __restrict__ key_bounds) {
     __shared__ uint32_t s_w[kRsThreads / 64];
-    __shared__ uint32_t s_carry, s_vis;
+    __shared__ uint32_t s_carry, s_vis, s_kmin, s_kmax;
     const int tid = threadIdx.x, lane = tid & 63, w = tid >> 6;
-    if (tid == 0) { s_carry = 0; s_vis = 0; }
+    if (tid == 0) { s_carry = 0; s_vis = 0; s_kmin = 0xFFFFFFFFu; s_kmax = 0u; }
     __syncthreads();
     uint32_t vis_mine = 0;
+    uint32_t kmin_mine = 0xFFFFFFFFu, kmax_mine = 0u;
     for (int c = 0; c < nblocks; c += kRsThreads) {
         const int i = c + tid;
         const uint32_t x = i < nblocks ? block_total[i] : 0u;
         vis_mine += i < nblocks ? block_total[nblocks + 2 + i] : 0u;
+        if (key_bounds && i < nblocks) { const uint2 k = block_keys[i]; kmin_mine = min(kmin_mine, k.x); kmax_mine = max(kmax_mine, k.y); }
         uint32_t incl = wave_inclusive_scan(x);
         if (lane == 63) s_w[w] = incl;
         __syncthreads();
@@ -303,8 +378,13 @@
     {
         const uint32_t tot = wave_inclusive_scan(vis_mine);
         if (lane == 63 && tot) atomicAdd(&s_vis, tot);
-        __syncthreads();
-    }
+        if (key_bounds) {
+            const uint32_t kmin = ~wave_inclusive_max(~kmin_mine), kmax = wave_inclusive_max(kmax_mine);
+            if (lane == 63) { atomicMin(&s_kmin, kmin); atomicMax(&s_kmax, kmax); }
+        }
+        __syncthreads();
+    }
+    if (tid == 0 && key_bounds) { key_bounds[0] = s_kmin; key_bounds[1] = s_kmax; }
     if (tid == 0) { block_total[nblocks] = s_carry; block_total[nblocks + 1] = s_vis; if (total_host) { total_host[0] = s_carry; total_host[1] = s_vis; } }
 }
 
@@ -416,15 +496,16 @@
         const uint32_t* nd = (n_live && p > 0) ? n_live : nullptr;
         const int drop = (n_live && p == 0) ? 1 : 0;
         if (!sweep) {
-            if (big) hipLaunchKernelGGL(rs_hist_kernel<kSortItemsBig>, dim3(nb), dim3(kRsThreads), 0, s, ki, n, nd, drop, shift, bits, hist, nb);
-            else hipLaunchKernelGGL(rs_hist_kernel<kRsItems>, dim3(nb), dim3(kRsThreads), 0, s, ki, n, nd, drop, shift, bits, hist, nb);
-            hipLaunchKernelGGL(rs_scan_rows_kernel, dim3(1 << bits), dim3(kRsThreads), 0, s, hist, nb, nd, n, kRsThreads * (big ? kSortItemsBig : kRsItems), row_total);
+            if (big) hipLaunchKernelGGL(rs_hist_kernel<kSortItemsBig>, dim3(nb), dim3(kRsThreads), 0, s, ki, n, nd, drop, shift, bits, hist, nb, SpanArgs{});
+            else hipLaunchKernelGGL(rs_hist_kernel<kRsItems>, dim3(nb), dim3(kRsThreads), 0, s, ki, n, nd, drop, shift, bits, hist, nb, SpanArgs{});
+            hipLaunchKernelGGL(rs_scan_rows_kernel, dim3(1 << bits), dim3(kRsThreads), 0, s, hist, nb, nd, n, kRsThreads * (big ? kSortItemsBig : kRsItems), row_total,
+                               (const uint32_t*)nullptr, 0);
         }
 #define SR_SCATTER_W(B, A, I, Wd) do { if (sweep && B == 8) hipLaunchKernelGGL((rs_scatter_kernel<B == 8 ? 8 : 0, A, I, Wd, B == 8>), dim3(nb), dim3(kRsThreads), 0, s, ki, vi, ko, vo, n, nd, drop, shift, bits, \
                                                  (const uint32_t*)nullptr, (const uint32_t*)(ghist + p * kRsMaxBins), nb, (Wd ? p == 0 : last) ? aux_src : nullptr, last ? aux_out : nullptr, ri, ro, rect_bx, rect_by, \
-                                                 hist, tickets + p, (uint32_t)(p + 1) << 29);                                                                    \
+                                                 hist, tickets + p, (uint32_t)(p + 1) << 29, SpanArgs{});                                                        \
                                    else hipLaunchKernelGGL((rs_scatter_kernel<B, A, I, Wd>), dim3(nb), dim3(kRsThreads), 0, s, ki, vi, ko, vo, n, nd, drop, shift, bits, (const uint32_t*)hist, \
-                                                 (const uint32_t*)row_total, nb, (Wd ? p == 0 : last) ? aux_src : nullptr, last ? aux_out : nullptr, ri, ro, rect_bx, rect_by, (uint32_t*)nullptr, (uint32_t*)nullptr, 0u); } while (0)
+                                                 (const uint32_t*)row_total, nb, (Wd ? p == 0 : last) ? aux_src : nullptr, last ? aux_out : nullptr, ri, ro, rect_bx, rect_by, (uint32_t*)nullptr, (uint32_t*)nullptr, 0u, SpanArgs{}); } while (0)
 #define SR_SCATTER_R(B, A, I) do { if (wide) SR_SCATTER_W(B, A, I, true); else SR_SCATTER_W(B, A, I, false); } while (0)
 #define SR_SCATTER(B, I) do { if (rank_mode == kRankAtomic) SR_SCATTER_R(B, true, I); else SR_SCATTER_R(B, false, I); } while (0)
         switch (bits) {
@@ -442,15 +523,65 @@
     return hipGetLastError();
 }
 
+static inline bool depth_sort_big(uint32_t n) { return n >= kSortRideFrom; }
+static inline int depth_sort_blocks(uint32_t n) { return depth_sort_big(n) ? rs_blocks(n, kSortItemsBig) : rs_blocks(n); }
+static inline bool depth_sort_hist_in_ride(uint32_t n) { return n >= 1024u && !depth_sort_big(n); }
+static inline size_t depth_sort_tail_offset(uint32_t n) {
+    return align_up((size_t)n * 4, 256) * 3 + (depth_sort_hist_in_ride(n) ? 0 : align_up((size_t)depth_sort_blocks(n) * kSpanMaxBins * 4, 256));
+}
+size_t depth_sort_pairs_temp_bytes(uint32_t n) { return radix_sort_temp_bytes(n > 0 ? n : 1); }
+size_t depth_sort_key_bounds_offset(uint32_t n) { return depth_sort_tail_offset(n > 0 ? n : 1) + kSpanMaxBins * 4; }
+size_t depth_sort_block_keys_offset(uint32_t n) { return align_up(((size_t)(n > 0 ? n : 1) + 63) / 64 * 8, 256); }
+hipError_t depth_sort_pairs(const uint32_t* keys_in, uint32_t* keys_out, uint32_t* vals_out, uint32_t n, void* temp, size_t temp_bytes, hipStream_t s,
+                            const uint2* aux_src, uint2* aux_out, RankMode rank_mode, int rect_bx, int rect_by, const uint32_t* n_live,
+                            const uint32_t* key_bounds) {
+    if (n == 0) return hipSuccess;
+    if (temp_bytes < depth_sort_pairs_temp_bytes(n) || depth_sort_key_bounds_offset(n) + 8 > radix_sort_temp_bytes(n) || (rank_mode != kRankAtomic && rank_mode != kRankBallot) || !aux_src || !aux_out || !n_live || !key_bounds)
+        return hipErrorInvalidValue;
+    char* t = static_cast<char*>(temp);
+    SpanArgs sp{};
+    sp.bounds = key_bounds;
+    sp.tk = reinterpret_cast<uint32_t*>(t); t += align_up((size_t)n * 4, 256);
+    sp.tv = reinterpret_cast<uint32_t*>(t); t += align_up((size_t)n * 4, 256);
+    sp.tr = reinterpret_cast<uint32_t*>(t); t += align_up((size_t)n * 4, 256);
+    sp.ok = keys_out; sp.ov = vals_out; sp.oaux = aux_out;
+    const bool big = depth_sort_big(n);
+    const int nb = depth_sort_blocks(n);
+    uint32_t* hist = depth_sort_hist_in_ride(n) ? sp.tr : reinterpret_cast<uint32_t*>(t);
+    uint32_t* row_total = reinterpret_cast<uint32_t*>(static_cast<char*>(temp) + depth_sort_tail_offset(n));
+    if (key_bounds != row_total + kSpanMaxBins) return hipErrorInvalidValue;
+    const bool wide = rect_bx > 0 && rect_by > 0 && 2 * (rect_bx + rect_by) <= 32 && n >= kSortRideFrom;
+    for (int p = 0; p < 4; ++p) {
+        sp.pass = p;
+        const uint32_t* nd = p > 0 ? n_live : nullptr;
+        const int drop = p == 0 ? 1 : 0;
+        if (big) hipLaunchKernelGGL((rs_hist_kernel<kSortItemsBig, true>), dim3(nb), dim3(kRsThreads), 0, s, keys_in, n, nd, drop, 0, 0, hist, nb, sp);
+        else hipLaunchKernelGGL((rs_hist_kernel<kRsItems, true>), dim3(nb), dim3(kRsThreads), 0, s, keys_in, n, nd, drop, 0, 0, hist, nb, sp);
+        hipLaunchKernelGGL(rs_scan_rows_kernel, dim3(kSpanMaxBins), dim3(kRsThreads), 0, s, hist, nb, nd, n, kRsThreads * (big ? kSortItemsBig : kRsItems), row_total,
+                           key_bounds, p);
+#define SR_SPAN_SCATTER(A, I, Wd) hipLaunchKernelGGL((rs_scatter_kernel<0, A, I, Wd, false, true>), dim3(nb), dim3(kRsThreads), 0, s, keys_in, (const uint32_t*)nullptr,     \
+                                      (uint32_t*)nullptr, (uint32_t*)nullptr, n, nd, drop, 0, 0, (const uint32_t*)hist, (const uint32_t*)row_total, nb, aux_src,             \
+                                      (uint2*)nullptr, (const uint32_t*)nullptr, (uint32_t*)nullptr, rect_bx, rect_by, (uint32_t*)nullptr, (uint32_t*)nullptr, 0u, sp)
+#define SR_SPAN_SCATTER_I(A, I) do { if (wide) SR_SPAN_SCATTER(A, I, true); else SR_SPAN_SCATTER(A, I, false); } while (0)
+#define SR_SPAN_SCATTER_A(A) do { if (big) SR_SPAN_SCATTER_I(A, kSortItemsBig); else SR_SPAN_SCATTER_I(A, kRsItems); } while (0)
+        if (rank_mode == kRankAtomic) SR_SPAN_SCATTER_A(true); else SR_SPAN_SCATTER_A(false);
+#undef SR_SPAN_SCATTER_A
+#undef SR_SPAN_SCATTER_I
+#undef SR_SPAN_SCATTER
+    }
+    return hipGetLastError();
+}
+
 size_t tile_count_scan_temp_bytes(uint32_t n) { return align_up((2 * (size_t)scan_blocks(n > 0 ? n : 1) + 2) * 4, 256); }
 
-hipError_t tile_count_scan(const uint32_t* counts, uint32_t* out, uint32_t n, void* temp, size_t temp_bytes, uint32_t* total_host, hipStream_t s) {
+hipError_t tile_count_scan(const uint32_t* counts, uint32_t* out, uint32_t n, void* temp, size_t temp_bytes, uint32_t* total_host, const uint2* wave_keys,
+                           uint2* block_keys, uint32_t* key_bounds, hipStream_t s) {
     if (n == 0) return hipSuccess;
     if (temp_bytes < tile_count_scan_temp_bytes(n)) return hipErrorInvalidValue;
     const int nb = scan_blocks(n);
     uint32_t* totals = static_cast<uint32_t*>(temp);
-    hipLaunchKernelGGL(scan_blocks_kernel, dim3(nb), dim3(kRsThreads), 0, s, counts, n, out, totals);
-    hipLaunchKernelGGL(scan_totals_kernel, dim3(1), dim3(kRsThreads), 0, s, totals, nb, total_host);
+    hipLaunchKernelGGL(scan_blocks_kernel, dim3(nb), dim3(kRsThreads), 0, s, counts, n, out, totals, key_bounds ? wave_keys : nullptr, block_keys);
+    hipLaunchKernelGGL(scan_totals_kernel, dim3(1), dim3(kRsThreads), 0, s, totals, nb, total_host, (const uint2*)block_keys, key_bounds);
     return hipGetLastError();
 }
 
```

New measurement: 927.7 Msplats/s, median of 6. No clear change (+0.5%).
